# richardshuai/ExPecto

Measured on AMD Instinct MI355X. Metric: variants/sec (200 windows × 2002 feats) at 1/2/4/8 MI355X; HBM GB/s vs peak, higher is better.
Workload: dtype fp32 in/out (f16x3: power-of-2-scaled 2-way fp16 split = 22-bit operands, 3 MFMA products, fp32 accumulate; bf16x6 recompute on fp16 overflow)

## Files before the change

expecto_amd/csrc/beluga.hip:

```cpp
#include <hip/hip_runtime.h>

#include <algorithm>
#include <array>
#include <cassert>
#include <cstdint>
#include <cstdlib>
#include <cstring>
#include <map>
#include <mutex>
#include <tuple>
#include <string>
#include <vector>

#include "common.h"
#include "gemm_kernel.h"

namespace expecto {

constexpr int kLen = 2000;
constexpr int kNFeat = 2002;
constexpr int kFc1In = 67840;
constexpr int kFc1Out = 2003;
constexpr int kHidLd = 2016;
constexpr int kWM = 4;
// ... 218 lines not shown
  if (bad && ovf) *ovf = 1;
  _Float16* d = reinterpret_cast<_Float16*>(h1) + act_index<2>(row, kHidLd, n);
  *reinterpret_cast<halfx4*>(d) = hv;
  *reinterpret_cast<halfx4*>(d + 32) = lv;
}

constexpr int kFc2Chunk = 8;
__device__ __forceinline__ float fc2_value(float s, const float* __restrict__ col_scale, const float* __restrict__ bias,
                                           int n) {
  if (col_scale) s *= col_scale[n];
  const float v = s + bias[n];
  return 1.0f / (1.0f + expf(-v));
}
__global__ __launch_bounds__(256) void fc2_reduce(const float* __restrict__ part, int splits, long long split_stride,
                                                  int M, const float* __restrict__ bias,
                                                  const float* __restrict__ col_scale,
                                                  const long long* __restrict__ c_rows, float* __restrict__ y) {
  static_assert(kNFeat % 2 == 0 && kHidLd % 2 == 0, "2 features per thread");
  const int n = 2 * (blockIdx.x * blockDim.x + threadIdx.x);
  if (n >= kNFeat) return;
  for (long long m = blockIdx.y; m < M; m += gridDim.y) {
    const float* src = part + m * kHidLd + n;
    float s0 = 0.f, s1 = 0.f;
    for (int k0 = 0; k0 < splits; k0 += kFc2Chunk) {
      float2 v[kFc2Chunk];
#pragma unroll
      for (int u = 0; u < kFc2Chunk; ++u)
        v[u] = *reinterpret_cast<const float2*>(src + (long long)min(k0 + u, splits - 1) * split_stride);
#pragma unroll
      for (int u = 0; u < kFc2Chunk; ++u)
        if (k0 + u < splits) {
          s0 += v[u].x;
          s1 += v[u].y;
        }
    }
    float2 o;
    o.x = fc2_value(s0, col_scale, bias, n);
    o.y = fc2_value(s1, col_scale, bias, n + 1);
    *reinterpret_cast<float2*>(y + (c_rows ? c_rows[m] : m) * kNFeat + n) = o;
  }
}
__global__ void fc2_reduce1(const float* __restrict__ part, int splits, long long split_stride, int M,
                            const float* __restrict__ bias, const float* __restrict__ col_scale,
                            const long long* __restrict__ c_rows, float* __restrict__ y) {
  const long long i = (long long)blockIdx.x * blockDim.x + threadIdx.x;
  if (i >= (long long)M * kNFeat) return;
  const int m = (int)(i / kNFeat), n = (int)(i - (long long)m * kNFeat);
  const long long src = (long long)m * kHidLd + n;
  float s = 0.f;
  for (int k = 0; k < splits; ++k) s += part[k * split_stride + src];
  y[(c_rows ? c_rows[m] : m) * kNFeat + n] = fc2_value(s, col_scale, bias, n);
}

__global__ void pool4_phases(const float* __restrict__ in, int n_seg, int s_in, int t_in, int C,
                             int n_ph, int4 ph, int s_out, float* __restrict__ out, int fmt) {
  const int c = threadIdx.x;
  const int g = blockIdx.x;
  const int i = blockIdx.y % n_ph;
  const long long seg = blockIdx.y / n_ph;
  const int p = i == 0 ? ph.x : i == 1 ? ph.y : i == 2 ? ph.z : ph.w;
  if (c >= C || g >= (t_in - p) / 4) return;
  const long long r0 = seg * s_in + p + 4LL * g, orow = (seg * n_ph + i) * s_out + g;
  float m = load_act_rt(fmt, in, r0, C, c);
#pragma unroll
  for (int j = 1; j < 4; ++j) m = fmaxf(m, load_act_rt(fmt, in, r0 + j, C, c));
  store_act_rt(fmt, out, orow, C, c, m);
}

typedef _Float16 halfx8 __attribute__((ext_vector_type(8)));
__global__ __launch_bounds__(256) void pool4_phases_h2(const float* __restrict__ in, int s_in, int t_in, int C,
                                                        int n_ph, int4 ph, int s_out, float* __restrict__ out) {
  const int c8 = threadIdx.x & 63;
  const int g = blockIdx.x * 4 + (threadIdx.x >> 6);
  const int i = blockIdx.y % n_ph;
  const long long seg = blockIdx.y / n_ph;
  const int p = i == 0 ? ph.x : i == 1 ? ph.y : i == 2 ? ph.z : ph.w;
  if (c8 >= C / 8 || g >= (t_in - p) / 4) return;
  const long long rb = (long long)C * 4;
  const int cofs = (c8 >> 2) * 128 + (c8 & 3) * 16;
  const char* src = reinterpret_cast<const char*>(in) + (seg * s_in + p + 4LL * g) * rb + cofs;
  halfx8 hi[4], lo[4];
#pragma unroll
  for (int j = 0; j < 4; ++j) {
    hi[j] = *reinterpret_cast<const halfx8*>(src + j * rb);
    lo[j] = *reinterpret_cast<const halfx8*>(src + j * rb + 64);
  }
  halfx8 oh, ol;
#pragma unroll
  for (int e = 0; e < 8; ++e) {
    float m = (float)hi[0][e] + (float)lo[0][e];
#pragma unroll
    for (int j = 1; j < 4; ++j) m = fmaxf(m, (float)hi[j][e] + (float)lo[j][e]);
    _Float16 h, l;
    split_h2(m, h, l);
    oh[e] = h;
    ol[e] = l;
  }
  char* dst = reinterpret_cast<char*>(out) + ((seg * n_ph + i) * s_out + g) * rb + cofs;
  *reinterpret_cast<halfx8*>(dst) = oh;
  *reinterpret_cast<halfx8*>(dst + 64) = ol;
}

__global__ __launch_bounds__(256) void pool4_phases_h2m(const float* __restrict__ in, int s_in, int t_in, int C,
                                                         int n_ph, int4 ph, int s_out, float* __restrict__ out) {
  const int c8 = threadIdx.x & 63;
  const int g = blockIdx.x * 4 + (threadIdx.x >> 6);
  const long long seg = blockIdx.y;
  const int pmin = ph.x;
  const int pmax = n_ph == 1 ? ph.x : n_ph == 2 ? ph.y : n_ph == 3 ? ph.z : ph.w;
  if (c8 >= C / 8 || g >= (t_in - pmin) / 4) return;
  const long long rb = (long long)C * 4;
  const int cofs = (c8 >> 2) * 128 + (c8 & 3) * 16;
  const char* src = reinterpret_cast<const char*>(in) + (seg * s_in + pmin + 4LL * g) * rb + cofs;
  const int nr = min(pmax - pmin + 4, t_in - pmin - 4 * g);
  halfx8 hi[7], lo[7];
#pragma unroll
  for (int j = 0; j < 7; ++j) {
    if (j < nr) {
      hi[j] = *reinterpret_cast<const halfx8*>(src + j * rb);
      lo[j] = *reinterpret_cast<const halfx8*>(src + j * rb + 64);
    }
  }
  float fv[7][8];
#pragma unroll
  for (int j = 0; j < 7; ++j)
#pragma unroll
    for (int e = 0; e < 8; ++e) fv[j][e] = j < nr ? (float)hi[j][e] + (float)lo[j][e] : 0.f;
#pragma unroll
  for (int i = 0; i < 4; ++i) {
    if (i >= n_ph) break;
    const int p = i == 0 ? ph.x : i == 1 ? ph.y : i == 2 ? ph.z : ph.w;
    if (g >= (t_in - p) / 4) continue;
    const int o = p - pmin;
    halfx8 oh, ol;
#pragma unroll
    for (int e = 0; e < 8; ++e) {
      float m = 0.f;
#pragma unroll
      for (int j = 0; j < 4; ++j) {
        const float v = o == 0 ? fv[j][e] : o == 1 ? fv[j + 1][e] : o == 2 ? fv[j + 2][e] : fv[j + 3][e];
        m = j == 0 ? v : fmaxf(m, v);
      }
      _Float16 h, l;
      split_h2(m, h, l);
      oh[e] = h;
      ol[e] = l;
    }
    char* dst = reinterpret_cast<char*>(out) + ((seg * n_ph + i) * s_out + g) * rb + cofs;
    *reinterpret_cast<halfx8*>(dst) = oh;
    *reinterpret_cast<halfx8*>(dst + 64) = ol;
  }
}

__global__ void seg_a_rows(const int* __restrict__ win_seg, const int* __restrict__ win_off,
                           const int* __restrict__ win_row, const int* __restrict__ widx, int w0, int m_count,
                           int seg_base, int rc, int seg_len, int n_ph, int4 ph_idx, int s7, long long row_base,
                           long long* __restrict__ a_rows, long long* __restrict__ c_rows) {
  const int m = blockIdx.x * blockDim.x + threadIdx.x;
  if (m >= m_count) return;
  const int w = widx ? widx[m] : w0 + m;
  c_rows[m] = row_base + (win_row ? win_row[w] : w);
  const int o = rc ? seg_len - 2000 - win_off[w] : win_off[w];
  const int q = o >> 2, p = q & 3, off6 = (q - p) >> 2;
  const int pi = p == 0 ? ph_idx.x : p == 1 ? ph_idx.y : p == 2 ? ph_idx.z : ph_idx.w;
  const long long blk = (long long)(win_seg[w] - seg_base) * n_ph + pi;
  a_rows[m] = (blk * s7 + off6) * 640;
}

constexpr int kDW[7] = {0, 8, 5, 12, 6, 13, 20};
constexpr int kDA[7] = {0, 15, 28, 19, 32, 20, 27};
constexpr int kDT[7] = {0, 1993, 496, 489, 120, 113, 106};
constexpr int kDC[7] = {4, 320, 320, 480, 480, 640, 640};

struct DeltaRows {
  int r[7];
  int base[7];
};

__device__ __forceinline__ int clampi(int v, int lo, int hi) { return v < lo ? lo : (v > hi ? hi : v); }
__device__ __forceinline__ int floor4(int v) { return v >= 0 ? v >> 2 : -((3 - v) >> 2); }

__device__ __forceinline__ DeltaRows delta_rows(int p) {
  DeltaRows d;
  d.r[0] = p;
  d.r[1] = clampi(p - 7, 0, kDT[1] - kDW[1]);
  d.r[2] = clampi(floor4(d.r[1] - 7), 0, kDT[2] - kDW[2]);
  d.r[3] = clampi(d.r[2] - 7, 0, kDT[3] - kDW[3]);
  d.r[4] = clampi(floor4(d.r[3] - 7), 0, kDT[4] - kDW[4]);
  d.r[5] = clampi(d.r[4] - 7, 0, kDT[5] - kDW[5]);
  d.r[6] = clampi(d.r[5] - 7, 0, kDT[6] - kDW[6]);
  d.base[0] = 0;
  d.base[1] = d.r[1];
  d.base[2] = 4 * d.r[2];
  d.base[3] = d.r[3];
  d.base[4] = 4 * d.r[4];
  d.base[5] = d.r[5];
  d.base[6] = d.r[6];
  return d;
}

__device__ __forceinline__ int pair_pos(const int* var_pos, int m, int nv, int v0) {
  const int s = m / nv, v = v0 + m % nv;
  const int pv = min(max(var_pos[v], 0), kLen - 1);
  return s ? kLen - 1 - pv : pv;
}

__global__ void delta_codes(const uint8_t* __restrict__ alt, long long stride, int nv, int v0,
                            const int* __restrict__ var_pos, uint8_t* __restrict__ out, int R) {
  const int i = threadIdx.x & 15;
  const int m = blockIdx.x * (blockDim.x >> 4) + (threadIdx.x >> 4);
  if (m >= R) return;
  const int s = m / nv, v = v0 + m % nv;
  const int start = delta_rows(pair_pos(var_pos, m, nv, v0)).r[1];
  const uint8_t* a = alt + (long long)v * stride;
  const int pos = min(start + i, kLen - 1);
  uint8_t c;
  if (s) {
    const uint8_t f = a[kLen - 1 - pos];
    c = f < 4 ? (uint8_t)(3 - f) : f;
  } else {
    c = a[pos];
  }
  out[(long long)m * 16 + i] = c;
}

__global__ __launch_bounds__(256) void delta_assemble(const float* __restrict__ ref, int ref_rows,
                                                      const float* __restrict__ dprev, int l, int row16, int nv, int v0,
                                                      const int* __restrict__ var_pos, float* __restrict__ out) {
  const int m = blockIdx.x;
  const DeltaRows d = delta_rows(pair_pos(var_pos, m, nv, v0));
  const int rp = d.r[l - 1], wp = kDW[l - 1];
  floatx4* to = reinterpret_cast<floatx4*>(out) + (long long)m * kDA[l] * row16;
  for (int k = threadIdx.x; k < kDA[l] * row16; k += blockDim.x) {
    const int i = k / row16, c = k - i * row16;
    const int src = min(d.base[l] + i, ref_rows - 1);
    const floatx4* from = (src >= rp && src < rp + wp)
                              ? reinterpret_cast<const floatx4*>(dprev) + ((long long)m * wp + src - rp) * row16
                              : reinterpret_cast<const floatx4*>(ref) + ((long long)m * ref_rows + src) * row16;
    to[k] = from[c];
  }
}

__global__ void fc1_slab_mask(const int* __restrict__ var_pos, int nv, int v0, int R, int tile_rows, int slab_k,
                              unsigned* __restrict__ mask) {
  const int m = blockIdx.x * blockDim.x + threadIdx.x;
  if (m >= R) return;
  const int r6 = delta_rows(pair_pos(var_pos, m, nv, v0)).r[6];
  const int k0 = r6 * 640, k1 = (r6 + kDW[6]) * 640 - 1;
  unsigned bits = 0;
  for (int ks = k0 / slab_k; ks <= k1 / slab_k; ++ks) bits |= 1u << ks;
  atomicOr(mask + m / tile_rows, bits);
}

__global__ __launch_bounds__(64) void slab_macs(const unsigned* __restrict__ mask, int tiles, double per_bit,
                                                double* __restrict__ acc) {
  int bits = 0;
  for (int i = threadIdx.x; i < tiles; i += 64) bits += __popc(mask[i]);
  for (int o = 32; o > 0; o >>= 1) bits += __shfl_down(bits, o);
  if (threadIdx.x == 0) atomicAdd(acc, bits * per_bit);
}

__global__ __launch_bounds__(256) void pair_patch_apply(const float* __restrict__ d6, float* __restrict__ act6, int nv,
                                                        int v0, const int* __restrict__ var_pos, int row16) {
  const int m = blockIdx.x;
  const int r6 = delta_rows(pair_pos(var_pos, m, nv, v0)).r[6];
  const floatx4* src = reinterpret_cast<const floatx4*>(d6) + (long long)m * kDW[6] * row16;
  floatx4* dst = reinterpret_cast<floatx4*>(act6) + ((long long)m * 106 + r6) * row16;
  for (int k = threadIdx.x; k < kDW[6] * row16; k += blockDim.x) dst[k] = src[k];
}

constexpr int kSegTab = 20;
constexpr int kW4u = 19, kA4u = 26;
struct SegDims {
  int L, T1, P1, T3, T4, S5, T5, T6;
};

__global__ void seg_delta_table(const int* __restrict__ var_pos, int s0, int ns, int rc, SegDims g, int n_ph, int4 ph,
                                int* __restrict__ tab) {
  const int m = blockIdx.x * blockDim.x + threadIdx.x;
  if (m >= ns) return;
  int q = min(max(var_pos[s0 + m], 0), g.L - 1);
  if (rc) q = g.L - 1 - q;
  int* t = tab + m * kSegTab;
  const int r1 = clampi(q - 7, 0, g.T1 - kDW[1]);
  const int r2 = clampi(floor4(r1 - 7), 0, g.P1 - kDW[2]);
  const int r3 = clampi(r2 - 7, 0, g.T3 - kDW[3]);
  const int r4 = clampi(r3 - 7, 0, g.T4 - kW4u);
  t[0] = q;
  t[1] = r1;
  t[2] = r2;
  t[3] = r3;
  t[4] = r4;
  for (int i = 0; i < n_ph; ++i) {
    const int p = i == 0 ? ph.x : i == 1 ? ph.y : i == 2 ? ph.z : ph.w;
    const int r4p = clampi(floor4(r4 - p), 0, g.S5 - kDW[4]);
    const int r5 = clampi(r4p - 7, 0, g.T5 - kDW[5]);
    t[5 + i] = r4p;
    t[9 + i] = r5;
    t[13 + i] = clampi(r5 - 7, 0, g.T6 - kDW[6]);
  }
}

__global__ void seg_delta_codes(const uint8_t* __restrict__ codes, long long stride, const uint8_t* __restrict__ alt_code,
                                int s0, int ns, int rc, int L, const int* __restrict__ tab, uint8_t* __restrict__ out) {
  const int i = threadIdx.x & 15;
  const int m = blockIdx.x * (blockDim.x >> 4) + (threadIdx.x >> 4);
  if (m >= ns) return;
  const int q = tab[m * kSegTab], x = min(tab[m * kSegTab + 1] + i, L - 1);
  uint8_t c = x == q ? alt_code[s0 + m] : codes[(long long)(s0 + m) * stride + (rc ? L - 1 - x : x)];
  if (rc && c < 4) c = (uint8_t)(3 - c);
  out[(long long)m * 16 + i] = c;
}

constexpr int kC1Pat = kDA[2] + 7, kC1PatStride = 48;
__global__ void seg_delta_codes2(const uint8_t* __restrict__ codes, long long stride, const uint8_t* __restrict__ alt_code,
                                 int s0, int ns, int rc, int L, const int* __restrict__ tab, uint8_t* __restrict__ out) {
  const int i = threadIdx.x % kC1PatStride;
  const int m = blockIdx.x * (blockDim.x / kC1PatStride) + threadIdx.x / kC1PatStride;
  if (m >= ns) return;
  const int q = tab[m * kSegTab], x = 4 * tab[m * kSegTab + 2] + i;
  uint8_t c = 4;
  if (i < kC1Pat && x < L) {
    c = x == q ? alt_code[s0 + m] : codes[(long long)(s0 + m) * stride + (rc ? L - 1 - x : x)];
    if (rc && c < 4) c = (uint8_t)(3 - c);
  }
  out[(long long)m * kC1PatStride + i] = c;
}

__global__ void delta_codes2(const uint8_t* __restrict__ alt, long long stride, int nv, int v0,
                             const int* __restrict__ var_pos, uint8_t* __restrict__ out, int R) {
  const int i = threadIdx.x % kC1PatStride;
  const int m = blockIdx.x * (blockDim.x / kC1PatStride) + threadIdx.x / kC1PatStride;
  if (m >= R) return;
  const int s = m / nv, v = v0 + m % nv;
  const int pos = 4 * delta_rows(pair_pos(var_pos, m, nv, v0)).r[2] + i;
  const uint8_t* a = alt + (long long)v * stride;
  uint8_t c = 4;
  if (i < kC1Pat && pos < kLen) {
    if (s) {
      const uint8_t f = a[kLen - 1 - pos];
      c = f < 4 ? (uint8_t)(3 - f) : f;
    } else {
      c = a[pos];
    }
  }
  out[(long long)m * kC1PatStride + i] = c;
}

__global__ __launch_bounds__(256) void seg_delta_assemble(const float* __restrict__ ref, int ref_rows,
                                                          const float* __restrict__ dprev, int wprev,
                                                          const int* __restrict__ tab, int nb, int ib, int mult, int irp,
                                                          int arows, int row16, float* __restrict__ out) {
  const int m = blockIdx.x;
  const int seg = m / nb, off = nb > 1 ? m % nb : 0;
  const int base = mult * tab[seg * kSegTab + ib + off], rp = tab[seg * kSegTab + irp + off];
  floatx4* to = reinterpret_cast<floatx4*>(out) + (long long)m * arows * row16;
  for (int k = threadIdx.x; k < arows * row16; k += blockDim.x) {
    const int i = k / row16, c = k - i * row16;
    const int src = min(base + i, ref_rows - 1);
    const floatx4* from = (src >= rp && src < rp + wprev)
                              ? reinterpret_cast<const floatx4*>(dprev) + ((long long)m * wprev + src - rp) * row16
                              : reinterpret_cast<const floatx4*>(ref) + ((long long)m * ref_rows + src) * row16;
    to[k] = from[c];
  }
}

constexpr int kSegEdge = 32;
__device__ __forceinline__ int seg_edge_lo(const int* t) { return min(4 * t[5], 2 + 4 * t[6]); }
__global__ void seg_delta_pool(const float* __restrict__ conv4, int t4, const float* __restrict__ d4, int n_ph,
                               int4 ph, const int* __restrict__ tab, int fmt, float* __restrict__ out, int edge = 0) {
  const int c = threadIdx.x;
  if (c >= 480) return;
  const int gi = blockIdx.x, m = blockIdx.y;
  const int seg = m / n_ph, i = m % n_ph;
  const int p = i == 0 ? ph.x : i == 1 ? ph.y : i == 2 ? ph.z : ph.w;
  const int r4 = tab[seg * kSegTab + 4];
  const int row0 = p + 4 * (tab[seg * kSegTab + 5 + i] + gi);
  const int elo = edge ? seg_edge_lo(tab + seg * kSegTab) : 0;
  float mx = 0.f;
#pragma unroll
  for (int j = 0; j < 4; ++j) {
    const int row = row0 + j;
    const bool alt = row >= r4 && row < r4 + kW4u;
    const float* b = alt ? d4 : conv4;
    const long long r = alt    ? (long long)seg * kW4u + row - r4
                        : edge ? (long long)seg * kSegEdge + row - elo
                               : (long long)seg * t4 + row;
    const float v = load_act_rt(fmt, b, r, 480, c);
    mx = j == 0 ? v : fmaxf(mx, v);
  }
  store_act_rt(fmt, out, (long long)m * kDW[4] + gi, 480, c, mx);
}

__global__ void pool2_tile_seams(const float* __restrict__ seam, long long M, int s_in, int t4, int s5,
                                 float* __restrict__ out) {
  const int c8 = threadIdx.x;
  if (c8 >= 60) return;
  const long long k = blockIdx.x + 1, b = 256 * k;
  if (b + 1 >= M) return;
  const long long w = (b - 2) / s_in;
  const int t = (int)(b - 2 - w * s_in), g = (t - 2) >> 2;
  if (t + 3 >= t4) return;
  constexpr long long rb = 480 * 4;
  const int cofs = (c8 >> 2) * 128 + (c8 & 3) * 16;
  const char* sb = reinterpret_cast<const char*>(seam);
  const char* src[4] = {sb + ((k - 1) * 4 + 2) * rb, sb + ((k - 1) * 4 + 3) * rb, sb + (k * 4 + 0) * rb,
                        sb + (k * 4 + 1) * rb};
  halfx8 oh, ol;
  float m[8];
#pragma unroll
  for (int j = 0; j < 4; ++j) {
    const halfx8 hv = *reinterpret_cast<const halfx8*>(src[j] + cofs), lv = *reinterpret_cast<const halfx8*>(src[j] + cofs + 64);
#pragma unroll
    for (int e = 0; e < 8; ++e) {
      const float v = (float)hv[e] + (float)lv[e];
      m[e] = j == 0 ? v : fmaxf(m[e], v);
    }
  }
#pragma unroll
  for (int e = 0; e < 8; ++e) {
    _Float16 h, l;
    split_h2(m[e], h, l);
    oh[e] = h;
    ol[e] = l;
  }
  char* dst = reinterpret_cast<char*>(out) + ((2 * w + 1) * s5 + g) * rb + cofs;
  *reinterpret_cast<halfx8*>(dst) = oh;
  *reinterpret_cast<halfx8*>(dst + 64) = ol;
}

constexpr int kAltRows6 = 232;
__global__ void seg_alt_blocks(const float* __restrict__ ref6, const float* __restrict__ d6, int n_ph, int t6,
                               const int* __restrict__ tab, int row16, float* __restrict__ out) {
  const int m = blockIdx.y;
  const int q = tab[(m / n_ph) * kSegTab];
  const int t = (q >= 1999 ? (q - 1999) >> 4 : 0) + blockIdx.x;
  if (t >= t6 || t >= (q >> 4) + 106) return;
  const int r6 = tab[(m / n_ph) * kSegTab + 13 + m % n_ph];
  const floatx4* src = (t >= r6 && t < r6 + kDW[6])
                           ? reinterpret_cast<const floatx4*>(d6) + ((long long)m * kDW[6] + t - r6) * row16
                           : reinterpret_cast<const floatx4*>(ref6) + ((long long)m * t6 + t) * row16;
  floatx4* dst = reinterpret_cast<floatx4*>(out) + ((long long)m * t6 + t) * row16;
  for (int c = threadIdx.x; c < row16; c += blockDim.x) dst[c] = src[c];
}

__global__ void fc1_slab_mask_seg(const int* __restrict__ widx, int n_alt, const int* __restrict__ win_seg,
                                  const int* __restrict__ win_off, int seg_base, int rc, int seg_len, int4 ph_idx,
                                  const int* __restrict__ tab, int tile_rows, int slab_k, unsigned* __restrict__ mask) {
  const int m = blockIdx.x * blockDim.x + threadIdx.x;
  if (m >= n_alt) return;
  const int w = widx[m];
  const int o = rc ? seg_len - 2000 - win_off[w] : win_off[w];
  const int q = o >> 2, p = q & 3, off6 = (q - p) >> 2;
  const int pi = p == 0 ? ph_idx.x : p == 1 ? ph_idx.y : p == 2 ? ph_idx.z : ph_idx.w;
  const int r6 = tab[(win_seg[w] - seg_base) * kSegTab + 13 + pi];
  const int lo = max(r6 - off6, 0), hi = min(r6 + kDW[6] - off6, 106);
  if (lo >= hi) return;
  unsigned bits = 0;
  for (int ks = lo * 640 / slab_k; ks <= (hi * 640 - 1) / slab_k; ++ks) bits |= 1u << ks;
  atomicOr(mask + m / tile_rows, bits);
}

__global__ void copy_rows(const float* __restrict__ src, float* __restrict__ dst, const int* __restrict__ widx,
                          const int* __restrict__ win_row, long long row_base) {
  const int w = widx[blockIdx.x];
  const long long r = (row_base + (win_row ? win_row[w] : w)) * kNFeat;
  for (int i = threadIdx.x; i < kNFeat; i += blockDim.x) dst[r + i] = src[r + i];
}

__global__ void pair_rows(long long* __restrict__ c_rows, int M, int nv, int v0, long long strand_stride) {
  const int m = blockIdx.x * blockDim.x + threadIdx.x;
  if (m < M) c_rows[m] = (long long)(m / nv) * strand_stride + v0 + m % nv;
}

constexpr int kFkK = 16000;
constexpr int kFkKb = kFkK / GBK;
constexpr int kFkSlabs = 2;
constexpr int kFkTailK = kFc1In - 4 * kFkK;
constexpr int kFkKbTotal = 9 * kFkKb + kFkTailK / GBK;
constexpr long long kFkKTotal = 9LL * kFkK + kFkTailK;
constexpr int kFkSeq[9] = {3, 2, 3, 1, 0, 1, 3, 2, 3};
constexpr int kFkBlk[9] = {0, 1, 1, 2, 3, 3, 2, 3, 3};
constexpr int kFkRole[4][4] = {{0, 1, 3, 4}, {1, 2, 4, 5}, {3, 4, 6, 7}, {4, 5, 7, 8}};
constexpr int kFkW[9][4] = {{1, 0, 0, 0}, {1, 1, 0, 0}, {0, -1, 0, 0}, {1, 0, 1, 0}, {1, 1, 1, 1},
                            {0, -1, 0, -1}, {0, 0, -1, 0}, {0, 0, -1, -1}, {0, 0, 0, 1}};
constexpr int kFkParts = 4 * kFkSlabs + 1;

__global__ void fk_weights(const float* __restrict__ w1, long long rows, float* __restrict__ wk) {
  const long long i = (long long)blockIdx.x * blockDim.x + threadIdx.x;
  if (i >= rows * kFkKTotal) return;
  const long long n = i / kFkKTotal;
  const int k = (int)(i - n * kFkKTotal);
  const float* wr = w1 + n * kFc1In;
  if (k >= 9 * kFkK) {
    wk[i] = wr[4 * kFkK + (k - 9 * kFkK)];
    return;
  }
  const int g = k / kFkK, kk = k - g * kFkK;
  double s = 0.0;
#pragma unroll
  for (int q = 0; q < 4; ++q)
    if (kFkW[g][q]) s += kFkW[g][q] * (double)wr[q * kFkK + kk];
  wk[i] = (float)s;
}

__global__ __launch_bounds__(320) void fk_seq_h2(const float* __restrict__ x, int T, int s, const int* __restrict__ tab,
                                                 int n_ph, const int* __restrict__ gres, float* __restrict__ d1,
                                                 float* __restrict__ d2, float* __restrict__ dd, int* __restrict__ ovf) {
  const int c8 = threadIdx.x % 80;
  const long long blk = blockIdx.x / 7;
  const int k = (int)(blockIdx.x - blk * 7) * 4 + threadIdx.x / 80;
  if (k >= 25) return;
  int lo = 0, hi = T;
  if (tab) {
    const int q = tab[(blk / n_ph) * kSegTab];
    lo = q >= 1999 ? (q - 1999) >> 4 : 0;
    hi = min(T, (q >> 4) + 106);
  }
  const int g = gres ? gres[blk] : -1;
  if (g == -2) return;
  int r = k;
  if (r < lo) r += (lo - r + 24) / 25 * 25;
  if (r + 25 >= hi) return;
  constexpr long long rb = 640 * 4;
  const long long base = blk * s * rb + (c8 >> 2) * 128 + (c8 & 3) * 16;
  auto ld = [&](int row, float (&v)[8]) {
    const char* p = reinterpret_cast<const char*>(x) + base + row * rb;
    const halfx8 h = *reinterpret_cast<const halfx8*>(p);
    const halfx8 l = *reinterpret_cast<const halfx8*>(p + 64);
#pragma unroll
    for (int e = 0; e < 8; ++e) v[e] = (float)h[e] + (float)l[e];
  };
  bool bad = false;
  auto put = [&](float* dst, int row, const float (&y)[8]) {
    halfx8 h, l;
#pragma unroll
    for (int e = 0; e < 8; ++e) {
      bad |= !(fabsf(y[e]) < 65504.f);
      _Float16 a, b;
      split_h2p(y[e], a, b);
      h[e] = a;
      l[e] = b;
    }
    const int j = c8 & 7;
    const bool low = j < 4;
    u32x4 send = __builtin_bit_cast(u32x4, low ? l : h), recv;
#pragma unroll
    for (int w = 0; w < 4; ++w) recv[w] = (unsigned)__builtin_amdgcn_update_dpp(0, (int)send[w], 0x141, 0xf, 0xf, false);
    const u32x4 keep = __builtin_bit_cast(u32x4, low ? h : l);
    char* d = reinterpret_cast<char*>(dst) + blk * s * rb + row * rb + (c8 >> 3) * 256;
    auto st = [](char* p, const u32x4& v) { *reinterpret_cast<u32x4*>(p) = v; };
    if (low) {
      st(d + j * 16, keep);
      st(d + 128 + (3 - j) * 16, recv);
    } else {
      st(d + 64 + (7 - j) * 16, recv);
      st(d + 128 + 64 + (j - 4) * 16, keep);
    }
  };
  float v0[8], v1[8], v2[8] = {}, v3[8] = {};
  ld(r, v0);
  ld(r + 25, v1);
  if (r + 50 < hi) ld(r + 50, v2);
  if (r + 75 < hi) ld(r + 75, v3);
  for (; r + 25 < hi; r += 25) {
    float nv[8] = {};
    if (r + 100 < hi) ld(r + 100, nv);
    bool need1 = true, need2 = true;
    if (g >= 0) {
      const int rel = ((r - g) % 100 + 100) % 100;
      need1 = rel >= 50;
      need2 = (rel >= 25 && rel < 50) || rel >= 75;
    }
    float a[8], y[8];
#pragma unroll
    for (int e = 0; e < 8; ++e) a[e] = v0[e] - v1[e];
    if (need1) put(d1, r, a);
    if (r + 50 < hi && need2) {
#pragma unroll
      for (int e = 0; e < 8; ++e) y[e] = v0[e] - v2[e];
      put(d2, r, y);
    }
    if (r + 75 < hi) {
#pragma unroll
      for (int e = 0; e < 8; ++e) y[e] = a[e] - (v2[e] - v3[e]);
      put(dd, r, y);
    }
#pragma unroll
    for (int e = 0; e < 8; ++e) {
      v0[e] = v1[e];
      v1[e] = v2[e];
      v2[e] = v3[e];
      v3[e] = nv[e];
    }
  }
  if (bad) *ovf = 1;
}

__global__ void fk_reduce_h2(const float* __restrict__ part, const int* __restrict__ prow, long long count4,
                             const float* __restrict__ bias, float* __restrict__ h1, const float* __restrict__ col_scale,
                             float osc, int* __restrict__ ovf) {
  const long long i4 = (long long)blockIdx.x * blockDim.x + threadIdx.x;
  if (i4 >= count4) return;
  const long long row = i4 / (kHidLd / 4);
  const int n = (int)(i4 - row * (kHidLd / 4)) * 4;
  floatx4 s = {0.f, 0.f, 0.f, 0.f};
#pragma unroll
  for (int j = 0; j < kFkParts; ++j) {
    const floatx4 v = *reinterpret_cast<const floatx4*>(part + (long long)prow[row * kFkParts + j] * kHidLd + n);
#pragma unroll
    for (int e = 0; e < 4; ++e) s[e] += v[e];
  }
  halfx4 hv, lv;
  bool bad = false;
#pragma unroll
  for (int e = 0; e < 4; ++e) {
    const float t = s[e] * col_scale[n + e];
    const float v = n + e < kFc1Out ? fmaxf(t + bias[min(n + e, kFc1Out - 1)], 0.f) : 0.f;
    const float x = v * osc;
// ... 337 lines not shown
#pragma unroll
    for (int c = 0; c < 4; ++c) m[c] = r == 0 ? s[c] : fmaxf(m[c], s[c]);
  }
  floatx4 v;
  float vmax = 0.f;
#pragma unroll
  for (int c = 0; c < 4; ++c) {
    v[c] = fmaxf(fmaf(m[c], osc, bb[c] * osc), 0.f);
    vmax = fmaxf(vmax, v[c]);
  }
  if (fmt == 1) {
    bf16x4 x0, x1, x2;
    split3(v, x0, x1, x2);
    char* d = reinterpret_cast<char*>(out) + ((win * s_out + g) * 10 + (q >> 3)) * 192 + (q & 7) * 8;
    *reinterpret_cast<bf16x4*>(d) = x0;
    *reinterpret_cast<bf16x4*>(d + 64) = x1;
    *reinterpret_cast<bf16x4*>(d + 128) = x2;
    return;
  }
  const halfx4 hv = __builtin_convertvector(v, halfx4);
  const halfx4 lv = __builtin_convertvector(v - __builtin_convertvector(hv, floatx4), halfx4);
  char* d = reinterpret_cast<char*>(out) + ((win * s_out + g) * 10 + (q >> 3)) * 128 + (q & 7) * 8;
  *reinterpret_cast<halfx4*>(d) = hv;
  *reinterpret_cast<halfx4*>(d + 64) = lv;
  if (!(vmax < 65504.f)) *ovf = 1;
}

__global__ __launch_bounds__(256) void onehot_codes(const float* __restrict__ x, long long n, int len,
                                                    uint8_t* __restrict__ codes, int* __restrict__ bad) {
  const int len4 = len >> 2;
  const long long q = (long long)blockIdx.x * blockDim.x + threadIdx.x;
  if (q >= n * len4) return;
  const long long w = q / len4;
  const int p = (int)(q - w * len4) * 4;
  const float* xr = x + w * 4LL * len + p;
  unsigned b[4][4];
#pragma unroll
  for (int c = 0; c < 4; ++c) {
    const floatx4 v = *reinterpret_cast<const floatx4*>(xr + (long long)c * len);
#pragma unroll
    for (int e = 0; e < 4; ++e) b[c][e] = __float_as_uint(v[e]);
  }
  bool ok = true;
  unsigned packed = 0;
#pragma unroll
  for (int e = 0; e < 4; ++e) {
    unsigned code = 4, ones = 0;
#pragma unroll
    for (int c = 0; c < 4; ++c) {
      if (b[c][e] == 0x3f800000u) {
        ++ones;
        code = c;
      } else if (b[c][e] != 0u) {
        ok = false;
      }
    }
    ok &= ones <= 1;
    packed |= code << (8 * e);
  }
  if (!ok) *bad = 1;
  if (codes) *reinterpret_cast<unsigned*>(codes + w * len + p) = packed;
}

namespace {
constexpr int kNumLayers = 9;
struct ConvGeo {
  int cin, cout, s_in, t_valid, s_out, pool;
};
constexpr int kS1 = 1996;
constexpr ConvGeo kConv[5] = {
    {320, 320, kS1, 496, 496, 1},
    {320, 480, 496, 489, 492, 0},
    {480, 480, 492, 120, 120, 1},
    {480, 640, 120, 113, 113, 0},
    {640, 640, 113, 106, 106, 0},
};
constexpr int kFc2SplitsDefault = 7;
constexpr int kFcSplitsDefault = 8;
}

struct expecto_beluga {
  int device = 0;
  int max_batch = 0;
  float* w1 = nullptr;
  float* b1 = nullptr;
  float* wt[5] = {};
  float* bt[5] = {};
  float* fc1w = nullptr;
  float* fc1b = nullptr;
  float* fc2w = nullptr;
  float* fc2b = nullptr;
  float* wp[5] = {};
  float* fc1p = nullptr;
  float* fc2p = nullptr;
  float* wh[7] = {};
  int* swd[7] = {};
  float* w1h = nullptr;
  float* cs1 = nullptr;
  float* cs[7] = {};
  int sx[7] = {};
  int f16_target = 10;
  bool f16_ready = false;
  int* ovf = nullptr;
  bool ovf_deferred = false;
  float* calib = nullptr;
  long long fallbacks = 0;
  void* stage_buf[2] = {};
  size_t stage_cap[2] = {};
  hipEvent_t stage_ev[2] = {};
  int stage_next = 0;
  double* macs_d = nullptr;
  float* P = nullptr;
  float* Q = nullptr;
  float* part = nullptr;
  float* part2 = nullptr;
  float* h1 = nullptr;
  long long* a_rows = nullptr;
  long long* c_rows = nullptr;
  int fc2_rows = 0;
  int* win_seg_d = nullptr;
  int* alt_w_d = nullptr;
  int* copy_w_d = nullptr;
  int* seg_var_d = nullptr;
  int seg_var_cap = 0;
  int* win_off_d = nullptr;
  int* win_row_d = nullptr;
  int* fc_perm_d = nullptr;
  hipStream_t st2 = nullptr;
  hipEvent_t pev[16] = {};
  bool overlap = true;
  float* DA = nullptr;
  float* D0 = nullptr;
  float* D1 = nullptr;
  uint8_t* delta_codes = nullptr;
  int* seg_tab = nullptr;
  float* slab_mask = nullptr;
  int win_cap = 0;
  size_t bytes = 0;
  std::vector<void*> allocs;
  int precision = EXPECTO_PRECISION_BF16X6;
  int fc_splits = kFcSplitsDefault;
  int fc2_splits = kFc2SplitsDefault;
  double fc1_m_order_mb = 80.0;
  int fc1_order = 3;
  int fc1_m_group = 8;
  bool fc_wide = true;
  int conv_tile = 0;
  bool conv_ea = true;
  bool fc_skinny = true;
  int fc1_narrow = -1;
  int conv_narrow = -1;
  bool narrow_scope = false;
  int seg_chunk_windows = 0;
  int cus = 0;
  bool pool_one_pass = true;
  bool pool_fused = true;
  float* seam = nullptr;
  float* edge = nullptr;
  size_t seam_cap = 0, edge_cap = 0;
  bool fuse_conv1 = true;
  bool kmer_on = true;
  float* kmer = nullptr;
  uint64_t kmer_key = 0;
  bool kmer_quad = true;
  int kmer_state = 1;
  bool fk_on = true;
  int fk_role = 4;
  float* fkw = nullptr;
  int* fk_sw = nullptr;
  float* fk_cs = nullptr;
  float* fk_seq[3] = {};
  long long fk_seq_rows = 0;
  long long* fk_grows = nullptr;
  long long* fk_wrows = nullptr;
  int* fk_prow = nullptr;
  unsigned* fk_mask = nullptr;
  int fk_slice = 24576;
  float* fk_part = nullptr;
  float* fk_h1 = nullptr;
  long long* fk_arows = nullptr;
  long long* fk_crows = nullptr;
  int* fk_gres = nullptr;
  long long fk_gres_cap = 0;
  float* fk_aseq[3] = {};
  long long fk_aseq_rows = 0;
  int* fk_rgrp = nullptr;
  int* fk_ginfo = nullptr;
  int* fk_winfo = nullptr;
  int* fk_aprow = nullptr;
  int* fk_aperm = nullptr;
  unsigned* fk_smask = nullptr;
  bool onehot_as_codes = true;
  uint8_t* oh_codes = nullptr;
  int* oh_bad = nullptr;
  bool oh_hint_bad = false;
  int* hflags = nullptr;
  int* hflags_d = nullptr;
  bool profiling = false;
  std::vector<hipEvent_t> ev_pool;
  std::vector<std::pair<int, int>> pending;
  size_t ev_next = 0;
  int timer_base = 0;
  double ms[2 * kNumLayers] = {};
  long long calls[2 * kNumLayers] = {};
  double macs[2 * kNumLayers] = {};
  struct LaunchRec {
    int layer;
    long long rows;
    int idx;
    double macs;
  };
  std::vector<LaunchRec> pending_launch;
  std::map<std::pair<int, long long>, std::array<double, 3>> launch_stats;
};

namespace {
int dalloc(expecto_beluga* h, float** p, size_t nfloat) {
  void* ptr = nullptr;
  hipError_t e = hipMalloc(&ptr, nfloat * sizeof(float));
  if (e != hipSuccess) {
    set_error(std::string("hipMalloc: ") + hipGetErrorString(e));
    return EXPECTO_ENOMEM;
  }
  e = hipMemset(ptr, 0, nfloat * sizeof(float));
  if (e != hipSuccess) {
    (void)hipFree(ptr);
    set_error(std::string("hipMemset: ") + hipGetErrorString(e));
    return EXPECTO_EHIP;
  }
  h->allocs.push_back(ptr);
  h->bytes += nfloat * sizeof(float);
  *p = static_cast<float*>(ptr);
  return EXPECTO_OK;
}

int npad_of(int n) { return (n + GBN - 1) / GBN * GBN; }

struct KmerEntry {
  int device;
  uint64_t key;
  std::vector<float> w;
  float* T;
  std::vector<const expecto_beluga*> holders;
};
std::mutex g_kmer_mu;
std::vector<KmerEntry> g_kmer;

uint64_t fnv1a(const void* p, size_t n, uint64_t hsh = 1469598103934665603ULL) {
  const unsigned char* b = static_cast<const unsigned char*>(p);
  for (size_t i = 0; i < n; ++i) hsh = (hsh ^ b[i]) * 1099511628211ULL;
  return hsh;
}

int kmer_no_room(expecto_beluga* h, const char* why) {
  h->kmer_state = 2;
  fprintf(stderr, "expecto_hip: no k-mer tables on device %d (%s): conv2 runs on the MFMAs (about -25%% throughput)\n",
          h->device, why);
  return EXPECTO_OK;
}

int kmer_acquire(expecto_beluga* h, const float* const* params, hipStream_t st) {
  const size_t tb = kKmerFloats * sizeof(float), fb = (size_t)kMer8 * 320 * sizeof(double);
  if (const char* e = getenv("EXPECTO_KMER_MAX_BYTES"))
    if ((double)tb > atof(e)) return kmer_no_room(h, "EXPECTO_KMER_MAX_BYTES");
  std::vector<float> hw(320 * 32 + 320 + 320 * 320 * 8);
  EXPECTO_HIP_CHECK(hipMemcpyAsync(hw.data(), params[0], 320 * 32 * sizeof(float), hipMemcpyDeviceToHost, st));
  EXPECTO_HIP_CHECK(hipMemcpyAsync(hw.data() + 320 * 32, params[1], 320 * sizeof(float), hipMemcpyDeviceToHost, st));
  EXPECTO_HIP_CHECK(hipMemcpyAsync(hw.data() + 320 * 33, params[2], 320 * 320 * 8 * sizeof(float),
                                   hipMemcpyDeviceToHost, st));
  EXPECTO_HIP_CHECK(hipStreamSynchronize(st));
  const uint64_t key = fnv1a(hw.data(), hw.size() * sizeof(float));
  std::lock_guard<std::mutex> lock(g_kmer_mu);
  for (KmerEntry& e : g_kmer)
    if (e.device == h->device && e.key == key && e.w == hw) {
      e.holders.push_back(h);
      h->kmer = e.T;
      h->kmer_key = key;
      h->kmer_state = 0;
      return EXPECTO_OK;
    }
  void *t = nullptr, *f = nullptr, *gg = nullptr;
  if (hipMalloc(&t, tb) != hipSuccess || hipMalloc(&f, fb) != hipSuccess || hipMalloc(&gg, 8 * fb) != hipSuccess) {
    (void)hipGetLastError();
    for (void* x : {t, f, gg})
      if (x) (void)hipFree(x);
    return kmer_no_room(h, "device allocation failed");
  }
  float* T = static_cast<float*>(t);
  double* F = static_cast<double*>(f);
  double* G = static_cast<double*>(gg);
  kmer_conv1<<<dim3(kMer8), dim3(320), 0, st>>>(h->w1, h->b1, F);
  int rc = check_launch("kmer_conv1");
  for (int j = 0; j < 8; ++j)
    kmer_conv2<<<dim3((kMer8 + 63) / 64, 5), dim3(256), 0, st>>>(F, h->wt[0], j, G + (size_t)j * kMer8 * 320);
  for (int i = 0; i < 4; ++i)
    kmer_pair<<<dim3((unsigned)((kMer9 * 320 + 255) / 256)), dim3(256), 0, st>>>(
        G + (size_t)(2 * i) * kMer8 * 320, G + (size_t)(2 * i + 1) * kMer8 * 320, T + (size_t)i * kMer9 * 320);
  for (int hq = 0; hq < 2; ++hq)
    kmer_quad<<<dim3((unsigned)((kMer11 * 320 + 255) / 256)), dim3(256), 0, st>>>(
        G, hq, T + (4 * (size_t)kMer9 + hq * (size_t)kMer11) * 320);
  rc = rc ? rc : check_launch("kmer table");
  if (!rc && hipStreamSynchronize(st) != hipSuccess) rc = check_launch("kmer table sync");
  (void)hipFree(f);
  (void)hipFree(gg);
  if (rc) {
    (void)hipFree(t);
    return rc;
  }
  g_kmer.push_back({h->device, key, std::move(hw), T, {h}});
  h->kmer = T;
  h->kmer_key = key;
  h->kmer_state = 0;
  return EXPECTO_OK;
}

void kmer_release(expecto_beluga* h) {
  if (!h->kmer) return;
  std::lock_guard<std::mutex> lock(g_kmer_mu);
  for (size_t i = 0; i < g_kmer.size(); ++i)
    if (g_kmer[i].T == h->kmer) {
      auto& hs = g_kmer[i].holders;
      const auto it = std::find(hs.begin(), hs.end(), h);
      assert(it != hs.end() && "k-mer table held by an unregistered handle");
      if (it != hs.end()) hs.erase(it);
      if (hs.empty()) {
        (void)hipFree(g_kmer[i].T);
        g_kmer.erase(g_kmer.begin() + (long)i);
      }
      break;
    }
  h->kmer = nullptr;
}

size_t kmer_reported_bytes(const expecto_beluga* h) {
  if (!h->kmer) return 0;
  std::lock_guard<std::mutex> lock(g_kmer_mu);
// ... 398 lines not shown
    if ((rc = check_launch("beluga_conv_h3p pool2"))) return rc;
  }
  LayerTimer lt(h, 3, st);
  if (a.m_tiles > 1)
    pool2_tile_seams<<<dim3((unsigned)(a.m_tiles - 1)), dim3(64), 0, st>>>(h->seam, a.M, s_in, t4, s5, dst);
  return check_launch("pool2_tile_seams");
}

float* h1_rows(expecto_beluga* h, long long rows) { return h->h1 + rows * kHidLd * act_bytes() / 4; }

bool fc_wide_tiles(const expecto_beluga* h) { return h->fc_wide && g_precision == EXPECTO_PRECISION_F16X3; }

bool fc1_narrow(const expecto_beluga* h, long long mtt);
bool fc_skinny(const expecto_beluga* h, long long rows);

int run_fc1(expecto_beluga* h, const float* act, const long long* a_rows, int nb, float* h1, hipStream_t st,
            const unsigned* ks_mask = nullptr, double slab_frac = 1.0, long long part_rows = 0) {
  if (part_rows <= 0) part_rows = nb;
  int rc;
  const long long m_tiles = (nb + gemm_bm() - 1) / gemm_bm();
  const bool wide = fc_wide_tiles(h);
  const int n_tiles1 = wide ? (kHidLd + FCW_BN - 1) / FCW_BN : npad_of(kFc1Out) / GBN;
  const int splits = h->fc_splits;
  {
    GemmArgs a{};
    a.A = act;
    a.a_rows = a_rows;
    a.lda = (long long)kFc1In;
    a.M = nb;
    a.B = h->fc1w;
    a.Bp = g_precision == EXPECTO_PRECISION_F16X3 ? h->wh[5] : h->fc1p;
    a.ldb = kFc1In;
    a.kper = kFc1In / splits;
    a.taps = 1;
    a.n_tiles = n_tiles1;
    a.m_tiles = m_tiles;
    a.m_fastest = (double)m_tiles * gemm_bm() * (kFc1In / splits) * 4.0 <= h->fc1_m_order_mb * (1 << 20) ? 1 : 0;
    a.linear_order = a.m_fastest;
    if (h->fc1_order == 2 && !a.m_fastest && m_tiles % 8 == 0 && planes_gemm() && g_precision == EXPECTO_PRECISION_F16X3)
      a.m_fastest = 2;
    if (h->fc1_order == 3 && g_precision == EXPECTO_PRECISION_F16X3) {
      a.m_fastest = 3;
      a.m_group = h->fc1_m_group;
      a.linear_order = 0;
    }
    if (wide) {
      a.m_fastest = 0;
      a.linear_order = 0;
      a.n_tile_cols = FCW_BN;
      if (!ks_mask && fc_skinny(h, nb)) {
        a.n_tile_cols = 16 * FCS_NB;
        a.n_tiles = kHidLd / a.n_tile_cols;
      } else if (!ks_mask && fc1_narrow(h, m_tiles * splits)) {
        a.n_tile_cols = 112;
        a.n_tiles = kHidLd / 112;
      }
    }
    a.C = h->part;
    a.ldc = kHidLd;
    a.n_store = kHidLd;
    a.split_stride = part_rows * kHidLd;
    a.ks_mask = ks_mask;
    EXPECTO_REQUIRE(!ks_mask || planes_gemm(), "slab mask needs the planes GEMM");
    LayerTimer lt(h, 6, st);
    if (h->profiling) h->macs[h->timer_base + 6] += (double)nb * kFc1Out * kFc1In * slab_frac;
    if ((rc = launch_gemm<7, EPI_PARTIAL>(a, splits, st))) return rc;
  }
  {
    LayerTimer lt(h, 7, st);
    const long long count = (long long)nb * kHidLd;
    const bool f16 = g_precision == EXPECTO_PRECISION_F16X3;
    if (act_fmt() == 2)
      fc1_reduce_h2<<<dim3((unsigned)((count / 4 + 255) / 256)), dim3(256), 0, st>>>(
          h->part, splits, part_rows * kHidLd, count / 4, h->fc1b, h1, h->cs[5], exp2i(h->sx[6]), h->ovf);
    else
      fc1_reduce<<<dim3((unsigned)((count + 255) / 256)), dim3(256), 0, st>>>(
          h->part, splits, part_rows * kHidLd, count, h->fc1b, h1, act_fmt(), f16 ? h->cs[5] : nullptr, exp2i(h->sx[6]), h->ovf);
    if ((rc = check_launch("fc1_reduce"))) return rc;
  }
  return EXPECTO_OK;
}

int run_fc2(expecto_beluga* h, const float* h1, int nb, float* y, hipStream_t st, const long long* c_rows) {
  int rc;
  const long long m_tiles = (nb + gemm_bm() - 1) / gemm_bm();
  {
    GemmArgs a{};
    a.A = h1;
    a.lda = kHidLd;
    a.M = nb;
    a.B = h->fc2w;
    a.Bp = g_precision == EXPECTO_PRECISION_F16X3 ? h->wh[6] : h->fc2p;
    a.col_scale = g_precision == EXPECTO_PRECISION_F16X3 ? h->cs[6] : nullptr;
    a.ldb = kHidLd;
    a.kper = kHidLd / h->fc2_splits;
    a.taps = 1;
    const bool wide = fc_wide_tiles(h) && h->fc2_splits > 1;
    a.n_tiles = wide ? (kNFeat + FCW_BN - 1) / FCW_BN : npad_of(kNFeat) / GBN;
    a.m_tiles = m_tiles;
    a.m_fastest = (double)m_tiles * gemm_bm() * (kHidLd / h->fc2_splits) * 4.0 <= h->fc1_m_order_mb * (1 << 20) ? 1 : 0;
    if (wide) {
      a.m_fastest = 0;
      a.n_tile_cols = FCW_BN;
      if (fc_skinny(h, nb)) {
        a.n_tile_cols = 16 * FCS_NB;
        a.n_tiles = (kNFeat + a.n_tile_cols - 1) / a.n_tile_cols;
      } else if (fc1_narrow(h, m_tiles * h->fc2_splits)) {
        a.n_tile_cols = 112;
        a.n_tiles = (kNFeat + 111) / 112;
      }
    }
    a.C = h->part2;
    a.ldc = kHidLd;
    a.n_store = kNFeat;
    a.split_stride = (long long)nb * kHidLd;
    LayerTimer lt(h, 8, st);
    if (h->profiling) h->macs[h->timer_base + 8] += (double)nb * kNFeat * kFc1Out;
    if (h->fc2_splits == 1) {
      a.C = y;
      a.ldc = kNFeat;
      a.c_rows = c_rows;
      a.bias = h->fc2b;
      a.s_in = a.t_valid = a.s_out = 1;
      return launch_gemm<8, EPI_SIGMOID>(a, 1, st);
    }
    if ((rc = launch_gemm<8, EPI_PARTIAL>(a, h->fc2_splits, st))) return rc;
    if ((reinterpret_cast<uintptr_t>(y) & 7) == 0)
      fc2_reduce<<<dim3((unsigned)((kNFeat / 2 + 255) / 256), (unsigned)std::max<long long>(1, std::min<long long>(nb, 65535))), dim3(256), 0,
                   st>>>(h->part2, h->fc2_splits, (long long)nb * kHidLd, nb, h->fc2b, a.col_scale, c_rows, y);
    else
      fc2_reduce1<<<dim3((unsigned)(((long long)nb * kNFeat + 255) / 256)), dim3(256), 0, st>>>(
          h->part2, h->fc2_splits, (long long)nb * kHidLd, nb, h->fc2b, a.col_scale, c_rows, y);
    if ((rc = check_launch("fc2_reduce"))) return rc;
  }
  return EXPECTO_OK;
}

int run_fc(expecto_beluga* h, const float* act, const long long* a_rows, int nb, float* y, hipStream_t st,
           const long long* c_rows = nullptr, const unsigned* ks_mask = nullptr, double slab_frac = 1.0,
           long long part_rows = 0) {
  int rc;
  if ((rc = run_fc1(h, act, a_rows, nb, h->h1, st, ks_mask, slab_frac, part_rows))) return rc;
  return run_fc2(h, h->h1, nb, y, st, c_rows);
}

int count_desc_macs(expecto_beluga* h, const unsigned* mask, int tiles, double per_tile, hipStream_t st);

bool fk_use(const expecto_beluga* h) {
  return h->fk_on && h->fkw && g_precision == EXPECTO_PRECISION_F16X3 && h->fk_role < 4;
}
bool fk_use_seg(const expecto_beluga* h) { return h->fk_on && h->fkw && g_precision == EXPECTO_PRECISION_F16X3; }

int fk_cap(const expecto_beluga* h) { return std::max(h->max_batch, h->fk_slice); }

int fk_tables(expecto_beluga* h) {
  if (h->fk_grows) return EXPECTO_OK;
  const size_t mb = h->max_batch, tiles = (mb + 255) / 256, cap = fk_cap(h);
  float *a = nullptr, *b = nullptr, *c = nullptr, *d = nullptr;
  int rc;
  if ((rc = dalloc(h, &a, 2 * 9 * cap)) || (rc = dalloc(h, &b, 2 * mb)) || (rc = dalloc(h, &c, kFkParts * cap)) ||
      (rc = dalloc(h, &d, kFkParts * tiles)))
    return rc;
  h->fk_grows = reinterpret_cast<long long*>(a);
  h->fk_wrows = reinterpret_cast<long long*>(b);
  h->fk_prow = reinterpret_cast<int*>(c);
  h->fk_mask = reinterpret_cast<unsigned*>(d);
  return EXPECTO_OK;
}

int fk_seg_buffers(expecto_beluga* h) {
  if (h->fk_part) return EXPECTO_OK;
  const size_t cap = fk_cap(h);
  float *a = nullptr, *b = nullptr;
  int rc;
  if ((rc = dalloc(h, &h->fk_part, (size_t)kFkParts * cap * kHidLd)) || (rc = dalloc(h, &h->fk_h1, act_alloc(cap * kHidLd))) ||
      (rc = dalloc(h, &a, 2 * cap)) || (rc = dalloc(h, &b, 2 * cap)))
    return rc;
  h->fk_arows = reinterpret_cast<long long*>(a);
  h->fk_crows = reinterpret_cast<long long*>(b);
  float *c = nullptr, *d = nullptr, *e = nullptr, *f = nullptr, *q = nullptr, *m = nullptr;
  if ((rc = dalloc(h, &c, 9 * cap)) || (rc = dalloc(h, &d, 2 * cap)) || (rc = dalloc(h, &e, 2 * cap)) ||
      (rc = dalloc(h, &f, kFkParts * cap)) || (rc = dalloc(h, &q, cap)) || (rc = dalloc(h, &m, 19 * (cap / 256 + 1))))
    return rc;
  h->fk_rgrp = reinterpret_cast<int*>(c);
  h->fk_ginfo = reinterpret_cast<int*>(d);
  h->fk_winfo = reinterpret_cast<int*>(e);
  h->fk_aprow = reinterpret_cast<int*>(f);
  h->fk_aperm = reinterpret_cast<int*>(q);
  h->fk_smask = reinterpret_cast<unsigned*>(m);
  return EXPECTO_OK;
}

int fk_seq_alloc(expecto_beluga* h, long long rows, int set = 0) {
  float** b = set ? h->fk_aseq : h->fk_seq;
  long long& cap = set ? h->fk_aseq_rows : h->fk_seq_rows;
  if (rows <= cap && b[0]) return EXPECTO_OK;
  for (int i = 0; i < 3; ++i)
    if (b[i]) {
      EXPECTO_HIP_CHECK(hipFree(b[i]));
      b[i] = nullptr;
    }
  h->bytes -= (size_t)cap * 640 * 4 * 3;
  cap = 0;
  for (int i = 0; i < 3; ++i) {
    hipError_t e = hipMalloc(&b[i], (size_t)rows * 640 * 4 + 16 * 640 * 4);
    if (e != hipSuccess) {
      set_error(std::string("hipMalloc (FC1 sequences): ") + hipGetErrorString(e));
      return EXPECTO_ENOMEM;
    }
  }
  cap = rows;
  h->bytes += (size_t)rows * 640 * 4 * 3;
  return EXPECTO_OK;
}

int fk_sequences(expecto_beluga* h, const float* x, long long blocks, int T, int s, const int* tab, int n_ph,
                 hipStream_t st, const int* gres = nullptr, int set = 0) {
  int rc;
  if ((rc = fk_seq_alloc(h, blocks * s, set))) return rc;
  float* const* out = set ? h->fk_aseq : h->fk_seq;
  LayerTimer lt(h, 7, st);
  const long long nblk = blocks * 7;
  EXPECTO_REQUIRE(nblk > 0 && nblk < (1LL << 31), "FC1 sequence grid");
  fk_seq_h2<<<dim3((unsigned)nblk), dim3(320), 0, st>>>(x, T, s, tab, n_ph, gres, out[0], out[1], out[2], h->ovf);
  return check_launch("fk_seq_h2");
}

struct FkProducts {
  const long long* g_rows;
  int off[9];
  int cnt[9];
  int lay[9];
};

int fk_reduce(expecto_beluga* h, const float* part, const int* prow, int n, float* h1, hipStream_t st) {
  LayerTimer lt(h, 7, st);
  const long long count4 = (long long)n * (kHidLd / 4);
  fk_reduce_h2<<<dim3((unsigned)((count4 + 255) / 256)), dim3(256), 0, st>>>(part, prow, count4, h->fc1b, h1, h->fk_cs,
                                                                           exp2i(h->sx[6]), h->ovf);
  return check_launch("fk_reduce_h2");
}

constexpr int kFcNarrowNb = 7;
static_assert(kHidLd % (16 * kFcNarrowNb) == 0 && kHidLd % FCW_BN == 0, "FC1 N tiles");
bool fc1_narrow(const expecto_beluga* h, long long mtt) {
  if (h->fc1_narrow >= 0) return h->fc1_narrow != 0;
  if (!h->narrow_scope) return false;
  const long long cus = h->cus > 0 ? h->cus : 256;
  return mtt * (kHidLd / (16 * kFcNarrowNb)) <= cus;
}

static_assert(kHidLd % (16 * FCS_NB) == 0 &&
                  (kNFeat + 16 * FCS_NB - 1) / (16 * FCS_NB) * 16 * FCS_NB <= (kNFeat + GBN - 1) / GBN * GBN,
              "skinny FC tiles");
bool fc_skinny(const expecto_beluga* h, long long rows) {
  return h->fc_skinny && rows <= 32 && (h->fc1_narrow >= 0 ? h->fc1_narrow != 0 : h->narrow_scope);
}

int fk_fc1(expecto_beluga* h, const float* x, float* const* seq, const FkProducts& pr, const long long* w_rows, int n,
           const int* prow, float* h1, hipStream_t st, const unsigned* mask = nullptr, int tiles = 0,
           float* part = nullptr, long long part_cap = 0) {
  if (!part) {
    part = h->part;
    part_cap = (long long)std::max(h->fc_splits, kFkParts) * h->max_batch;
  }
  FcGroup G{};
  G.kb_total = kFkKbTotal;
  G.n_tiles = (kHidLd + FCW_BN - 1) / FCW_BN;
  G.n_store = kHidLd;
  G.ldc = kHidLd;
  const char* wb = reinterpret_cast<const char*>(h->fkw);
  long long row = 0;
  long long blk = 0;
  int mslot = 0;
  double macs = 0.0;
  auto add = [&](const float* A, const long long* ar, long long aoff, int kb0, int nk, int M, int lay) {
    FcDesc& d = G.d[G.n];
    d.A = A;
    d.a_rows = ar;
    d.a_off = aoff;
    d.Bp = wb + (long long)kb0 * 128;
    d.C = part + row * kHidLd;
    d.mask = mask ? mask + (size_t)mslot * tiles : nullptr;
    ++mslot;
    d.M = M;
    d.m_tiles = (M + X6P_BM - 1) / X6P_BM;
    d.nk = nk;
    d.blk0 = (int)blk;
    blk += (long long)d.m_tiles * G.n_tiles;
    row += lay;
    macs += (double)M * kFc1Out * nk * GBK;
    ++G.n;
  };
  for (int g = 0; g < 9; ++g) {
    const int lay = pr.lay[g] ? pr.lay[g] : pr.cnt[g];
    for (int s = 0; lay > 0 && s < kFkSlabs; ++s) {
      if (pr.cnt[g] > 0)
        add(kFkSeq[g] ? seq[kFkSeq[g] - 1] : x, pr.g_rows + pr.off[g], 25LL * kFkBlk[g] * 640 + (long long)s * kFkK / kFkSlabs,
            g * kFkKb + s * kFkKb / kFkSlabs, kFkKb / kFkSlabs, pr.cnt[g], lay);
      else {
        row += lay;
        ++mslot;
      }
    }
  }
  add(x, w_rows, 100LL * 640, 9 * kFkKb, kFkTailK / GBK, n, n);
  EXPECTO_REQUIRE(G.n <= FCK_MAX && blk < (1LL << 31), "Karatsuba FC1 descriptors");
  EXPECTO_REQUIRE(row <= part_cap, "Karatsuba FC1 partial rows");
  {
    LayerTimer lt(h, 6, st);
    if (h->profiling) {
      if (!mask) {
        h->macs[h->timer_base + 6] += macs;
      } else {
        for (int i = 0; i < G.n; ++i) {
          const FcDesc& d = G.d[i];
          int rc = count_desc_macs(h, d.mask, d.m_tiles, (double)d.M / d.m_tiles * kFc1Out * d.nk * GBK, st);
          if (rc) return rc;
        }
      }
    }
    G.rr = mask ? 0 : 1;
    const long long mtt = blk / G.n_tiles;
    const bool narrow = !mask && fc1_narrow(h, mtt);
    if (narrow) {
      G.n_tiles = kHidLd / (16 * kFcNarrowNb);
      for (int i = 0; i < G.n; ++i) G.d[i].blk0 = G.d[i].blk0 / (kHidLd / FCW_BN) * G.n_tiles;
    }
    const long long grid = G.rr ? (mtt + 7) / 8 * 8 * G.n_tiles : mtt * G.n_tiles;
    if (narrow)
      beluga_fc_h3k_narrow<<<dim3((unsigned)grid), dim3(512), 0, st>>>(G);
    else
      beluga_fc_h3k<0><<<dim3((unsigned)grid), dim3(512), 0, st>>>(G);
    int rc = check_launch("beluga_fc_h3k");
    if (rc) return rc;
  }
  return prow ? fk_reduce(h, part, prow, n, h1, st) : EXPECTO_OK;
}

struct FkWin {
  int w, blk, off6;
};
int fk_role_of(int off6) { return (off6 / 25) & 3; }
FkWin fk_win(int w, const int* win_seg, const int* win_off, int s0, bool rc, int L, int n_ph, const int* ph_idx) {
  const int o = rc ? L - kLen - win_off[w] : win_off[w];
  const int q = o >> 2, p = q & 3;
  return {w, (win_seg[w] - s0) * n_ph + ph_idx[p], (q - p) >> 2};
}
bool fk_same_group(const FkWin& a, const FkWin& b) {
  return a.blk == b.blk && a.off6 - 25 * fk_role_of(a.off6) == b.off6 - 25 * fk_role_of(b.off6);
}

void fk_slice_tables(const std::vector<FkWin>& ws, int i0, int i1, int T6, std::vector<long long>& grows,
                     FkProducts& pr, std::vector<int>& prow, std::vector<int>* rgrp = nullptr,
                     std::vector<int>* ginfo = nullptr) {
  const int n = i1 - i0;
  std::vector<int> gi(n);
  std::vector<long long> gst;
  std::vector<unsigned> need;
  for (int i = i0; i < i1; ++i) {
    const FkWin& w = ws[i];
    if (i == i0 || !fk_same_group(w, ws[i - 1])) {
      gst.push_back(((long long)w.blk * T6 + w.off6 - 25 * fk_role_of(w.off6)) * 640);
      need.push_back(0u);
    }
    gi[i - i0] = (int)gst.size() - 1;
    for (int j = 0; j < 4; ++j) need.back() |= 1u << kFkRole[fk_role_of(w.off6)][j];
    if (ginfo && gi[i - i0] * 2 == (int)ginfo->size()) {
      ginfo->push_back(w.blk);
      ginfo->push_back(w.off6 - 25 * fk_role_of(w.off6));
    }
  }
  const int ng = (int)gst.size();
  std::vector<int> ridx((size_t)9 * ng, -1);
  grows.clear();
  if (rgrp) rgrp->clear();
  for (int g = 0; g < 9; ++g) {
    pr.off[g] = (int)grows.size();
    int c = 0;
    for (int k = 0; k < ng; ++k)
      if ((need[k] >> g) & 1u) {
        ridx[(size_t)g * ng + k] = c++;
        grows.push_back(gst[k]);
        if (rgrp) rgrp->push_back(k);
      }
    pr.cnt[g] = c;
    pr.lay[g] = 0;
  }
  int base[9][kFkSlabs] = {};
  int row = 0;
  for (int g = 0; g < 9; ++g)
    for (int s = 0; pr.cnt[g] > 0 && s < kFkSlabs; ++s) {
      base[g][s] = row;
      row += pr.cnt[g];
    }
  prow.assign((size_t)n * kFkParts, 0);
  for (int i = 0; i < n; ++i) {
    const int role = fk_role_of(ws[i0 + i].off6);
    for (int j = 0; j < 4; ++j) {
      const int g = kFkRole[role][j];
      for (int s = 0; s < kFkSlabs; ++s) prow[(size_t)i * kFkParts + kFkSlabs * j + s] = base[g][s] + ridx[(size_t)g * ng + gi[i]];
    }
    prow[(size_t)i * kFkParts + kFkParts - 1] = row + i;
  }
}

int fk_windows(expecto_beluga* h, const float* act, int R, float* y, hipStream_t st, const long long* c_rows,
               const unsigned* mask = nullptr, int tiles = 0) {
  int rc;
  if ((rc = fk_tables(h)) || (rc = fk_sequences(h, act, R, 106, 106, nullptr, 1, st))) return rc;
  fk_window_tables<<<dim3((R + 255) / 256), dim3(256), 0, st>>>(R, 106, h->fk_role, h->fk_grows, h->fk_wrows, h->fk_prow);
  if ((rc = check_launch("fk_window_tables"))) return rc;
  FkProducts pr{h->fk_grows, {}, {}, {}};
  for (int j = 0; j < 4; ++j) pr.cnt[kFkRole[h->fk_role][j]] = R;
  if ((rc = fk_fc1(h, act, h->fk_seq, pr, h->fk_wrows, R, h->fk_prow, h->h1, st, mask, tiles))) return rc;
  return run_fc2(h, h->h1, R, y, st, c_rows);
}

int count_slab_macs(expecto_beluga* h, const unsigned* mask, int tiles, long long nb, hipStream_t st) {
  if (!h->macs_d) {
    float* f = nullptr;
    int rc = dalloc(h, &f, 4 * kNumLayers);
    if (rc) return rc;
    h->macs_d = reinterpret_cast<double*>(f);
    EXPECTO_HIP_CHECK(hipMemsetAsync(h->macs_d, 0, 2 * kNumLayers * sizeof(double), st));
  }
  const double per_bit = (double)nb * kFc1Out * kFc1In / ((double)tiles * h->fc_splits);
  slab_macs<<<dim3(1), dim3(64), 0, st>>>(mask, tiles, per_bit, h->macs_d + kNumLayers + 6);
  return check_launch("slab_macs");
}

int count_desc_macs(expecto_beluga* h, const unsigned* mask, int tiles, double per_tile, hipStream_t st) {
  if (!h->macs_d) {
    float* f = nullptr;
    int rc = dalloc(h, &f, 4 * kNumLayers);
    if (rc) return rc;
    h->macs_d = reinterpret_cast<double*>(f);
    EXPECTO_HIP_CHECK(hipMemsetAsync(h->macs_d, 0, 2 * kNumLayers * sizeof(double), st));
  }
  slab_macs<<<dim3(1), dim3(64), 0, st>>>(mask, tiles, per_tile, h->macs_d + h->timer_base + 6);
  return check_launch("slab_macs");
}

int forward_chunk(expecto_beluga* h, const float* x, const uint8_t* codes, long long code_stride, int n_src,
                  int mode, long long row0, int nb, float* y, hipStream_t st) {
  int rc;
  g_precision = h->precision;
  g_conv_ea = h->conv_ea;
  struct Scope {
    expecto_beluga* h;
    ~Scope() { h->narrow_scope = false; }
  } scope{h};
  h->narrow_scope = true;
  const bool kmer = use_kmer(h, x);
  const bool fuse = !kmer && fuse_conv1(h, x);
  const C1Src f1{codes, code_stride, n_src, mode, row0, kLen};
  if (!kmer && !fuse && (rc = run_conv1(h, x, codes, code_stride, n_src, mode, row0, nb, kLen, kS1, st))) return rc;
  float* src = h->P;
  float* dst = h->Q;
  for (int l = 0; l < 5; ++l) {
    const ConvGeo& g = kConv[l];
    if (l == 0 && kmer)
      rc = run_conv2_kmer(h, f1, nb, g.t_valid, g.s_out, dst, st);
    else
      rc = run_conv(h, l, src, dst, nb, g.s_in, g.t_valid, g.s_out, g.pool != 0, st, l == 0 && fuse ? &f1 : nullptr);
    if (rc) return rc;
    std::swap(src, dst);
  }
  if (fk_use(h)) return fk_windows(h, src, nb, y, st, nullptr);
  return run_fc(h, src, nullptr, nb, y, st);
}

int ensure_delta(expecto_beluga* h) {
  if (h->DA) return EXPECTO_OK;
  const size_t pad = 16 * 640;
  const size_t da = (size_t)h->max_batch * kDA[6] * 640 + pad, dd = (size_t)h->max_batch * kDW[6] * 640 + pad;
  float *pc = nullptr, *tb = nullptr;
  int rc;
  if ((rc = dalloc(h, &h->DA, act_alloc(da))) || (rc = dalloc(h, &h->D0, act_alloc(dd))) ||
      (rc = dalloc(h, &h->D1, act_alloc(dd))) || (rc = dalloc(h, &pc, (size_t)h->max_batch * kC1PatStride / 4)) ||
      (rc = dalloc(h, &tb, (size_t)h->max_batch * kSegTab)) ||
      (rc = dalloc(h, &h->slab_mask, (size_t)h->max_batch / 64 + 64)))
    return rc;
  h->delta_codes = reinterpret_cast<uint8_t*>(pc);
  h->seg_tab = reinterpret_cast<int*>(tb);
  if (h->overlap) {
    EXPECTO_HIP_CHECK(hipStreamCreateWithFlags(&h->st2, hipStreamNonBlocking));
    for (hipEvent_t& e : h->pev) EXPECTO_HIP_CHECK(hipEventCreateWithFlags(&e, hipEventDisableTiming));
  }
  return EXPECTO_OK;
}

struct SegGeo {
  int L, T1, S1, P1, T3, T4, S5, T5, T6;
  size_t p_rows_floats, q_rows_floats;
};

SegGeo seg_geo(int L, int n_ph) {
  SegGeo g{};
  g.L = L;
  g.T1 = L - 7;
  g.S1 = (g.T1 + 3) / 4 * 4;
  g.P1 = (g.T1 - 7) / 4;
  g.T3 = g.P1 - 7;
  g.T4 = g.T3 - 7;
  g.S5 = g.T4 / 4;
  g.T5 = g.S5 - 7;
  g.T6 = g.T5 - 7;
  const size_t p_conv1 = (size_t)g.S1 * 320, p_conv3 = (size_t)((g.T3 + 3) & ~3) * 480, p_pool2 = (size_t)n_ph * g.S5 * 480,
               p_conv6 = (size_t)n_ph * g.T6 * 640;
  const size_t q_pool1 = (size_t)g.P1 * 320, q_conv4 = (size_t)g.T4 * 480, q_conv5 = (size_t)n_ph * g.T5 * 640;
  g.p_rows_floats = std::max(std::max(p_conv1, p_conv3), std::max(p_pool2, p_conv6));
  g.q_rows_floats = std::max(q_pool1, std::max(q_conv4, q_conv5));
  return g;
}

struct SegPairs {
  const int* var_pos;
  const uint8_t* alt_code;
  float* y_alt;
  long long strand_stride;
};

int forward_segments(expecto_beluga* h, const uint8_t* codes, int n_seg, int L, long long code_stride, int mode,
                     const int* win_seg, const int* win_off, const int* win_row, int n_win, float* y,
                     hipStream_t st, const SegPairs* pr = nullptr) {
  EXPECTO_REQUIRE(L >= kLen && L % 4 == 0, "segment length must be >= 2000 and a multiple of 4");
  g_precision = h->precision;
  g_conv_ea = h->conv_ea;
  int rc;
  if (pr && (rc = ensure_delta(h))) return rc;
  int present[4] = {0, 0, 0, 0};
  for (int w = 0; w < n_win; ++w) {
    EXPECTO_REQUIRE(win_seg[w] >= 0 && win_seg[w] < n_seg, "window segment out of range");
    EXPECTO_REQUIRE(w == 0 || win_seg[w] >= win_seg[w - 1], "windows must be sorted by segment");
    const int o = win_off[w];
    EXPECTO_REQUIRE(o >= 0 && o % 4 == 0 && o + kLen <= L, "window offset must be 4-aligned inside the segment");
    if (mode != EXPECTO_STRAND_RC) present[(o >> 2) & 3] = 1;
    if (mode != EXPECTO_STRAND_FWD) present[((L - kLen - o) >> 2) & 3] = 1;
  }
  int n_ph = 0, ph[4] = {0, 0, 0, 0}, ph_idx[4] = {0, 0, 0, 0};
  for (int p = 0; p < 4; ++p)
    if (present[p]) {
      ph_idx[p] = n_ph;
      ph[n_ph++] = p;
    }
  const SegGeo g = seg_geo(L, std::max(n_ph, 1));
  const size_t p_cap = p_floats(h->max_batch) - 16 * 640, q_cap = q_floats(h->max_batch) - 16 * 640;
  const int seg_cap = (int)std::min<size_t>(p_cap / g.p_rows_floats, q_cap / g.q_rows_floats);
  EXPECTO_REQUIRE(seg_cap >= 1, "segment too long for this handle's workspace (raise max_batch)");
  std::vector<int> first(n_seg + 1, n_win);
  for (int w = n_win - 1; w >= 0; --w) first[win_seg[w]] = w;
  for (int sg = n_seg - 1; sg >= 0; --sg) first[sg] = std::min(first[sg], first[sg + 1]);
  if (n_win > h->win_cap) {
    for (int** b : {&h->win_seg_d, &h->win_off_d, &h->win_row_d, &h->alt_w_d, &h->copy_w_d, &h->fc_perm_d}) {
      if (*b) EXPECTO_HIP_CHECK(hipFree(*b));
      *b = nullptr;
    }
    h->win_cap = 0;
    for (int** b : {&h->win_seg_d, &h->win_off_d, &h->win_row_d, &h->alt_w_d, &h->copy_w_d})
      EXPECTO_HIP_CHECK(hipMalloc(b, n_win * sizeof(int)));
    EXPECTO_HIP_CHECK(hipMalloc(&h->fc_perm_d, 4 * n_win * sizeof(int)));
    h->win_cap = n_win;
  }
  std::vector<int> alt_w, copy_w;
  if (pr) {
    for (int sg = 0; sg < n_seg; ++sg)
      EXPECTO_REQUIRE(pr->var_pos[sg] >= 0 && pr->var_pos[sg] < L, "variant position outside its segment");
    for (int w = 0; w < n_win; ++w) {
      const int q = pr->var_pos[win_seg[w]];
      (win_off[w] <= q && q < win_off[w] + kLen ? alt_w : copy_w).push_back(w);
    }
    if (n_seg > h->seg_var_cap) {
      if (h->seg_var_d) EXPECTO_HIP_CHECK(hipFree(h->seg_var_d));
      h->seg_var_d = nullptr;
      h->seg_var_cap = 0;
      EXPECTO_HIP_CHECK(hipMalloc(&h->seg_var_d, n_seg * sizeof(int)));
      h->seg_var_cap = n_seg;
    }
  }
  std::vector<HostCopy> copies;
  if (pr) {
    copies.push_back({h->seg_var_d, pr->var_pos, n_seg * sizeof(int)});
    copies.push_back({h->alt_w_d, alt_w.data(), alt_w.size() * sizeof(int)});
    copies.push_back({h->copy_w_d, copy_w.data(), copy_w.size() * sizeof(int)});
  }
  if (win_row) {
    for (int w = 0; w < n_win; ++w) EXPECTO_REQUIRE(win_row[w] >= 0 && win_row[w] < n_win, "window row out of range");
    copies.push_back({h->win_row_d, win_row, n_win * sizeof(int)});
  }
  copies.push_back({h->win_seg_d, win_seg, n_win * sizeof(int)});
  copies.push_back({h->win_off_d, win_off, n_win * sizeof(int)});
  const int strands = mode == EXPECTO_STRAND_BOTH ? 2 : 1;
  const int blk_per_seg = pr ? std::max(n_ph, 1) : 0;
  std::vector<std::pair<int, int>> chunks;
  for (int s0 = 0; s0 < n_seg;) {
    int s1 = s0 + 1;
    while (s1 < n_seg && s1 - s0 < seg_cap && (long long)(s1 + 1 - s0) * blk_per_seg <= h->max_batch &&
           (h->seg_chunk_windows <= 0 || first[s1 + 1] - first[s0] <= h->seg_chunk_windows))
      ++s1;
    chunks.push_back({s0, s1});
    s0 = s1;
  }
  std::vector<int> fc_perm;
  if (pr) {
    fc_perm.resize((size_t)strands * n_win);
    std::vector<char> is_alt(n_win, 0);
    for (int w : alt_w) is_alt[w] = 1;
    for (int sd = 0; sd < strands; ++sd) {
      const bool rcs = (mode == EXPECTO_STRAND_RC) || sd == 1;
      int* out = fc_perm.data() + (size_t)sd * n_win;
      for (const auto& c : chunks) {
        const int w0 = first[c.first], w1 = first[c.second];
        int k = w0;
        std::vector<int> a;
        for (int w = w0; w < w1; ++w)
          if (is_alt[w]) a.push_back(w);
        std::stable_sort(a.begin(), a.end(), [&](int x, int y) {
          const int px = pr->var_pos[win_seg[x]] - win_off[x], py = pr->var_pos[win_seg[y]] - win_off[y];
          return rcs ? px > py : px < py;
        });
        for (int w : a) out[k++] = w;
        for (int w = w0; w < w1; ++w)
          if (!is_alt[w]) out[k++] = w;
      }
    }
    copies.push_back({h->fc_perm_d, fc_perm.data(), fc_perm.size() * sizeof(int)});
  }
  const bool fkm = fk_use_seg(h) && !(pr && 3 * alt_w.size() > (size_t)n_win);
  std::vector<std::vector<FkWin>> fk_ref, fk_alt;
  std::vector<char> fk_is_alt(pr ? n_win : 0, 0);
  for (int w : alt_w) fk_is_alt[w] = 1;
  if (fkm) {
    fc_perm.assign((size_t)4 * n_win, 0);
    for (int sd = 0; sd < strands; ++sd) {
      const bool rcs = (mode == EXPECTO_STRAND_RC) || sd == 1;
      for (const auto& c : chunks) {
        const int w0 = first[c.first], w1 = first[c.second];
        struct Key {
          int cls;
          long long rel;
          int blk, G, off6, w;
        };
        std::vector<FkWin> ref, alt;
        std::vector<Key> key;
        std::map<std::pair<int, int>, int> galt;
        for (int w = w0; w < w1; ++w) {
          const FkWin fw = fk_win(w, win_seg, win_off, c.first, rcs, L, n_ph, ph_idx);
          ref.push_back(fw);
          if (pr && fk_is_alt[w]) {
            alt.push_back(fw);
            galt[{fw.blk, fw.off6 - 25 * fk_role_of(fw.off6)}] = 1;
          }
        }
        for (const FkWin& fw : ref) {
          const int G = fw.off6 - 25 * fk_role_of(fw.off6);
          const bool ga = pr && galt.count({fw.blk, G});
          long long rel = 0;
          if (ga) {
            const int q = pr->var_pos[win_seg[fw.w]];
            rel = (long long)(rcs ? L - 1 - q : q) - 16LL * G;
          }
          key.push_back({ga ? 0 : 1, rel, fw.blk, G, fw.off6, fw.w});
        }
        std::vector<int> ord(ref.size());
        for (size_t k = 0; k < ord.size(); ++k) ord[k] = (int)k;
        std::sort(ord.begin(), ord.end(), [&](int a, int b) {
          const Key &x = key[a], &y = key[b];
          return std::tie(x.cls, x.rel, x.blk, x.G, x.off6, x.w) < std::tie(y.cls, y.rel, y.blk, y.G, y.off6, y.w);
        });
        std::vector<FkWin> sorted;
        for (int k : ord) sorted.push_back(ref[k]);
        for (size_t k = 0; k < sorted.size(); ++k) fc_perm[(size_t)sd * n_win + w0 + k] = sorted[k].w;
        fk_ref.push_back(std::move(sorted));
        fk_alt.push_back(std::move(alt));
      }
    }
    if (pr) copies.pop_back();
    copies.push_back({h->fc_perm_d, fc_perm.data(), fc_perm.size() * sizeof(int)});
  }
  if ((rc = stage_copies(h, copies, st))) return rc;
  const long long strand_rows = pr ? pr->strand_stride : n_win;
  const int eb = act_bytes();
  hipStream_t sa = (pr && h->st2) ? h->st2 : st;
  const SegDims gd{L, g.T1, g.P1, g.T3, g.T4, g.S5, g.T5, g.T6};
  const int4 ph4 = make_int4(ph[0], ph[1], ph[2], ph[3]);
  for (int sd = 0; sd < strands; ++sd) {
    const bool is_rc = (mode == EXPECTO_STRAND_RC) || sd == 1;
    for (const auto& chunk : chunks) {
      const int s0 = chunk.first, s1 = chunk.second;
      const int w0 = first[s0], nw = first[s1] - first[s0];
      const int ns = s1 - s0;
      const long long nb = (long long)ns * n_ph;
      auto alt_asm = [&](int l, const float* ref, int ref_rows, const float* dprev, int wprev, int nbk, int ib,
                         int mult, int irp, int arows, hipEvent_t ready, hipEvent_t done) -> int {
        if (sa != st) {
          EXPECTO_HIP_CHECK(hipEventRecord(ready, st));
          EXPECTO_HIP_CHECK(hipStreamWaitEvent(sa, ready, 0));
        }
        const int row16 = kConv[l].cin * eb / 16;
        seg_delta_assemble<<<dim3(ns * nbk), dim3(256), 0, sa>>>(ref, ref_rows, dprev, wprev, h->seg_tab, nbk,
                                                                      ib, mult, irp, arows, row16, h->DA);
        int r = check_launch("seg_delta_assemble");
        if (!r && sa != st) EXPECTO_HIP_CHECK(hipEventRecord(done, sa));
        return r;
      };
      auto alt_gemm = [&](int l, int nbk, int arows, int w, bool pool, float* dnext) -> int {
        DeltaScope ds(h);
        return run_conv(h, l, h->DA, dnext, (long long)ns * nbk, arows, w, w, pool, sa);
      };
      auto st_wait = [&](hipEvent_t e) -> int {
        if (sa != st) EXPECTO_HIP_CHECK(hipStreamWaitEvent(st, e, 0));
        return EXPECTO_OK;
      };
      if (pr && sa != st) {
        EXPECTO_HIP_CHECK(hipEventRecord(h->pev[0], st));
        EXPECTO_HIP_CHECK(hipStreamWaitEvent(sa, h->pev[0], 0));
      }
      const bool kmer = use_kmer(h, nullptr);
      const bool fuse = !kmer && fuse_conv1(h, nullptr);
      const C1Src f1{codes + (long long)s0 * code_stride, code_stride, ns, is_rc ? EXPECTO_STRAND_RC : EXPECTO_STRAND_FWD,
                     0, L};
      if (!kmer && !fuse && (rc = run_conv1(h, nullptr, f1.codes, code_stride, ns, f1.mode, 0, ns, L, g.S1, st)))
        return rc;
      if (pr) {
        seg_delta_table<<<dim3((ns + 255) / 256), dim3(256), 0, sa>>>(h->seg_var_d, s0, ns, is_rc ? 1 : 0, gd, n_ph,
                                                                     ph4, h->seg_tab);
        if ((rc = check_launch("seg_delta_table"))) return rc;
        if (kmer || fuse) {
          seg_delta_codes2<<<dim3((ns + 4) / 5), dim3(5 * kC1PatStride), 0, sa>>>(
              codes, code_stride, pr->alt_code, s0, ns, is_rc ? 1 : 0, L, h->seg_tab, h->delta_codes);
          if ((rc = check_launch("seg_delta_codes2"))) return rc;
          DeltaScope ds(h);
          if (fuse && (rc = run_conv1(h, nullptr, h->delta_codes, kC1PatStride, ns, EXPECTO_STRAND_FWD, 0, ns, kC1Pat,
                                      kDA[2], sa, h->DA)))
            return rc;
        } else {
          seg_delta_codes<<<dim3((ns + 15) / 16), dim3(256), 0, sa>>>(codes, code_stride, pr->alt_code, s0, ns,
                                                                     is_rc ? 1 : 0, L, h->seg_tab, h->delta_codes);
          if ((rc = check_launch("seg_delta_codes"))) return rc;
          DeltaScope ds(h);
          if ((rc = run_conv1(h, nullptr, h->delta_codes, 16, ns, EXPECTO_STRAND_FWD, 0, ns, kDA[1], kDW[1], sa,
                              h->D0)))
            return rc;
        }
      }
      if (pr && !kmer && !fuse && (rc = alt_asm(0, h->P, g.S1, h->D0, kDW[1], 1, 2, 4, 1, kDA[2], h->pev[1], h->pev[2])))
        return rc;
      if (kmer)
        rc = run_conv2_kmer(h, f1, ns, g.P1, g.P1, h->Q, st);
      else
        rc = run_conv(h, 0, h->P, h->Q, ns, g.S1, g.P1, g.P1, true, st, fuse ? &f1 : nullptr);
      if (rc) return rc;
      if (pr && kmer) {
        DeltaScope ds(h);
        const C1Src fa{h->delta_codes, kC1PatStride, ns, EXPECTO_STRAND_FWD, 0, kC1Pat};
        if ((rc = run_conv2_kmer(h, fa, ns, kDW[2], kDW[2], h->D1, sa))) return rc;
      } else if (pr && ((!fuse && (rc = st_wait(h->pev[2]))) || (rc = alt_gemm(0, 1, kDA[2], kDW[2], true, h->D1)))) {
        return rc;
      }
      if (pr && (rc = alt_asm(1, h->Q, g.P1, h->D1, kDW[2], 1, 3, 1, 2, kDA[3], h->pev[3], h->pev[4]))) return rc;
      const int T3p = (g.T3 + 3) & ~3;
      if ((rc = run_conv(h, 1, h->Q, h->P, ns, g.P1, g.T3, T3p, false, st))) return rc;
      if (pr && ((rc = st_wait(h->pev[4])) || (rc = alt_gemm(1, 1, kDA[3], kDW[3], false, h->D0)))) return rc;
      if (pr && (rc = alt_asm(2, h->P, T3p, h->D0, kDW[3], 1, 4, 1, 3, kA4u, h->pev[5], h->pev[6]))) return rc;
      const bool pfused = conv4_pool_fused(h, (long long)ns * T3p, n_ph, ph);
      struct PQSwap {
        expecto_beluga* h;
        bool on;
        ~PQSwap() {
          if (on) std::swap(h->P, h->Q);
        }
      } pq{h, false};
      if (pfused) {
        if ((rc = run_conv4_pool_fused(h, h->P, h->Q, ns, T3p, g.T4, g.S5, pr ? h->seg_tab : nullptr, st))) return rc;
        std::swap(h->P, h->Q);
        pq.on = true;
      } else if ((rc = run_conv(h, 2, h->P, h->Q, ns, T3p, g.T4, g.T4, false, st))) {
        return rc;
      }
      if (pr && ((rc = st_wait(h->pev[6])) || (rc = alt_gemm(2, 1, kA4u, kW4u, false, h->D1)))) return rc;
      if (!pfused) {
        LayerTimer lt(h, 3, st);
        if (act_fmt() == 2 && h->pool_one_pass) {
          dim3 grid((g.S5 + 3) / 4, ns);
          pool4_phases_h2m<<<grid, dim3(256), 0, st>>>(h->Q, g.T4, g.T4, 480, n_ph, ph4, g.S5, h->P);
        } else if (act_fmt() == 2) {
          dim3 grid((g.S5 + 3) / 4, ns * n_ph);
          pool4_phases_h2<<<grid, dim3(256), 0, st>>>(h->Q, g.T4, g.T4, 480, n_ph, ph4, g.S5, h->P);
        } else {
          dim3 grid(g.S5, ns * n_ph);
          pool4_phases<<<grid, dim3(480), 0, st>>>(h->Q, ns, g.T4, g.T4, 480, n_ph, ph4, g.S5, h->P, act_fmt());
        }
        if ((rc = check_launch("pool4_phases"))) return rc;
      }
      if (pr) {
        if (sa != st) {
          EXPECTO_HIP_CHECK(hipEventRecord(h->pev[7], st));
          EXPECTO_HIP_CHECK(hipStreamWaitEvent(sa, h->pev[7], 0));
        }
        seg_delta_pool<<<dim3(kDW[4], (unsigned)nb), dim3(480), 0, sa>>>(pfused ? h->edge : h->Q, g.T4, h->D1, n_ph,
                                                                         ph4, h->seg_tab, act_fmt(), h->D0,
                                                                         pfused ? 1 : 0);
        if ((rc = check_launch("seg_delta_pool"))) return rc;
        if (sa != st) EXPECTO_HIP_CHECK(hipEventRecord(h->pev[8], sa));
        if ((rc = alt_asm(3, h->P, g.S5, h->D0, kDW[4], n_ph, 9, 1, 5, kDA[5], h->pev[9], h->pev[10]))) return rc;
        if ((rc = st_wait(h->pev[8]))) return rc;
      }
      if ((rc = run_conv(h, 3, h->P, h->Q, nb, g.S5, g.T5, g.T5, false, st))) return rc;
      if (pr && ((rc = st_wait(h->pev[10])) || (rc = alt_gemm(3, n_ph, kDA[5], kDW[5], false, h->D1)))) return rc;
      if (pr && (rc = alt_asm(4, h->Q, g.T5, h->D1, kDW[5], n_ph, 13, 1, 9, kDA[6], h->pev[11], h->pev[12])))
        return rc;
      if ((rc = run_conv(h, 4, h->Q, h->P, nb, g.T5, g.T6, g.T6, false, st))) return rc;
      if (pr) {
        if ((rc = alt_gemm(4, n_ph, kDA[6], kDW[6], false, h->D0))) return rc;
        if (sa != st) EXPECTO_HIP_CHECK(hipEventRecord(h->pev[13], sa));
      }
      if (nw > 0 && fkm) {
        const int4 phi = make_int4(ph_idx[0], ph_idx[1], ph_idx[2], ph_idx[3]);
        const long long row_base = (long long)sd * strand_rows;
        const size_t ci = (size_t)sd * chunks.size() + (size_t)(&chunk - chunks.data());
        const long long cap = fk_cap(h);
        const std::vector<FkWin>& ws = fk_ref[ci];
        const int* perm = h->fc_perm_d + (size_t)sd * n_win + w0;
        std::vector<int> gres((size_t)nb, -2);
        for (const FkWin& w : ws) {
          const int r = (w.off6 - 25 * fk_role_of(w.off6)) % 100;
          int& e = gres[(size_t)w.blk];
          e = e == -2 ? r : (e == r ? r : -1);
        }
        if (nb > h->fk_gres_cap) {
          if (h->fk_gres) EXPECTO_HIP_CHECK(hipFree(h->fk_gres));
          h->fk_gres = nullptr;
          h->bytes -= (size_t)h->fk_gres_cap * sizeof(int);
          h->fk_gres_cap = 0;
          EXPECTO_HIP_CHECK(hipMalloc(&h->fk_gres, (size_t)nb * sizeof(int)));
          h->fk_gres_cap = nb;
          h->bytes += (size_t)nb * sizeof(int);
        }
        if ((rc = stage_copies(h, {{h->fk_gres, gres.data(), gres.size() * sizeof(int)}}, st)) || (rc = fk_tables(h)) ||
            (rc = fk_seg_buffers(h)) || (rc = fk_sequences(h, h->P, nb, g.T6, g.T6, nullptr, n_ph, st, h->fk_gres)))
          return rc;
        const bool has_alt = pr && !fk_alt[ci].empty();
        bool alt_ready = false;
        for (size_t i0 = 0; i0 < ws.size();) {
          size_t i1 = i0;
          while (i1 < ws.size()) {
            size_t j = i1 + 1;
            while (j < ws.size() && fk_same_group(ws[j], ws[i1])) ++j;
            if (j - i0 > (size_t)cap && i1 > i0) break;
            i1 = j;
          }
          EXPECTO_REQUIRE(i1 - i0 <= (size_t)cap, "a Karatsuba FC1 window group exceeds the FC1 slice");
          const int fn = (int)(i1 - i0);
          std::vector<long long> grows;
          std::vector<int> prow, rgrp, ginfo;
          FkProducts prd{h->fk_grows, {}, {}, {}};
          fk_slice_tables(ws, (int)i0, (int)i1, g.T6, grows, prd, prow, &rgrp, &ginfo);
          if ((rc = stage_copies(h, {{h->fk_grows, grows.data(), grows.size() * sizeof(long long)},
                                     {h->fk_prow, prow.data(), prow.size() * sizeof(int)}}, st)))
            return rc;
          seg_a_rows<<<dim3((fn + 255) / 256), dim3(256), 0, st>>>(
              h->win_seg_d, h->win_off_d, win_row ? h->win_row_d : nullptr, perm + i0, 0, fn, s0, is_rc ? 1 : 0, L,
              n_ph, phi, g.T6, row_base, h->fk_arows, h->fk_crows);
          if ((rc = check_launch("seg_a_rows")) ||
              (rc = fk_fc1(h, h->P, h->fk_seq, prd, h->fk_arows, fn, h->fk_prow, h->fk_h1, st, nullptr, 0, h->fk_part,
                           kFkParts * cap)))
            return rc;
          for (int r0 = 0; r0 < fn; r0 += h->max_batch)
            if ((rc = run_fc2(h, h->fk_h1 + (long long)r0 * kHidLd, std::min(h->max_batch, fn - r0), y, st,
                              h->fk_crows + r0)))
              return rc;
          int n_ag = 0;
          size_t nw_pre = 0;
          for (size_t i = i0; has_alt && i < i1; ++i) {
            bool galt = false;
            size_t j = i;
            for (; j < i1 && fk_same_group(ws[j], ws[i]); ++j) galt |= fk_is_alt[ws[j].w] != 0;
            if (!galt) break;
            ++n_ag;
            nw_pre = j - i0;
            i = j - 1;
          }
          if (n_ag > 0) {
            FkProducts pa = prd;
            FkMaskDesc md{};
            for (int gq = 0; gq < 9; ++gq) {
              int c = 0;
              for (int i = 0; i < prd.cnt[gq]; ++i)
                if (rgrp[prd.off[gq] + i] < n_ag) ++c;
              pa.cnt[gq] = c;
              pa.lay[gq] = prd.cnt[gq];
              for (int sb = 0; prd.cnt[gq] > 0 && sb < kFkSlabs; ++sb) {
                md.g[md.n] = gq;
                md.s[md.n] = sb;
                md.off[md.n] = prd.off[gq];
                md.cnt[md.n] = c;
                ++md.n;
              }
            }
            md.nw = (int)nw_pre;
            std::vector<int> winfo, aperm, aprow;
            for (size_t i = 0; i < nw_pre; ++i) {
              winfo.push_back(ws[i0 + i].blk);
              winfo.push_back(ws[i0 + i].off6);
              if (fk_is_alt[ws[i0 + i].w]) {
                aperm.push_back(ws[i0 + i].w);
                aprow.insert(aprow.end(), prow.begin() + (long long)i * kFkParts, prow.begin() + (long long)(i + 1) * kFkParts);
              }
            }
            const int na = (int)aperm.size();
            const int tiles = (int)(cap / 256 + 1);
            if ((rc = stage_copies(h, {{h->fk_rgrp, rgrp.data(), rgrp.size() * sizeof(int)},
                                       {h->fk_ginfo, ginfo.data(), ginfo.size() * sizeof(int)},
                                       {h->fk_winfo, winfo.data(), winfo.size() * sizeof(int)},
                                       {h->fk_aperm, aperm.data(), aperm.size() * sizeof(int)},
                                       {h->fk_aprow, aprow.data(), aprow.size() * sizeof(int)}}, st)))
              return rc;
            if (!alt_ready) {
              if ((rc = st_wait(h->pev[13]))) return rc;
              seg_alt_blocks<<<dim3(kAltRows6, (unsigned)nb), dim3(64), 0, st>>>(h->P, h->D0, n_ph, g.T6, h->seg_tab,
                                                                                640 * eb / 16, h->Q);
              if ((rc = check_launch("seg_alt_blocks"))) return rc;
              DeltaScope ds(h);
              if ((rc = fk_sequences(h, h->Q, nb, g.T6, g.T6, h->seg_tab, n_ph, st, h->fk_gres, 1))) return rc;
              alt_ready = true;
            }
            EXPECTO_HIP_CHECK(hipMemsetAsync(h->fk_smask, 0, (size_t)(md.n + 1) * tiles * sizeof(unsigned), st));
            int rows_max = md.nw;
            for (int i = 0; i < md.n; ++i) rows_max = std::max(rows_max, md.cnt[i]);
            if (rows_max > 0) {
              fk_seg_mask<<<dim3((rows_max + 255) / 256, md.n + 1), dim3(256), 0, st>>>(
                  md, h->fk_rgrp, h->fk_ginfo, h->fk_winfo, h->seg_tab, n_ph, make_int4(0, 0, 0, 0), tiles, h->fk_smask);
              if ((rc = check_launch("fk_seg_mask"))) return rc;
            }
            DeltaScope ds(h);
            if ((rc = fk_fc1(h, h->Q, h->fk_aseq, pa, h->fk_arows, (int)nw_pre, nullptr, h->fk_h1, st, h->fk_smask, tiles,
                             h->fk_part, kFkParts * cap)) ||
                (na > 0 && (rc = fk_reduce(h, h->fk_part, h->fk_aprow, na, h->fk_h1, st))))
              return rc;
            if (na > 0) {
              seg_a_rows<<<dim3((na + 255) / 256), dim3(256), 0, st>>>(
                  h->win_seg_d, h->win_off_d, win_row ? h->win_row_d : nullptr, h->fk_aperm, 0, na, s0, is_rc ? 1 : 0,
                  L, n_ph, phi, g.T6, row_base, h->fk_arows, h->fk_crows);
              if ((rc = check_launch("seg_a_rows"))) return rc;
              for (int r0 = 0; r0 < na; r0 += h->max_batch)
                if ((rc = run_fc2(h, h->fk_h1 + (long long)r0 * kHidLd, std::min(h->max_batch, na - r0), pr->y_alt, st,
                                  h->fk_crows + r0)))
                  return rc;
            }
          }
          i0 = i1;
        }
        if (pr) {
          const int ic0 = (int)(std::lower_bound(copy_w.begin(), copy_w.end(), w0) - copy_w.begin());
          const int ic1 = (int)(std::lower_bound(copy_w.begin(), copy_w.end(), w0 + nw) - copy_w.begin());
          if (ic1 > ic0) {
            copy_rows<<<dim3(ic1 - ic0), dim3(256), 0, st>>>(y, pr->y_alt, h->copy_w_d + ic0,
                                                             win_row ? h->win_row_d : nullptr, row_base);
            if ((rc = check_launch("copy_rows"))) return rc;
          }
        }
      } else if (nw > 0) {
        const int4 phi = make_int4(ph_idx[0], ph_idx[1], ph_idx[2], ph_idx[3]);
        const long long row_base = (long long)sd * strand_rows;
        const int* widx = pr ? h->fc_perm_d + (size_t)sd * n_win + w0 : nullptr;
        int n_alt = 0, ic0 = 0, ic1 = 0;
        if (pr) {
          n_alt = (int)(std::lower_bound(alt_w.begin(), alt_w.end(), w0 + nw) -
                        std::lower_bound(alt_w.begin(), alt_w.end(), w0));
          ic0 = (int)(std::lower_bound(copy_w.begin(), copy_w.end(), w0) - copy_w.begin());
          ic1 = (int)(std::lower_bound(copy_w.begin(), copy_w.end(), w0 + nw) - copy_w.begin());
        }
        const bool gather2 = h->fc2_splits == 1;
        int pend = 0;
        auto flush2 = [&]() -> int {
          const int n2 = pend;
          pend = 0;
          return n2 ? run_fc2(h, h->h1, n2, y, st, h->c_rows) : EXPECTO_OK;
        };
        for (int f0 = 0; f0 < nw; f0 += h->max_batch) {
          const int fn = std::min(h->max_batch, nw - f0);
          if (gather2 && pend + fn > h->fc2_rows && (rc = flush2())) return rc;
          long long* crow = h->c_rows + (gather2 ? pend : 0);
          seg_a_rows<<<dim3((fn + 255) / 256), dim3(256), 0, st>>>(
              h->win_seg_d, h->win_off_d, win_row ? h->win_row_d : nullptr, widx ? widx + f0 : nullptr, w0 + f0,
              fn, s0, is_rc ? 1 : 0, L, n_ph, phi, g.T6, row_base, h->a_rows, crow);
          if ((rc = check_launch("seg_a_rows"))) return rc;
          if (gather2) {
            if ((rc = run_fc1(h, h->P, h->a_rows, fn, h1_rows(h, pend), st))) return rc;
            pend += fn;
          } else if ((rc = run_fc(h, h->P, h->a_rows, fn, y, st, h->c_rows))) {
            return rc;
          }
          const int na = std::min(n_alt - f0, fn);
          if (na <= 0) continue;
          if (f0 == 0) {
            if ((rc = st_wait(h->pev[13]))) return rc;
            seg_alt_blocks<<<dim3(kAltRows6, (unsigned)nb), dim3(64), 0, st>>>(h->P, h->D0, n_ph, g.T6, h->seg_tab,
                                                                              640 * eb / 16, h->Q);
            if ((rc = check_launch("seg_alt_blocks"))) return rc;
          }
          long long* acrow = gather2 ? h->c_rows + h->fc2_rows : h->c_rows;
          seg_a_rows<<<dim3((na + 255) / 256), dim3(256), 0, st>>>(
              h->win_seg_d, h->win_off_d, win_row ? h->win_row_d : nullptr, widx + f0, 0, na, s0, is_rc ? 1 : 0,
              L, n_ph, phi, g.T6, row_base, h->a_rows, acrow);
          if ((rc = check_launch("seg_a_rows"))) return rc;
          const unsigned* mask = nullptr;
          double frac = 1.0;
          if (planes_gemm()) {
            const int tiles = (int)((na + gemm_bm() - 1) / gemm_bm());
            unsigned* md = reinterpret_cast<unsigned*>(h->slab_mask);
            EXPECTO_HIP_CHECK(hipMemsetAsync(md, 0, tiles * sizeof(unsigned), st));
            fc1_slab_mask_seg<<<dim3((na + 255) / 256), dim3(256), 0, st>>>(
                widx + f0, na, h->win_seg_d, h->win_off_d, s0, is_rc ? 1 : 0, L, phi, h->seg_tab, (int)gemm_bm(),
                kFc1In / h->fc_splits, md);
            if ((rc = check_launch("fc1_slab_mask_seg"))) return rc;
            mask = md;
            if (h->profiling) {
              if ((rc = count_slab_macs(h, md, tiles, na, st))) return rc;
              frac = 0.0;
            }
          }
          DeltaScope ds(h);
          if (gather2) {
            float* h1a = h1_rows(h, h->fc2_rows);
            if ((rc = run_fc1(h, h->Q, h->a_rows, na, h1a, st, mask, frac, fn)) ||
                (rc = run_fc2(h, h1a, na, pr->y_alt, st, acrow)))
              return rc;
          } else if ((rc = run_fc(h, h->Q, h->a_rows, na, pr->y_alt, st, h->c_rows, mask, frac, fn))) {
            return rc;
          }
        }
        if ((rc = flush2())) return rc;
        if (pr) {
          if (ic1 > ic0) {
            copy_rows<<<dim3(ic1 - ic0), dim3(256), 0, st>>>(y, pr->y_alt, h->copy_w_d + ic0,
                                                             win_row ? h->win_row_d : nullptr, row_base);
            if ((rc = check_launch("copy_rows"))) return rc;
          }
        }
      }
      if (pr && (rc = st_wait(h->pev[13]))) return rc;
    }
  }
  return EXPECTO_OK;
}
int forward_pairs(expecto_beluga* h, const uint8_t* ref, const uint8_t* alt, int n, long long stride,
                  const int* var_pos, int mode, float* y_ref, float* y_alt, long long strand_stride, hipStream_t st) {
  g_precision = h->precision;
  g_conv_ea = h->conv_ea;
  const int strands = mode == EXPECTO_STRAND_BOTH ? 2 : 1;
  int rc;
  if ((rc = ensure_delta(h))) return rc;
  const int eb = act_bytes();
  const int nv_max = std::max(1, h->max_batch / strands);
  hipStream_t sa = h->st2 ? h->st2 : st;
  auto order = [&](hipStream_t from, hipStream_t to, hipEvent_t e) -> int {
    if (from == to) return EXPECTO_OK;
    EXPECTO_HIP_CHECK(hipEventRecord(e, from));
    EXPECTO_HIP_CHECK(hipStreamWaitEvent(to, e, 0));
    return EXPECTO_OK;
  };
  for (int v0 = 0; v0 < n; v0 += nv_max) {
    const int nv = std::min(nv_max, n - v0), R = strands * nv;
    if ((rc = order(st, sa, h->pev[0]))) return rc;
    const bool kmer = use_kmer(h, nullptr);
    const bool fuse = !kmer && fuse_conv1(h, nullptr);
    const C1Src f1{ref + (long long)v0 * stride, stride, nv, mode, 0, kLen};
    if (!kmer && !fuse && (rc = run_conv1(h, nullptr, f1.codes, stride, nv, mode, 0, R, kLen, kS1, st))) return rc;
    if (kmer || fuse) {
      delta_codes2<<<dim3((R + 4) / 5), dim3(5 * kC1PatStride), 0, sa>>>(alt, stride, nv, v0, var_pos, h->delta_codes, R);
      if ((rc = check_launch("delta_codes2"))) return rc;
      DeltaScope ds(h);
      if (fuse && (rc = run_conv1(h, nullptr, h->delta_codes, kC1PatStride, R, EXPECTO_STRAND_FWD, 0, R, kC1Pat, kDA[2],
                                  sa, h->DA)))
        return rc;
    } else {
      delta_codes<<<dim3((R + 15) / 16), dim3(256), 0, sa>>>(alt, stride, nv, v0, var_pos, h->delta_codes, R);
      if ((rc = check_launch("delta_codes"))) return rc;
      DeltaScope ds(h);
      if ((rc = run_conv1(h, nullptr, h->delta_codes, 16, R, EXPECTO_STRAND_FWD, 0, R, kDA[1], kDW[1], sa, h->D0)))
        return rc;
    }
    float* src = h->P;
    float* dst = h->Q;
    float* dprev = h->D0;
    float* dnext = h->D1;
    for (int l = 0; l < 5; ++l) {
      const ConvGeo& g = kConv[l];
      const int L = l + 2;
      if ((rc = order(st, sa, h->pev[1 + 2 * l]))) return rc;
      const bool fused = l == 0 && fuse;
      const bool tab = l == 0 && kmer;
      if (tab)
        rc = run_conv2_kmer(h, f1, R, g.t_valid, g.s_out, dst, st);
      else
        rc = run_conv(h, l, src, dst, R, g.s_in, g.t_valid, g.s_out, g.pool != 0, st, fused ? &f1 : nullptr);
      if (rc) return rc;
      const int row16 = g.cin * eb / 16;
      if (!fused && !tab) {
        delta_assemble<<<dim3(R), dim3(256), 0, sa>>>(src, g.s_in, dprev, L, row16, nv, v0, var_pos, h->DA);
        if ((rc = check_launch("delta_assemble"))) return rc;
      }
      if ((rc = order(sa, st, h->pev[2 + 2 * l]))) return rc;
      DeltaScope ds(h);
      if (tab) {
        const C1Src fa{h->delta_codes, kC1PatStride, R, EXPECTO_STRAND_FWD, 0, kC1Pat};
        if ((rc = run_conv2_kmer(h, fa, R, kDW[L], kDW[L], dnext, sa))) return rc;
      } else if ((rc = run_conv(h, l, h->DA, dnext, R, kDA[L], kDW[L], kDW[L], g.pool != 0, sa))) {
        return rc;
      }
      std::swap(src, dst);
      std::swap(dprev, dnext);
    }
    if ((rc = order(sa, st, h->pev[11]))) return rc;
    float* act6 = src;
    pair_rows<<<dim3((R + 255) / 256), dim3(256), 0, st>>>(h->c_rows, R, nv, v0, strand_stride);
    if ((rc = check_launch("pair_rows"))) return rc;
    const bool fk = fk_use(h);
    if ((rc = fk ? fk_windows(h, act6, R, y_ref, st, h->c_rows) : run_fc(h, act6, nullptr, R, y_ref, st, h->c_rows)))
      return rc;
    pair_patch_apply<<<dim3(R), dim3(256), 0, st>>>(dprev, act6, nv, v0, var_pos, 640 * eb / 16);
    if ((rc = check_launch("pair_patch_apply"))) return rc;
    if (fk) {
      const int tiles = (R + X6P_BM - 1) / X6P_BM;
      EXPECTO_HIP_CHECK(hipMemsetAsync(h->fk_mask, 0, (size_t)kFkParts * tiles * sizeof(unsigned), st));
      fk_window_mask<<<dim3((R + 255) / 256), dim3(256), 0, st>>>(var_pos, nv, v0, R, h->fk_role, tiles, h->fk_mask);
      if ((rc = check_launch("fk_window_mask"))) return rc;
      DeltaScope ds(h);
      if ((rc = fk_windows(h, act6, R, y_alt, st, h->c_rows, h->fk_mask, tiles))) return rc;
      continue;
    }
    const unsigned* mask = nullptr;
    double frac = 1.0;
    if (planes_gemm()) {
      const int tiles = (int)((R + gemm_bm() - 1) / gemm_bm());
      unsigned* md = reinterpret_cast<unsigned*>(h->slab_mask);
      EXPECTO_HIP_CHECK(hipMemsetAsync(md, 0, tiles * sizeof(unsigned), st));
      fc1_slab_mask<<<dim3((R + 255) / 256), dim3(256), 0, st>>>(var_pos, nv, v0, R, (int)gemm_bm(),
                                                                  kFc1In / h->fc_splits, md);
      if ((rc = check_launch("fc1_slab_mask"))) return rc;
      mask = md;
      if (h->profiling) {
        if ((rc = count_slab_macs(h, md, tiles, R, st))) return rc;
        frac = 0.0;
      }
    }
    DeltaScope ds(h);
    if ((rc = run_fc(h, act6, nullptr, R, y_alt, st, h->c_rows, mask, frac))) return rc;
  }
  return EXPECTO_OK;
}

constexpr int kCalibWindows = 256;

int f16_col_scales(expecto_beluga* h, hipStream_t st) {
  const int np[7] = {npad_of(320), npad_of(480), npad_of(480), npad_of(640), npad_of(640), npad_of(kFc1Out),
                     npad_of(kNFeat)};
  for (int g = 0; g < 7; ++g) {
    col_scales<<<dim3((np[g] + 255) / 256), dim3(256), 0, st>>>(h->swd[g], np[g], h->sx[g], h->cs[g]);
    int rc = check_launch("col_scales");
    if (rc) return rc;
  }
  if (h->fkw) {
    col_scales<<<dim3((np[5] + 255) / 256), dim3(256), 0, st>>>(h->fk_sw, np[5], h->sx[5], h->fk_cs);
    return check_launch("col_scales (FC1 Karatsuba)");
  }
  return EXPECTO_OK;
}

int f16_calibrate(expecto_beluga* h, hipStream_t st) {
  const int nb = std::min(kCalibWindows, h->max_batch);
  int rc;
  if (!h->calib && (rc = dalloc(h, &h->calib, (size_t)nb * kNFeat + (size_t)nb * kLen / 4 + 64))) return rc;
  float* buf = h->calib;
  float* y = buf;
  uint8_t* codes = reinterpret_cast<uint8_t*>(buf + (size_t)nb * kNFeat);
  unsigned* amax = reinterpret_cast<unsigned*>(buf + (size_t)nb * kNFeat + (size_t)nb * kLen / 4);
  EXPECTO_HIP_CHECK(hipMemsetAsync(amax, 0, 8 * sizeof(unsigned), st));
  const long long nc = (long long)nb * kLen;
  calib_codes<<<dim3((unsigned)((nc + 255) / 256)), dim3(256), 0, st>>>(codes, nc, 0x5eed1234u);
  if ((rc = check_launch("calib_codes"))) return rc;
  const int saved = g_precision;
  const bool prof = h->profiling;
  h->profiling = false;
  g_precision = EXPECTO_PRECISION_BF16X6;
  auto amax_of = [&](const float* A, long long groups, int s_rows, int t_valid, int C, int b) {
    act_max<<<dim3(1024), dim3(256), 0, st>>>(A, groups, s_rows, t_valid, C, C, amax + b);
    return check_launch("act_max");
  };
  rc = run_conv1(h, nullptr, codes, kLen, nb, EXPECTO_STRAND_FWD, 0, nb, kLen, kS1, st);
  if (!rc) rc = amax_of(h->P, nb, kS1, kLen - 7, 320, 0);
  float* src = h->P;
  float* dst = h->Q;
  for (int l = 0; l < 5 && !rc; ++l) {
    const ConvGeo& g = kConv[l];
// ... 53 lines not shown
    split_planes_h2<<<dim3((unsigned)((n4 + 255) / 256)), dim3(256), 0, st>>>(
        y.w, y.rows, (int)y.K, h->swd[g], reinterpret_cast<_Float16*>(h->wh[g]));
    if ((rc = check_launch("split_planes_h2"))) return rc;
  }
  {
    float *w1r = nullptr, *sw1 = nullptr;
    if ((rc = dalloc(h, &w1r, 320 * 32)) || (rc = dalloc(h, &sw1, 320)) || (rc = dalloc(h, &h->cs1, 320)) ||
        (rc = dalloc(h, &h->w1h, 320 * 32)))
      return rc;
    repack_conv1<<<dim3(40), dim3(256), 0, st>>>(h->w1, w1r);
    row_scale_exp<<<dim3(320), dim3(256), 0, st>>>(w1r, 32, reinterpret_cast<int*>(sw1));
    split_planes_h2<<<dim3(10), dim3(256), 0, st>>>(w1r, 320, 32, reinterpret_cast<int*>(sw1),
                                                    reinterpret_cast<_Float16*>(h->w1h));
    col_scales<<<dim3(2), dim3(256), 0, st>>>(reinterpret_cast<int*>(sw1), 320, 0, h->cs1);
    if ((rc = check_launch("conv1 planes"))) return rc;
  }
  if (h->fk_on) {
    const int np1 = npad_of(kFc1Out);
    float* wk = nullptr;
    EXPECTO_HIP_CHECK(hipMalloc(&wk, (size_t)np1 * kFkKTotal * sizeof(float)));
    float *swf = nullptr;
    if ((rc = dalloc(h, &swf, np1)) || (rc = dalloc(h, &h->fk_cs, np1)) ||
        (rc = dalloc(h, &h->fkw, (size_t)np1 * kFkKTotal))) {
      (void)hipFree(wk);
      return rc;
    }
    h->fk_sw = reinterpret_cast<int*>(swf);
    const long long tot = (long long)np1 * kFkKTotal;
    fk_weights<<<dim3((unsigned)((tot + 255) / 256)), dim3(256), 0, st>>>(h->fc1w, np1, wk);
    row_scale_exp<<<dim3(np1), dim3(256), 0, st>>>(wk, (int)kFkKTotal, h->fk_sw);
    split_planes_h2<<<dim3((unsigned)((tot / 4 + 255) / 256)), dim3(256), 0, st>>>(
        wk, np1, (int)kFkKTotal, h->fk_sw, reinterpret_cast<_Float16*>(h->fkw));
    rc = check_launch("FC1 Karatsuba weights");
    (void)hipStreamSynchronize(st);
    (void)hipFree(wk);
    if (rc) return rc;
  }
  if ((rc = f16_calibrate(h, st))) return rc;
  h->f16_ready = true;
  return EXPECTO_OK;
}

__global__ void take_flags(const int* __restrict__ ovf, int* __restrict__ bad, int* __restrict__ out) {
  if (threadIdx.x != 0) return;
  if (ovf) out[0] = __hip_atomic_load(ovf, __ATOMIC_RELAXED, __HIP_MEMORY_SCOPE_AGENT);
  if (bad) {
    out[1] = __hip_atomic_load(bad, __ATOMIC_RELAXED, __HIP_MEMORY_SCOPE_AGENT);
    *bad = 0;
  }
}

template <class F>
int run_checked(expecto_beluga* h, hipStream_t st, F&& fn) {
  if (h->precision != EXPECTO_PRECISION_F16X3 || h->ovf_deferred) return fn();
  int rc = fn();
  if (rc) return rc;
  int* flag = h->hflags;
  take_flags<<<1, 64, 0, st>>>(h->ovf, nullptr, h->hflags_d);
  EXPECTO_HIP_CHECK(hipGetLastError());
  EXPECTO_HIP_CHECK(hipStreamSynchronize(st));
  if (!*flag) return EXPECTO_OK;
  EXPECTO_HIP_CHECK(hipMemsetAsync(h->ovf, 0, sizeof(int), st));
  h->fallbacks += 1;
  h->precision = EXPECTO_PRECISION_BF16X6;
  rc = fn();
  h->precision = EXPECTO_PRECISION_F16X3;
  return rc;
}
}

extern "C" {

int expecto_beluga_create(int device, const float* const* params, int max_batch, void* stream,
                          expecto_beluga_t* out) {
  EXPECTO_REQUIRE(out != nullptr && params != nullptr, "null argument");
  EXPECTO_REQUIRE(max_batch > 0 && max_batch <= (1 << 16), "max_batch out of range");
  for (int i = 0; i < EXPECTO_BELUGA_NPARAMS; ++i) EXPECTO_REQUIRE(params[i] != nullptr, "null parameter pointer");
  EXPECTO_HIP_CHECK(hipSetDevice(device));
  hipStream_t st = as_stream(stream);
  auto* h = new expecto_beluga();
  h->device = device;
  h->max_batch = max_batch;
  if (hipDeviceGetAttribute(&h->cus, hipDeviceAttributeMultiprocessorCount, device) != hipSuccess) h->cus = 0;
  int rc = 0;
  auto fail = [&](int code) {
    expecto_beluga_destroy(h);
    return code;
  };
  if ((rc = dalloc(h, &h->w1, 320 * 32)) || (rc = dalloc(h, &h->b1, 320))) return fail(rc);
  if (hipHostMalloc(&h->hflags, 4 * sizeof(int), hipHostMallocMapped) != hipSuccess ||
      hipHostGetDevicePointer(reinterpret_cast<void**>(&h->hflags_d), h->hflags, 0) != hipSuccess) {
    set_error("hipHostMalloc (flag words)");
    return fail(EXPECTO_ENOMEM);
  }
  EXPECTO_HIP_CHECK(hipMemcpyAsync(h->w1, params[0], 320 * 32 * sizeof(float), hipMemcpyDeviceToDevice, st));
  EXPECTO_HIP_CHECK(hipMemcpyAsync(h->b1, params[1], 320 * sizeof(float), hipMemcpyDeviceToDevice, st));
  for (int l = 0; l < 5; ++l) {
    const ConvGeo& g = kConv[l];
    const int np = npad_of(g.cout);
    const long long K = 8LL * g.cin;
    if ((rc = dalloc(h, &h->wt[l], (size_t)np * K)) || (rc = dalloc(h, &h->bt[l], np))) return fail(rc);
    const long long tot = np * K;
    repack_conv<<<dim3((unsigned)((tot + 255) / 256)), dim3(256), 0, st>>>(params[2 + 2 * l], g.cout, g.cin, np,
                                                                          h->wt[l]);
    pad_copy<<<dim3((np + 255) / 256), dim3(256), 0, st>>>(params[3 + 2 * l], g.cout, np, h->bt[l]);
    if ((rc = make_planes(h, h->wt[l], np, K, &h->wp[l], st))) return fail(rc);
  }
  const int np1 = npad_of(kFc1Out), np2 = npad_of(kNFeat);
  if ((rc = dalloc(h, &h->fc1w, (size_t)np1 * kFc1In)) || (rc = dalloc(h, &h->fc1b, np1)) ||
      (rc = dalloc(h, &h->fc2w, (size_t)np2 * kHidLd)) || (rc = dalloc(h, &h->fc2b, np2)))
    return fail(rc);
  {
    const long long tot = (long long)np1 * kFc1In;
    repack_fc1<<<dim3((unsigned)((tot + 255) / 256)), dim3(256), 0, st>>>(params[12], np1, h->fc1w);
    pad_copy<<<dim3((np1 + 255) / 256), dim3(256), 0, st>>>(params[13], kFc1Out, np1, h->fc1b);
    const long long tot2 = (long long)np2 * kHidLd;
    repack_fc2<<<dim3((unsigned)((tot2 + 255) / 256)), dim3(256), 0, st>>>(params[14], np2, h->fc2w);
    pad_copy<<<dim3((np2 + 255) / 256), dim3(256), 0, st>>>(params[15], kNFeat, np2, h->fc2b);
    if ((rc = make_planes(h, h->fc1w, np1, kFc1In, &h->fc1p, st)) ||
        (rc = make_planes(h, h->fc2w, np2, kHidLd, &h->fc2p, st)))
      return fail(rc);
  }
  if ((rc = check_launch("repack"))) return fail(rc);
  const size_t pf = p_floats(max_batch), qf = q_floats(max_batch);
  if (const char* e = getenv("EXPECTO_FC1_SPLITS")) {
    const int v = atoi(e);
    EXPECTO_REQUIRE(v >= 1 && v <= 32 && (kFc1In / GBK) % v == 0, "EXPECTO_FC1_SPLITS must divide 2120 and be <= 32");
    h->fc_splits = v;
  }
  if (const char* e = getenv("EXPECTO_FC2_SPLITS")) {
    const int v = atoi(e);
    EXPECTO_REQUIRE(v >= 1 && 63 % v == 0, "EXPECTO_FC2_SPLITS must divide 63");
    h->fc2_splits = v;
  }
  if (const char* e = getenv("EXPECTO_FC1_M_ORDER_MB")) h->fc1_m_order_mb = atof(e);
  if (const char* e = getenv("EXPECTO_FC1_ORDER")) h->fc1_order = atoi(e);
  if (const char* e = getenv("EXPECTO_FC1_M_GROUP")) h->fc1_m_group = std::max(1, atoi(e));
  if (const char* e = getenv("EXPECTO_FC_WIDE")) h->fc_wide = atoi(e) != 0;
  if (const char* e = getenv("EXPECTO_OVERLAP")) h->overlap = atoi(e) != 0;
  if (const char* e = getenv("EXPECTO_POOL_ONE_PASS")) h->pool_one_pass = atoi(e) != 0;
  if (const char* e = getenv("EXPECTO_POOL_FUSED")) h->pool_fused = atoi(e) != 0;
  if (const char* e = getenv("EXPECTO_FUSE_CONV1")) h->fuse_conv1 = atoi(e) != 0;
  if (const char* e = getenv("EXPECTO_CONV2_TABLE")) h->kmer_on = atoi(e) != 0;
  if (const char* e = getenv("EXPECTO_KMER_QUAD")) h->kmer_quad = atoi(e) != 0;
  if (const char* e = getenv("EXPECTO_ONEHOT_CODES")) h->onehot_as_codes = atoi(e) != 0;
  if (const char* e = getenv("EXPECTO_FC1_KARATSUBA")) h->fk_on = atoi(e) != 0;
  if (const char* e = getenv("EXPECTO_FC1K_SLICE")) h->fk_slice = std::max(1, atoi(e));
  if (const char* e = getenv("EXPECTO_FC1_ROLE")) {
    const int v = atoi(e);
    EXPECTO_REQUIRE(v >= 0 && v <= 4, "EXPECTO_FC1_ROLE must be 0..4");
    h->fk_role = v;
  }
  if (const char* e = getenv("EXPECTO_SEG_CHUNK_WINDOWS")) h->seg_chunk_windows = atoi(e);
  if (const char* e = getenv("EXPECTO_CONV_NARROW")) {
    const int v = atoi(e);
    EXPECTO_REQUIRE(v >= -1 && v <= 1, "EXPECTO_CONV_NARROW must be -1 (auto), 0 or 1");
    h->conv_narrow = v;
  }
  if (const char* e = getenv("EXPECTO_FC1_NARROW")) {
    const int v = atoi(e);
    EXPECTO_REQUIRE(v >= -1 && v <= 1, "EXPECTO_FC1_NARROW must be -1 (auto), 0 or 1");
    h->fc1_narrow = v;
  }
  if (const char* e = getenv("EXPECTO_CONV_EA")) h->conv_ea = atoi(e) != 0;
  if (const char* e = getenv("EXPECTO_FC_SKINNY")) h->fc_skinny = atoi(e) != 0;
  if (const char* e = getenv("EXPECTO_CONV_TILE")) {
    const int v = atoi(e);
    EXPECTO_REQUIRE(v == 0 || v == 256 || v == 384, "EXPECTO_CONV_TILE must be 0 (auto), 256 or 384");
    h->conv_tile = v;
  }
  h->fc2_rows = h->fc2_splits == 1 ? 4 * max_batch : max_batch;
  if (const char* e = getenv("EXPECTO_FC2_ROWS"))
    if (h->fc2_splits == 1) h->fc2_rows = std::max(max_batch, atoi(e));
  const size_t partf = (size_t)std::max(h->fc_splits, kFkParts) * max_batch * kHidLd;
  const size_t h1_rows = (size_t)h->fc2_rows + (h->fc2_splits == 1 ? max_batch : 0);
  if ((rc = dalloc(h, &h->P, act_alloc(pf))) || (rc = dalloc(h, &h->Q, act_alloc(qf))) ||
      (rc = dalloc(h, &h->part, partf)) || (rc = dalloc(h, &h->h1, act_alloc(h1_rows * kHidLd))) ||
      (rc = dalloc(h, &h->part2, (size_t)h->fc2_splits * max_batch * kHidLd)))
    return fail(rc);
  {
    float* rows = nullptr;
    if ((rc = dalloc(h, &rows, (size_t)(max_batch + h1_rows) * 2))) return fail(rc);
    h->a_rows = reinterpret_cast<long long*>(rows);
    h->c_rows = h->a_rows + max_batch;
  }
  EXPECTO_HIP_CHECK(hipMemsetAsync(h->P, 0, act_alloc(pf) * sizeof(float), st));
  EXPECTO_HIP_CHECK(hipMemsetAsync(h->Q, 0, act_alloc(qf) * sizeof(float), st));
  if ((rc = f16_prepare(h, st))) return fail(rc);
  if (h->kmer_on && (rc = kmer_acquire(h, params, st))) return fail(rc);
  h->precision = EXPECTO_PRECISION_F16X3;
  EXPECTO_HIP_CHECK(hipStreamSynchronize(st));
  *out = h;
  return EXPECTO_OK;
}

void expecto_beluga_destroy(expecto_beluga_t h) {
  if (!h) return;
  kmer_release(h);
  if (h->win_seg_d) (void)hipFree(h->win_seg_d);
  if (h->alt_w_d) (void)hipFree(h->alt_w_d);
  if (h->copy_w_d) (void)hipFree(h->copy_w_d);
  if (h->fc_perm_d) (void)hipFree(h->fc_perm_d);
  if (h->seg_var_d) (void)hipFree(h->seg_var_d);
  if (h->win_off_d) (void)hipFree(h->win_off_d);
  if (h->win_row_d) (void)hipFree(h->win_row_d);
  for (float* p : h->fk_seq)
    if (p) (void)hipFree(p);
  for (float* p : h->fk_aseq)
    if (p) (void)hipFree(p);
  if (h->fk_gres) (void)hipFree(h->fk_gres);
  if (h->seam) (void)hipFree(h->seam);
  if (h->edge) (void)hipFree(h->edge);
  for (void* p : h->allocs) (void)hipFree(p);
  for (hipEvent_t e : h->ev_pool) (void)hipEventDestroy(e);
  for (hipEvent_t e : h->pev)
    if (e) (void)hipEventDestroy(e);
  if (h->st2) (void)hipStreamDestroy(h->st2);
  for (int s = 0; s < 2; ++s) {
    if (h->stage_ev[s]) (void)hipEventSynchronize(h->stage_ev[s]);
    if (h->stage_buf[s]) (void)hipHostFree(h->stage_buf[s]);
    if (h->stage_ev[s]) (void)hipEventDestroy(h->stage_ev[s]);
  }
  if (h->hflags) (void)hipHostFree(h->hflags);
  delete h;
}

size_t expecto_beluga_device_bytes(expecto_beluga_t h) {
  return h ? h->bytes + kmer_reported_bytes(h) : 0;
}

int expecto_beluga_conv2_table_active(expecto_beluga_t h, int* reason) {
  EXPECTO_REQUIRE(h != nullptr, "null handle");
  if (reason) *reason = h->kmer_state;
  return h->kmer ? 1 : 0;
}

int expecto_beluga_set_fc1_role(expecto_beluga_t h, int role) {
  EXPECTO_REQUIRE(h != nullptr, "null handle");
  EXPECTO_REQUIRE(role >= 0 && role <= 4, "FC1 role must be 0..4");
  h->fk_role = role;
  return EXPECTO_OK;
}

int expecto_beluga_forward_onehot(expecto_beluga_t h, const float* x, int n, float* y, void* stream) {
  EXPECTO_REQUIRE(h != nullptr, "null handle");
  EXPECTO_REQUIRE(n >= 0, "negative batch");
  if (n == 0) return EXPECTO_OK;
  EXPECTO_REQUIRE(x != nullptr && y != nullptr, "null input/output");
  EXPECTO_HIP_CHECK(hipSetDevice(h->device));
  hipStream_t st = as_stream(stream);
  const bool candidate = h->onehot_as_codes && h->kmer && (reinterpret_cast<uintptr_t>(x) & 15) == 0 &&
                         (h->precision == EXPECTO_PRECISION_F16X3 || h->precision == EXPECTO_PRECISION_BF16X6);
  if (candidate && !h->oh_codes) {
    float *c = nullptr, *f = nullptr;
    int rc;
    if ((rc = dalloc(h, &c, ((size_t)h->max_batch * kLen + 3) / 4)) || (rc = dalloc(h, &f, 1))) return rc;
    h->oh_codes = reinterpret_cast<uint8_t*>(c);
    h->oh_bad = reinterpret_cast<int*>(f);
  }
  auto run = [&](bool as_codes, int* bad) {
    for (long long r0 = 0; r0 < n; r0 += h->max_batch) {
      const int nb = (int)std::min<long long>(h->max_batch, n - r0);
      int rc;
      if (as_codes) {
        {
          LayerTimer lt(h, 0, st);
          const long long q = (long long)nb * (kLen / 4);
          onehot_codes<<<dim3((unsigned)((q + 255) / 256)), dim3(256), 0, st>>>(x + r0 * 4 * kLen, nb, kLen,
                                                                              h->oh_codes, bad);
          if ((rc = check_launch("onehot_codes"))) return rc;
        }
        rc = forward_chunk(h, nullptr, h->oh_codes, kLen, nb, EXPECTO_STRAND_FWD, 0, nb, y + r0 * kNFeat, st);
      } else {
        rc = forward_chunk(h, x, nullptr, 0, 0, 0, r0, nb, y + r0 * kNFeat, st);
      }
      if (rc) return rc;
    }
    return (int)EXPECTO_OK;
  };
  if (candidate && h->precision == EXPECTO_PRECISION_F16X3 && !h->ovf_deferred && !h->oh_hint_bad) {
    int rc = run(true, h->oh_bad);
    if (rc) return rc;
    int* flags = h->hflags;
    take_flags<<<1, 64, 0, st>>>(h->ovf, h->oh_bad, h->hflags_d);
    EXPECTO_HIP_CHECK(hipGetLastError());
    EXPECTO_HIP_CHECK(hipStreamSynchronize(st));
    if (flags[1]) {
      h->oh_hint_bad = true;
      EXPECTO_HIP_CHECK(hipMemsetAsync(h->ovf, 0, sizeof(int), st));
      return run_checked(h, st, [&]() { return run(false, nullptr); });
    }
    if (!flags[0]) return EXPECTO_OK;
    EXPECTO_HIP_CHECK(hipMemsetAsync(h->ovf, 0, sizeof(int), st));
    h->fallbacks += 1;
    h->precision = EXPECTO_PRECISION_BF16X6;
    rc = run(true, nullptr);
    h->precision = EXPECTO_PRECISION_F16X3;
    return rc;
  }
  bool as_codes = false;
  if (candidate) {
    int bad = 0;
    {
      LayerTimer lt(h, 0, st);
      EXPECTO_HIP_CHECK(hipMemsetAsync(h->oh_bad, 0, sizeof(int), st));
      const long long q = (long long)n * (kLen / 4);
      onehot_codes<<<dim3((unsigned)((q + 255) / 256)), dim3(256), 0, st>>>(x, n, kLen, nullptr, h->oh_bad);
      int rc = check_launch("onehot_codes check");
      if (rc) return rc;
    }
    take_flags<<<1, 64, 0, st>>>(nullptr, h->oh_bad, h->hflags_d);
    EXPECTO_HIP_CHECK(hipGetLastError());
    EXPECTO_HIP_CHECK(hipStreamSynchronize(st));
    bad = h->hflags[1];
    as_codes = bad == 0;
    h->oh_hint_bad = !as_codes;
  }
  return run_checked(h, st, [&]() { return run(as_codes, nullptr); });
}

int expecto_beluga_forward_codes(expecto_beluga_t h, const uint8_t* codes, int n, long long code_stride,
                                 int strand_mode, float* y, void* stream) {
  EXPECTO_REQUIRE(h != nullptr, "null handle");
  EXPECTO_REQUIRE(n >= 0, "negative batch");
  EXPECTO_REQUIRE(strand_mode >= 0 && strand_mode <= 2, "bad strand mode");
  if (n == 0) return EXPECTO_OK;
  EXPECTO_REQUIRE(codes != nullptr && y != nullptr, "null input/output");
  EXPECTO_REQUIRE(code_stride >= kLen, "code_stride < 2000");
  EXPECTO_HIP_CHECK(hipSetDevice(h->device));
  hipStream_t st = as_stream(stream);
  const long long rows = strand_mode == EXPECTO_STRAND_BOTH ? 2LL * n : n;
  return run_checked(h, st, [&]() {
    for (long long r0 = 0; r0 < rows; r0 += h->max_batch) {
      const int nb = (int)std::min<long long>(h->max_batch, rows - r0);
      int rc = forward_chunk(h, nullptr, codes, code_stride, n, strand_mode, r0, nb, y + r0 * kNFeat, st);
      if (rc) return rc;
    }
    return (int)EXPECTO_OK;
  });
}

int expecto_beluga_forward_segments(expecto_beluga_t h, const uint8_t* codes, int n_seg, int seg_len,
                                    long long code_stride, int strand_mode, const int* win_seg, const int* win_off,
                                    const int* win_row, int n_win, float* y, void* stream) {
  EXPECTO_REQUIRE(h != nullptr, "null handle");
  EXPECTO_REQUIRE(n_seg >= 0 && n_win >= 0, "negative count");
  EXPECTO_REQUIRE(strand_mode >= 0 && strand_mode <= 2, "bad strand mode");
  if (n_win == 0 || n_seg == 0) return EXPECTO_OK;
  EXPECTO_REQUIRE(codes && y && win_seg && win_off, "null argument");
  EXPECTO_REQUIRE(code_stride >= seg_len, "code_stride < seg_len");
  EXPECTO_HIP_CHECK(hipSetDevice(h->device));
  hipStream_t st = as_stream(stream);
  return run_checked(h, st, [&]() {
    return forward_segments(h, codes, n_seg, seg_len, code_stride, strand_mode, win_seg, win_off, win_row, n_win, y,
                            st);
  });
}

int expecto_beluga_forward_segment_pairs(expecto_beluga_t h, const uint8_t* codes, const int* var_pos,
                                         const uint8_t* alt_code, int n_seg, int seg_len, long long code_stride,
                                         int strand_mode, const int* win_seg, const int* win_off, const int* win_row,
                                         int n_win, float* y_ref, float* y_alt, long long strand_stride,
                                         void* stream) {
// ... 170 lines not shown
```

Before: 1532.

## Merge forward and reverse-complement strands into one segment chunk loop

Folds the forward and reverse-complement strands into a single virtual entry space, so segments and windows of both strands can share one chunk. Kernels now take a SegStrands descriptor and work out strand, row offset and complement per element instead of being launched once per strand. This is meant to halve the number of chunk iterations and launches and to make the fc1/fc2 GEMM batches larger. It also moves fk_gres to a fixed per-batch allocation, and it brings more index arithmetic and a larger restructuring risk.

Measured after the change: 1558, median of 6. 1.02x the previous value.

```diff
diff --git a/expecto_amd/csrc/beluga.hip b/expecto_amd/csrc/beluga.hip
--- a/expecto_amd/csrc/beluga.hip
+++ b/expecto_amd/csrc/beluga.hip
@@ -394,18 +394,24 @@
   }
 }
 
+struct SegStrands {
+  int n_seg, rc_ent, n_win, rc_win;
+  long long rc_rows;
+};
+
 __global__ void seg_a_rows(const int* __restrict__ win_seg, const int* __restrict__ win_off,
                            const int* __restrict__ win_row, const int* __restrict__ widx, int w0, int m_count,
-                           int seg_base, int rc, int seg_len, int n_ph, int4 ph_idx, int s7, long long row_base,
+                           int ent_base, SegStrands ss, int seg_len, int n_ph, int4 ph_idx, int s7,
                            long long* __restrict__ a_rows, long long* __restrict__ c_rows) {
   const int m = blockIdx.x * blockDim.x + threadIdx.x;
   if (m >= m_count) return;
-  const int w = widx ? widx[m] : w0 + m;
-  c_rows[m] = row_base + (win_row ? win_row[w] : w);
-  const int o = rc ? seg_len - 2000 - win_off[w] : win_off[w];
+  const int v = widx ? widx[m] : w0 + m;
+  const int sd = v >= ss.n_win ? 1 : 0, w = v - sd * ss.n_win;
+  c_rows[m] = sd * ss.rc_rows + (win_row ? win_row[w] : w);
+  const int o = v >= ss.rc_win ? seg_len - 2000 - win_off[w] : win_off[w];
   const int q = o >> 2, p = q & 3, off6 = (q - p) >> 2;
   const int pi = p == 0 ? ph_idx.x : p == 1 ? ph_idx.y : p == 2 ? ph_idx.z : ph_idx.w;
-  const long long blk = (long long)(win_seg[w] - seg_base) * n_ph + pi;
+  const long long blk = (long long)(win_seg[w] + sd * ss.n_seg - ent_base) * n_ph + pi;
   a_rows[m] = (blk * s7 + off6) * 640;
 }
 
@@ -517,12 +523,13 @@
   int L, T1, P1, T3, T4, S5, T5, T6;
 };
 
-__global__ void seg_delta_table(const int* __restrict__ var_pos, int s0, int ns, int rc, SegDims g, int n_ph, int4 ph,
-                                int* __restrict__ tab) {
+__global__ void seg_delta_table(const int* __restrict__ var_pos, int e0, int ns, SegStrands ss, SegDims g, int n_ph,
+                                int4 ph, int* __restrict__ tab) {
   const int m = blockIdx.x * blockDim.x + threadIdx.x;
   if (m >= ns) return;
-  int q = min(max(var_pos[s0 + m], 0), g.L - 1);
-  if (rc) q = g.L - 1 - q;
+  const int e = e0 + m;
+  int q = min(max(var_pos[e >= ss.n_seg ? e - ss.n_seg : e], 0), g.L - 1);
+  if (e >= ss.rc_ent) q = g.L - 1 - q;
   int* t = tab + m * kSegTab;
   const int r1 = clampi(q - 7, 0, g.T1 - kDW[1]);
   const int r2 = clampi(floor4(r1 - 7), 0, g.P1 - kDW[2]);
@@ -544,26 +551,32 @@
 }
 
 __global__ void seg_delta_codes(const uint8_t* __restrict__ codes, long long stride, const uint8_t* __restrict__ alt_code,
-                                int s0, int ns, int rc, int L, const int* __restrict__ tab, uint8_t* __restrict__ out) {
+                                int e0, int ns, SegStrands ss, int L, const int* __restrict__ tab,
+                                uint8_t* __restrict__ out) {
   const int i = threadIdx.x & 15;
   const int m = blockIdx.x * (blockDim.x >> 4) + (threadIdx.x >> 4);
   if (m >= ns) return;
+  const int e = e0 + m, sg = e >= ss.n_seg ? e - ss.n_seg : e;
+  const bool rc = e >= ss.rc_ent;
   const int q = tab[m * kSegTab], x = min(tab[m * kSegTab + 1] + i, L - 1);
-  uint8_t c = x == q ? alt_code[s0 + m] : codes[(long long)(s0 + m) * stride + (rc ? L - 1 - x : x)];
+  uint8_t c = x == q ? alt_code[sg] : codes[(long long)sg * stride + (rc ? L - 1 - x : x)];
   if (rc && c < 4) c = (uint8_t)(3 - c);
   out[(long long)m * 16 + i] = c;
 }
 
 constexpr int kC1Pat = kDA[2] + 7, kC1PatStride = 48;
 __global__ void seg_delta_codes2(const uint8_t* __restrict__ codes, long long stride, const uint8_t* __restrict__ alt_code,
-                                 int s0, int ns, int rc, int L, const int* __restrict__ tab, uint8_t* __restrict__ out) {
+                                 int e0, int ns, SegStrands ss, int L, const int* __restrict__ tab,
+                                 uint8_t* __restrict__ out) {
   const int i = threadIdx.x % kC1PatStride;
   const int m = blockIdx.x * (blockDim.x / kC1PatStride) + threadIdx.x / kC1PatStride;
   if (m >= ns) return;
+  const int e = e0 + m, sg = e >= ss.n_seg ? e - ss.n_seg : e;
+  const bool rc = e >= ss.rc_ent;
   const int q = tab[m * kSegTab], x = 4 * tab[m * kSegTab + 2] + i;
   uint8_t c = 4;
   if (i < kC1Pat && x < L) {
-    c = x == q ? alt_code[s0 + m] : codes[(long long)(s0 + m) * stride + (rc ? L - 1 - x : x)];
+    c = x == q ? alt_code[sg] : codes[(long long)sg * stride + (rc ? L - 1 - x : x)];
     if (rc && c < 4) c = (uint8_t)(3 - c);
   }
   out[(long long)m * kC1PatStride + i] = c;
@@ -687,15 +700,17 @@
 }
 
 __global__ void fc1_slab_mask_seg(const int* __restrict__ widx, int n_alt, const int* __restrict__ win_seg,
-                                  const int* __restrict__ win_off, int seg_base, int rc, int seg_len, int4 ph_idx,
-                                  const int* __restrict__ tab, int tile_rows, int slab_k, unsigned* __restrict__ mask) {
+                                  const int* __restrict__ win_off, int ent_base, SegStrands ss, int seg_len,
+                                  int4 ph_idx, const int* __restrict__ tab, int tile_rows, int slab_k,
+                                  unsigned* __restrict__ mask) {
   const int m = blockIdx.x * blockDim.x + threadIdx.x;
   if (m >= n_alt) return;
-  const int w = widx[m];
-  const int o = rc ? seg_len - 2000 - win_off[w] : win_off[w];
+  const int v = widx[m];
+  const int sd = v >= ss.n_win ? 1 : 0, w = v - sd * ss.n_win;
+  const int o = v >= ss.rc_win ? seg_len - 2000 - win_off[w] : win_off[w];
   const int q = o >> 2, p = q & 3, off6 = (q - p) >> 2;
   const int pi = p == 0 ? ph_idx.x : p == 1 ? ph_idx.y : p == 2 ? ph_idx.z : ph_idx.w;
-  const int r6 = tab[(win_seg[w] - seg_base) * kSegTab + 13 + pi];
+  const int r6 = tab[(win_seg[w] + sd * ss.n_seg - ent_base) * kSegTab + 13 + pi];
   const int lo = max(r6 - off6, 0), hi = min(r6 + kDW[6] - off6, 106);
   if (lo >= hi) return;
   unsigned bits = 0;
@@ -704,9 +719,10 @@
 }
 
 __global__ void copy_rows(const float* __restrict__ src, float* __restrict__ dst, const int* __restrict__ widx,
-                          const int* __restrict__ win_row, long long row_base) {
-  const int w = widx[blockIdx.x];
-  const long long r = (row_base + (win_row ? win_row[w] : w)) * kNFeat;
+                          const int* __restrict__ win_row, int n_win, long long rc_rows) {
+  const int v = widx[blockIdx.x];
+  const int sd = v >= n_win ? 1 : 0, w = v - sd * n_win;
+  const long long r = (sd * rc_rows + (win_row ? win_row[w] : w)) * kNFeat;
   for (int i = threadIdx.x; i < kNFeat; i += blockDim.x) dst[r + i] = src[r + i];
 }
 
@@ -1350,6 +1366,7 @@
   int conv_narrow = -1;
   bool narrow_scope = false;
   int seg_chunk_windows = 0;
+  bool seg_merge_strands = true;
   int cus = 0;
   bool pool_one_pass = true;
   bool pool_fused = true;
@@ -1379,7 +1396,6 @@
   long long* fk_arows = nullptr;
   long long* fk_crows = nullptr;
   int* fk_gres = nullptr;
-  long long fk_gres_cap = 0;
   float* fk_aseq[3] = {};
   long long fk_aseq_rows = 0;
   int* fk_rgrp = nullptr;
@@ -2084,6 +2100,7 @@
 bool fk_use_seg(const expecto_beluga* h) { return h->fk_on && h->fkw && g_precision == EXPECTO_PRECISION_F16X3; }
 
 int fk_cap(const expecto_beluga* h) { return std::max(h->max_batch, h->fk_slice); }
+constexpr int kGresPerBatch = 3;
 
 int fk_tables(expecto_beluga* h) {
   if (h->fk_grows) return EXPECTO_OK;
@@ -2274,10 +2291,10 @@
   int w, blk, off6;
 };
 int fk_role_of(int off6) { return (off6 / 25) & 3; }
-FkWin fk_win(int w, const int* win_seg, const int* win_off, int s0, bool rc, int L, int n_ph, const int* ph_idx) {
-  const int o = rc ? L - kLen - win_off[w] : win_off[w];
+FkWin fk_win(int w, int seg, int off, bool rc, int L, int n_ph, const int* ph_idx) {
+  const int o = rc ? L - kLen - off : off;
   const int q = o >> 2, p = q & 3;
-  return {w, (win_seg[w] - s0) * n_ph + ph_idx[p], (q - p) >> 2};
+  return {w, seg * n_ph + ph_idx[p], (q - p) >> 2};
 }
 bool fk_same_group(const FkWin& a, const FkWin& b) {
   return a.blk == b.blk && a.off6 - 25 * fk_role_of(a.off6) == b.off6 - 25 * fk_role_of(b.off6);
@@ -2490,19 +2507,29 @@
       *b = nullptr;
     }
     h->win_cap = 0;
-    for (int** b : {&h->win_seg_d, &h->win_off_d, &h->win_row_d, &h->alt_w_d, &h->copy_w_d})
-      EXPECTO_HIP_CHECK(hipMalloc(b, n_win * sizeof(int)));
+    for (int** b : {&h->win_seg_d, &h->win_off_d, &h->win_row_d}) EXPECTO_HIP_CHECK(hipMalloc(b, n_win * sizeof(int)));
+    for (int** b : {&h->alt_w_d, &h->copy_w_d}) EXPECTO_HIP_CHECK(hipMalloc(b, 2 * n_win * sizeof(int)));
     EXPECTO_HIP_CHECK(hipMalloc(&h->fc_perm_d, 4 * n_win * sizeof(int)));
     h->win_cap = n_win;
   }
+  const int strands = mode == EXPECTO_STRAND_BOTH ? 2 : 1;
+  const int n_ent = strands * n_seg, n_vw = strands * n_win;
+  const SegStrands ss{n_seg, mode == EXPECTO_STRAND_FWD ? n_ent : mode == EXPECTO_STRAND_RC ? 0 : n_seg,
+                      n_win, mode == EXPECTO_STRAND_FWD ? n_vw : mode == EXPECTO_STRAND_RC ? 0 : n_win,
+                      pr ? pr->strand_stride : n_win};
+  auto vw_w = [&](int v) { return v >= n_win ? v - n_win : v; };
+  std::vector<int> vfirst(n_ent + 1, n_vw);
+  for (int e = 0; e < n_ent; ++e) vfirst[e] = e >= n_seg ? n_win + first[e - n_seg] : first[e];
+  std::vector<char> is_alt(n_win, 0);
   std::vector<int> alt_w, copy_w;
   if (pr) {
     for (int sg = 0; sg < n_seg; ++sg)
       EXPECTO_REQUIRE(pr->var_pos[sg] >= 0 && pr->var_pos[sg] < L, "variant position outside its segment");
     for (int w = 0; w < n_win; ++w) {
       const int q = pr->var_pos[win_seg[w]];
-      (win_off[w] <= q && q < win_off[w] + kLen ? alt_w : copy_w).push_back(w);
-    }
+      is_alt[w] = win_off[w] <= q && q < win_off[w] + kLen;
+    }
+    for (int v = 0; v < n_vw; ++v) (is_alt[vw_w(v)] ? alt_w : copy_w).push_back(v);
     if (n_seg > h->seg_var_cap) {
       if (h->seg_var_d) EXPECTO_HIP_CHECK(hipFree(h->seg_var_d));
       h->seg_var_d = nullptr;
@@ -2523,458 +2550,436 @@
   }
   copies.push_back({h->win_seg_d, win_seg, n_win * sizeof(int)});
   copies.push_back({h->win_off_d, win_off, n_win * sizeof(int)});
-  const int strands = mode == EXPECTO_STRAND_BOTH ? 2 : 1;
   const int blk_per_seg = pr ? std::max(n_ph, 1) : 0;
   std::vector<std::pair<int, int>> chunks;
-  for (int s0 = 0; s0 < n_seg;) {
-    int s1 = s0 + 1;
-    while (s1 < n_seg && s1 - s0 < seg_cap && (long long)(s1 + 1 - s0) * blk_per_seg <= h->max_batch &&
-           (h->seg_chunk_windows <= 0 || first[s1 + 1] - first[s0] <= h->seg_chunk_windows))
-      ++s1;
-    chunks.push_back({s0, s1});
-    s0 = s1;
+  for (int e0 = 0; e0 < n_ent;) {
+    int e1 = e0 + 1;
+    while (e1 < n_ent && (e1 != n_seg || h->seg_merge_strands) && e1 - e0 < seg_cap &&
+           (long long)(e1 + 1 - e0) * blk_per_seg <= h->max_batch &&
+           (h->seg_chunk_windows <= 0 || vfirst[e1 + 1] - vfirst[e0] <= h->seg_chunk_windows))
+      ++e1;
+    chunks.push_back({e0, e1});
+    e0 = e1;
   }
   std::vector<int> fc_perm;
   if (pr) {
-    fc_perm.resize((size_t)strands * n_win);
-    std::vector<char> is_alt(n_win, 0);
-    for (int w : alt_w) is_alt[w] = 1;
-    for (int sd = 0; sd < strands; ++sd) {
-      const bool rcs = (mode == EXPECTO_STRAND_RC) || sd == 1;
-      int* out = fc_perm.data() + (size_t)sd * n_win;
-      for (const auto& c : chunks) {
-        const int w0 = first[c.first], w1 = first[c.second];
-        int k = w0;
-        std::vector<int> a;
-        for (int w = w0; w < w1; ++w)
-          if (is_alt[w]) a.push_back(w);
-        std::stable_sort(a.begin(), a.end(), [&](int x, int y) {
-          const int px = pr->var_pos[win_seg[x]] - win_off[x], py = pr->var_pos[win_seg[y]] - win_off[y];
-          return rcs ? px > py : px < py;
-        });
-        for (int w : a) out[k++] = w;
-        for (int w = w0; w < w1; ++w)
-          if (!is_alt[w]) out[k++] = w;
-      }
+    fc_perm.resize((size_t)n_vw);
+    auto pos_of = [&](int v) {
+      const int w = vw_w(v), p = pr->var_pos[win_seg[w]] - win_off[w];
+      return v >= ss.rc_win ? kLen - 1 - p : p;
+    };
+    for (const auto& c : chunks) {
+      const int w0 = vfirst[c.first], w1 = vfirst[c.second];
+      int k = w0;
+      std::vector<int> a;
+      for (int v = w0; v < w1; ++v)
+        if (is_alt[vw_w(v)]) a.push_back(v);
+      std::stable_sort(a.begin(), a.end(), [&](int x, int y) { return pos_of(x) < pos_of(y); });
+      for (int v : a) fc_perm[k++] = v;
+      for (int v = w0; v < w1; ++v)
+        if (!is_alt[vw_w(v)]) fc_perm[k++] = v;
     }
     copies.push_back({h->fc_perm_d, fc_perm.data(), fc_perm.size() * sizeof(int)});
   }
-  const bool fkm = fk_use_seg(h) && !(pr && 3 * alt_w.size() > (size_t)n_win);
+  const bool fkm = fk_use_seg(h) && !(pr && 3 * alt_w.size() > (size_t)n_vw);
   std::vector<std::vector<FkWin>> fk_ref, fk_alt;
-  std::vector<char> fk_is_alt(pr ? n_win : 0, 0);
-  for (int w : alt_w) fk_is_alt[w] = 1;
+  auto fk_is_alt = [&](int v) { return is_alt[vw_w(v)] != 0; };
   if (fkm) {
     fc_perm.assign((size_t)4 * n_win, 0);
-    for (int sd = 0; sd < strands; ++sd) {
-      const bool rcs = (mode == EXPECTO_STRAND_RC) || sd == 1;
-      for (const auto& c : chunks) {
-        const int w0 = first[c.first], w1 = first[c.second];
-        struct Key {
-          int cls;
-          long long rel;
-          int blk, G, off6, w;
-        };
-        std::vector<FkWin> ref, alt;
-        std::vector<Key> key;
-        std::map<std::pair<int, int>, int> galt;
-        for (int w = w0; w < w1; ++w) {
-          const FkWin fw = fk_win(w, win_seg, win_off, c.first, rcs, L, n_ph, ph_idx);
-          ref.push_back(fw);
-          if (pr && fk_is_alt[w]) {
-            alt.push_back(fw);
-            galt[{fw.blk, fw.off6 - 25 * fk_role_of(fw.off6)}] = 1;
-          }
+    for (const auto& c : chunks) {
+      const int w0 = vfirst[c.first], w1 = vfirst[c.second];
+      struct Key {
+        int cls;
+        long long rel;
+        int blk, G, off6, w;
+      };
+      std::vector<FkWin> ref, alt;
+      std::vector<Key> key;
+      std::map<std::pair<int, int>, int> galt;
+      for (int v = w0; v < w1; ++v) {
+        const int w = vw_w(v);
+        const FkWin fw = fk_win(v, win_seg[w] + (v >= n_win ? n_seg : 0) - c.first, win_off[w], v >= ss.rc_win, L, n_ph,
+                                ph_idx);
+        ref.push_back(fw);
+        if (pr && fk_is_alt(v)) {
+          alt.push_back(fw);
+          galt[{fw.blk, fw.off6 - 25 * fk_role_of(fw.off6)}] = 1;
         }
-        for (const FkWin& fw : ref) {
-          const int G = fw.off6 - 25 * fk_role_of(fw.off6);
-          const bool ga = pr && galt.count({fw.blk, G});
-          long long rel = 0;
-          if (ga) {
-            const int q = pr->var_pos[win_seg[fw.w]];
-            rel = (long long)(rcs ? L - 1 - q : q) - 16LL * G;
-          }
-          key.push_back({ga ? 0 : 1, rel, fw.blk, G, fw.off6, fw.w});
+      }
+      for (const FkWin& fw : ref) {
+        const int G = fw.off6 - 25 * fk_role_of(fw.off6);
+        const bool ga = pr && galt.count({fw.blk, G});
+        long long rel = 0;
+        if (ga) {
+          const int q = pr->var_pos[win_seg[vw_w(fw.w)]];
+          rel = (long long)(fw.w >= ss.rc_win ? L - 1 - q : q) - 16LL * G;
         }
-        std::vector<int> ord(ref.size());
-        for (size_t k = 0; k < ord.size(); ++k) ord[k] = (int)k;
-        std::sort(ord.begin(), ord.end(), [&](int a, int b) {
-          const Key &x = key[a], &y = key[b];
-          return std::tie(x.cls, x.rel, x.blk, x.G, x.off6, x.w) < std::tie(y.cls, y.rel, y.blk, y.G, y.off6, y.w);
-        });
-        std::vector<FkWin> sorted;
-        for (int k : ord) sorted.push_back(ref[k]);
-        for (size_t k = 0; k < sorted.size(); ++k) fc_perm[(size_t)sd * n_win + w0 + k] = sorted[k].w;
-        fk_ref.push_back(std::move(sorted));
-        fk_alt.push_back(std::move(alt));
+        key.push_back({ga ? 0 : 1, rel, fw.blk, G, fw.off6, fw.w});
       }
+      std::vector<int> ord(ref.size());
+      for (size_t k = 0; k < ord.size(); ++k) ord[k] = (int)k;
+      std::sort(ord.begin(), ord.end(), [&](int a, int b) {
+        const Key &x = key[a], &y = key[b];
+        return std::tie(x.cls, x.rel, x.blk, x.G, x.off6, x.w) < std::tie(y.cls, y.rel, y.blk, y.G, y.off6, y.w);
+      });
+      std::vector<FkWin> sorted;
+      for (int k : ord) sorted.push_back(ref[k]);
+      for (size_t k = 0; k < sorted.size(); ++k) fc_perm[(size_t)w0 + k] = sorted[k].w;
+      fk_ref.push_back(std::move(sorted));
+      fk_alt.push_back(std::move(alt));
     }
     if (pr) copies.pop_back();
     copies.push_back({h->fc_perm_d, fc_perm.data(), fc_perm.size() * sizeof(int)});
   }
   if ((rc = stage_copies(h, copies, st))) return rc;
-  const long long strand_rows = pr ? pr->strand_stride : n_win;
   const int eb = act_bytes();
   hipStream_t sa = (pr && h->st2) ? h->st2 : st;
   const SegDims gd{L, g.T1, g.P1, g.T3, g.T4, g.S5, g.T5, g.T6};
   const int4 ph4 = make_int4(ph[0], ph[1], ph[2], ph[3]);
-  for (int sd = 0; sd < strands; ++sd) {
-    const bool is_rc = (mode == EXPECTO_STRAND_RC) || sd == 1;
-    for (const auto& chunk : chunks) {
-      const int s0 = chunk.first, s1 = chunk.second;
-      const int w0 = first[s0], nw = first[s1] - first[s0];
-      const int ns = s1 - s0;
-      const long long nb = (long long)ns * n_ph;
-      auto alt_asm = [&](int l, const float* ref, int ref_rows, const float* dprev, int wprev, int nbk, int ib,
-                         int mult, int irp, int arows, hipEvent_t ready, hipEvent_t done) -> int {
-        if (sa != st) {
-          EXPECTO_HIP_CHECK(hipEventRecord(ready, st));
-          EXPECTO_HIP_CHECK(hipStreamWaitEvent(sa, ready, 0));
+  for (const auto& chunk : chunks) {
+    const int s0 = chunk.first, s1 = chunk.second;
+    const int w0 = vfirst[s0], nw = vfirst[s1] - vfirst[s0];
+    const int ns = s1 - s0;
+    const long long nb = (long long)ns * n_ph;
+    auto alt_asm = [&](int l, const float* ref, int ref_rows, const float* dprev, int wprev, int nbk, int ib,
+                       int mult, int irp, int arows, hipEvent_t ready, hipEvent_t done) -> int {
+      if (sa != st) {
+        EXPECTO_HIP_CHECK(hipEventRecord(ready, st));
+        EXPECTO_HIP_CHECK(hipStreamWaitEvent(sa, ready, 0));
+      }
+      const int row16 = kConv[l].cin * eb / 16;
+      seg_delta_assemble<<<dim3(ns * nbk), dim3(256), 0, sa>>>(ref, ref_rows, dprev, wprev, h->seg_tab, nbk,
+                                                                    ib, mult, irp, arows, row16, h->DA);
+      int r = check_launch("seg_delta_assemble");
+      if (!r && sa != st) EXPECTO_HIP_CHECK(hipEventRecord(done, sa));
+      return r;
+    };
+    auto alt_gemm = [&](int l, int nbk, int arows, int w, bool pool, float* dnext) -> int {
+      DeltaScope ds(h);
+      return run_conv(h, l, h->DA, dnext, (long long)ns * nbk, arows, w, w, pool, sa);
+    };
+    auto st_wait = [&](hipEvent_t e) -> int {
+      if (sa != st) EXPECTO_HIP_CHECK(hipStreamWaitEvent(st, e, 0));
+      return EXPECTO_OK;
+    };
+    if (pr && sa != st) {
+      EXPECTO_HIP_CHECK(hipEventRecord(h->pev[0], st));
+      EXPECTO_HIP_CHECK(hipStreamWaitEvent(sa, h->pev[0], 0));
+    }
+    const bool kmer = use_kmer(h, nullptr);
+    const bool fuse = !kmer && fuse_conv1(h, nullptr);
+    const C1Src f1{codes, code_stride, n_seg, mode, s0, L};
+    if (!kmer && !fuse && (rc = run_conv1(h, nullptr, codes, code_stride, n_seg, mode, s0, ns, L, g.S1, st)))
+      return rc;
+    if (pr) {
+      seg_delta_table<<<dim3((ns + 255) / 256), dim3(256), 0, sa>>>(h->seg_var_d, s0, ns, ss, gd, n_ph, ph4,
+                                                                   h->seg_tab);
+      if ((rc = check_launch("seg_delta_table"))) return rc;
+      if (kmer || fuse) {
+        seg_delta_codes2<<<dim3((ns + 4) / 5), dim3(5 * kC1PatStride), 0, sa>>>(
+            codes, code_stride, pr->alt_code, s0, ns, ss, L, h->seg_tab, h->delta_codes);
+        if ((rc = check_launch("seg_delta_codes2"))) return rc;
+        DeltaScope ds(h);
+        if (fuse && (rc = run_conv1(h, nullptr, h->delta_codes, kC1PatStride, ns, EXPECTO_STRAND_FWD, 0, ns, kC1Pat,
+                                    kDA[2], sa, h->DA)))
+          return rc;
+      } else {
+        seg_delta_codes<<<dim3((ns + 15) / 16), dim3(256), 0, sa>>>(codes, code_stride, pr->alt_code, s0, ns, ss,
+                                                                   L, h->seg_tab, h->delta_codes);
+        if ((rc = check_launch("seg_delta_codes"))) return rc;
+        DeltaScope ds(h);
+        if ((rc = run_conv1(h, nullptr, h->delta_codes, 16, ns, EXPECTO_STRAND_FWD, 0, ns, kDA[1], kDW[1], sa,
+                            h->D0)))
+          return rc;
+      }
+    }
+    if (pr && !kmer && !fuse && (rc = alt_asm(0, h->P, g.S1, h->D0, kDW[1], 1, 2, 4, 1, kDA[2], h->pev[1], h->pev[2])))
+      return rc;
+    if (kmer)
+      rc = run_conv2_kmer(h, f1, ns, g.P1, g.P1, h->Q, st);
+    else
+      rc = run_conv(h, 0, h->P, h->Q, ns, g.S1, g.P1, g.P1, true, st, fuse ? &f1 : nullptr);
+    if (rc) return rc;
+    if (pr && kmer) {
+      DeltaScope ds(h);
+      const C1Src fa{h->delta_codes, kC1PatStride, ns, EXPECTO_STRAND_FWD, 0, kC1Pat};
+      if ((rc = run_conv2_kmer(h, fa, ns, kDW[2], kDW[2], h->D1, sa))) return rc;
+    } else if (pr && ((!fuse && (rc = st_wait(h->pev[2]))) || (rc = alt_gemm(0, 1, kDA[2], kDW[2], true, h->D1)))) {
+      return rc;
+    }
+    if (pr && (rc = alt_asm(1, h->Q, g.P1, h->D1, kDW[2], 1, 3, 1, 2, kDA[3], h->pev[3], h->pev[4]))) return rc;
+    const int T3p = (g.T3 + 3) & ~3;
+    if ((rc = run_conv(h, 1, h->Q, h->P, ns, g.P1, g.T3, T3p, false, st))) return rc;
+    if (pr && ((rc = st_wait(h->pev[4])) || (rc = alt_gemm(1, 1, kDA[3], kDW[3], false, h->D0)))) return rc;
+    if (pr && (rc = alt_asm(2, h->P, T3p, h->D0, kDW[3], 1, 4, 1, 3, kA4u, h->pev[5], h->pev[6]))) return rc;
+    const bool pfused = conv4_pool_fused(h, (long long)ns * T3p, n_ph, ph);
+    struct PQSwap {
+      expecto_beluga* h;
+      bool on;
+      ~PQSwap() {
+        if (on) std::swap(h->P, h->Q);
+      }
+    } pq{h, false};
+    if (pfused) {
+      if ((rc = run_conv4_pool_fused(h, h->P, h->Q, ns, T3p, g.T4, g.S5, pr ? h->seg_tab : nullptr, st))) return rc;
+      std::swap(h->P, h->Q);
+      pq.on = true;
+    } else if ((rc = run_conv(h, 2, h->P, h->Q, ns, T3p, g.T4, g.T4, false, st))) {
+      return rc;
+    }
+    if (pr && ((rc = st_wait(h->pev[6])) || (rc = alt_gemm(2, 1, kA4u, kW4u, false, h->D1)))) return rc;
+    if (!pfused) {
+      LayerTimer lt(h, 3, st);
+      if (act_fmt() == 2 && h->pool_one_pass) {
+        dim3 grid((g.S5 + 3) / 4, ns);
+        pool4_phases_h2m<<<grid, dim3(256), 0, st>>>(h->Q, g.T4, g.T4, 480, n_ph, ph4, g.S5, h->P);
+      } else if (act_fmt() == 2) {
+        dim3 grid((g.S5 + 3) / 4, ns * n_ph);
+        pool4_phases_h2<<<grid, dim3(256), 0, st>>>(h->Q, g.T4, g.T4, 480, n_ph, ph4, g.S5, h->P);
+      } else {
+        dim3 grid(g.S5, ns * n_ph);
+        pool4_phases<<<grid, dim3(480), 0, st>>>(h->Q, ns, g.T4, g.T4, 480, n_ph, ph4, g.S5, h->P, act_fmt());
+      }
+      if ((rc = check_launch("pool4_phases"))) return rc;
+    }
+    if (pr) {
+      if (sa != st) {
+        EXPECTO_HIP_CHECK(hipEventRecord(h->pev[7], st));
+        EXPECTO_HIP_CHECK(hipStreamWaitEvent(sa, h->pev[7], 0));
+      }
+      seg_delta_pool<<<dim3(kDW[4], (unsigned)nb), dim3(480), 0, sa>>>(pfused ? h->edge : h->Q, g.T4, h->D1, n_ph,
+                                                                       ph4, h->seg_tab, act_fmt(), h->D0,
+                                                                       pfused ? 1 : 0);
+      if ((rc = check_launch("seg_delta_pool"))) return rc;
+      if (sa != st) EXPECTO_HIP_CHECK(hipEventRecord(h->pev[8], sa));
+      if ((rc = alt_asm(3, h->P, g.S5, h->D0, kDW[4], n_ph, 9, 1, 5, kDA[5], h->pev[9], h->pev[10]))) return rc;
+      if ((rc = st_wait(h->pev[8]))) return rc;
+    }
+    if ((rc = run_conv(h, 3, h->P, h->Q, nb, g.S5, g.T5, g.T5, false, st))) return rc;
+    if (pr && ((rc = st_wait(h->pev[10])) || (rc = alt_gemm(3, n_ph, kDA[5], kDW[5], false, h->D1)))) return rc;
+    if (pr && (rc = alt_asm(4, h->Q, g.T5, h->D1, kDW[5], n_ph, 13, 1, 9, kDA[6], h->pev[11], h->pev[12])))
+      return rc;
+    if ((rc = run_conv(h, 4, h->Q, h->P, nb, g.T5, g.T6, g.T6, false, st))) return rc;
+    if (pr) {
+      if ((rc = alt_gemm(4, n_ph, kDA[6], kDW[6], false, h->D0))) return rc;
+      if (sa != st) EXPECTO_HIP_CHECK(hipEventRecord(h->pev[13], sa));
+    }
+    if (nw > 0 && fkm) {
+      const int4 phi = make_int4(ph_idx[0], ph_idx[1], ph_idx[2], ph_idx[3]);
+      const size_t ci = (size_t)(&chunk - chunks.data());
+      const long long cap = fk_cap(h);
+      const std::vector<FkWin>& ws = fk_ref[ci];
+      const int* perm = h->fc_perm_d + w0;
+      std::vector<int> gres((size_t)nb, -2);
+      for (const FkWin& w : ws) {
+        const int r = (w.off6 - 25 * fk_role_of(w.off6)) % 100;
+        int& e = gres[(size_t)w.blk];
+        e = e == -2 ? r : (e == r ? r : -1);
+      }
+      EXPECTO_REQUIRE(nb <= kGresPerBatch * (long long)h->max_batch, "conv6 blocks of a chunk exceed fk_gres");
+      if ((rc = stage_copies(h, {{h->fk_gres, gres.data(), gres.size() * sizeof(int)}}, st)) || (rc = fk_tables(h)) ||
+          (rc = fk_seg_buffers(h)) || (rc = fk_sequences(h, h->P, nb, g.T6, g.T6, nullptr, n_ph, st, h->fk_gres)))
+        return rc;
+      const bool has_alt = pr && !fk_alt[ci].empty();
+      bool alt_ready = false;
+      for (size_t i0 = 0; i0 < ws.size();) {
+        size_t i1 = i0;
+        while (i1 < ws.size()) {
+          size_t j = i1 + 1;
+          while (j < ws.size() && fk_same_group(ws[j], ws[i1])) ++j;
+          if (j - i0 > (size_t)cap && i1 > i0) break;
+          i1 = j;
         }
-        const int row16 = kConv[l].cin * eb / 16;
-        seg_delta_assemble<<<dim3(ns * nbk), dim3(256), 0, sa>>>(ref, ref_rows, dprev, wprev, h->seg_tab, nbk,
-                                                                      ib, mult, irp, arows, row16, h->DA);
-        int r = check_launch("seg_delta_assemble");
-        if (!r && sa != st) EXPECTO_HIP_CHECK(hipEventRecord(done, sa));
-        return r;
-      };
-      auto alt_gemm = [&](int l, int nbk, int arows, int w, bool pool, float* dnext) -> int {
-        DeltaScope ds(h);
-        return run_conv(h, l, h->DA, dnext, (long long)ns * nbk, arows, w, w, pool, sa);
-      };
-      auto st_wait = [&](hipEvent_t e) -> int {
-        if (sa != st) EXPECTO_HIP_CHECK(hipStreamWaitEvent(st, e, 0));
-        return EXPECTO_OK;
-      };
-      if (pr && sa != st) {
-        EXPECTO_HIP_CHECK(hipEventRecord(h->pev[0], st));
-        EXPECTO_HIP_CHECK(hipStreamWaitEvent(sa, h->pev[0], 0));
-      }
-      const bool kmer = use_kmer(h, nullptr);
-      const bool fuse = !kmer && fuse_conv1(h, nullptr);
-      const C1Src f1{codes + (long long)s0 * code_stride, code_stride, ns, is_rc ? EXPECTO_STRAND_RC : EXPECTO_STRAND_FWD,
-                     0, L};
-      if (!kmer && !fuse && (rc = run_conv1(h, nullptr, f1.codes, code_stride, ns, f1.mode, 0, ns, L, g.S1, st)))
-        return rc;
-      if (pr) {
-        seg_delta_table<<<dim3((ns + 255) / 256), dim3(256), 0, sa>>>(h->seg_var_d, s0, ns, is_rc ? 1 : 0, gd, n_ph,
-                                                                     ph4, h->seg_tab);
-        if ((rc = check_launch("seg_delta_table"))) return rc;
-        if (kmer || fuse) {
-          seg_delta_codes2<<<dim3((ns + 4) / 5), dim3(5 * kC1PatStride), 0, sa>>>(
-              codes, code_stride, pr->alt_code, s0, ns, is_rc ? 1 : 0, L, h->seg_tab, h->delta_codes);
-          if ((rc = check_launch("seg_delta_codes2"))) return rc;
-          DeltaScope ds(h);
-          if (fuse && (rc = run_conv1(h, nullptr, h->delta_codes, kC1PatStride, ns, EXPECTO_STRAND_FWD, 0, ns, kC1Pat,
-                                      kDA[2], sa, h->DA)))
+        EXPECTO_REQUIRE(i1 - i0 <= (size_t)cap, "a Karatsuba FC1 window group exceeds the FC1 slice");
+        const int fn = (int)(i1 - i0);
+        std::vector<long long> grows;
+        std::vector<int> prow, rgrp, ginfo;
+        FkProducts prd{h->fk_grows, {}, {}, {}};
+        fk_slice_tables(ws, (int)i0, (int)i1, g.T6, grows, prd, prow, &rgrp, &ginfo);
+        if ((rc = stage_copies(h, {{h->fk_grows, grows.data(), grows.size() * sizeof(long long)},
+                                   {h->fk_prow, prow.data(), prow.size() * sizeof(int)}}, st)))
+          return rc;
+        seg_a_rows<<<dim3((fn + 255) / 256), dim3(256), 0, st>>>(
+            h->win_seg_d, h->win_off_d, win_row ? h->win_row_d : nullptr, perm + i0, 0, fn, s0, ss, L, n_ph, phi,
+            g.T6, h->fk_arows, h->fk_crows);
+        if ((rc = check_launch("seg_a_rows")) ||
+            (rc = fk_fc1(h, h->P, h->fk_seq, prd, h->fk_arows, fn, h->fk_prow, h->fk_h1, st, nullptr, 0, h->fk_part,
+                         kFkParts * cap)))
+          return rc;
+        for (int r0 = 0; r0 < fn; r0 += h->max_batch)
+          if ((rc = run_fc2(h, h->fk_h1 + (long long)r0 * kHidLd, std::min(h->max_batch, fn - r0), y, st,
+                            h->fk_crows + r0)))
             return rc;
-        } else {
-          seg_delta_codes<<<dim3((ns + 15) / 16), dim3(256), 0, sa>>>(codes, code_stride, pr->alt_code, s0, ns,
-                                                                     is_rc ? 1 : 0, L, h->seg_tab, h->delta_codes);
-          if ((rc = check_launch("seg_delta_codes"))) return rc;
-          DeltaScope ds(h);
-          if ((rc = run_conv1(h, nullptr, h->delta_codes, 16, ns, EXPECTO_STRAND_FWD, 0, ns, kDA[1], kDW[1], sa,
-                              h->D0)))
-            return rc;
+        int n_ag = 0;
+        size_t nw_pre = 0;
+        for (size_t i = i0; has_alt && i < i1; ++i) {
+          bool galt = false;
+          size_t j = i;
+          for (; j < i1 && fk_same_group(ws[j], ws[i]); ++j) galt |= fk_is_alt(ws[j].w);
+          if (!galt) break;
+          ++n_ag;
+          nw_pre = j - i0;
+          i = j - 1;
         }
-      }
-      if (pr && !kmer && !fuse && (rc = alt_asm(0, h->P, g.S1, h->D0, kDW[1], 1, 2, 4, 1, kDA[2], h->pev[1], h->pev[2])))
-        return rc;
-      if (kmer)
-        rc = run_conv2_kmer(h, f1, ns, g.P1, g.P1, h->Q, st);
-      else
-        rc = run_conv(h, 0, h->P, h->Q, ns, g.S1, g.P1, g.P1, true, st, fuse ? &f1 : nullptr);
-      if (rc) return rc;
-      if (pr && kmer) {
-        DeltaScope ds(h);
-        const C1Src fa{h->delta_codes, kC1PatStride, ns, EXPECTO_STRAND_FWD, 0, kC1Pat};
-        if ((rc = run_conv2_kmer(h, fa, ns, kDW[2], kDW[2], h->D1, sa))) return rc;
-      } else if (pr && ((!fuse && (rc = st_wait(h->pev[2]))) || (rc = alt_gemm(0, 1, kDA[2], kDW[2], true, h->D1)))) {
-        return rc;
-      }
-      if (pr && (rc = alt_asm(1, h->Q, g.P1, h->D1, kDW[2], 1, 3, 1, 2, kDA[3], h->pev[3], h->pev[4]))) return rc;
-      const int T3p = (g.T3 + 3) & ~3;
-      if ((rc = run_conv(h, 1, h->Q, h->P, ns, g.P1, g.T3, T3p, false, st))) return rc;
-      if (pr && ((rc = st_wait(h->pev[4])) || (rc = alt_gemm(1, 1, kDA[3], kDW[3], false, h->D0)))) return rc;
-      if (pr && (rc = alt_asm(2, h->P, T3p, h->D0, kDW[3], 1, 4, 1, 3, kA4u, h->pev[5], h->pev[6]))) return rc;
-      const bool pfused = conv4_pool_fused(h, (long long)ns * T3p, n_ph, ph);
-      struct PQSwap {
-        expecto_beluga* h;
-        bool on;
-        ~PQSwap() {
-          if (on) std::swap(h->P, h->Q);
-        }
-      } pq{h, false};
-      if (pfused) {
-        if ((rc = run_conv4_pool_fused(h, h->P, h->Q, ns, T3p, g.T4, g.S5, pr ? h->seg_tab : nullptr, st))) return rc;
-        std::swap(h->P, h->Q);
-        pq.on = true;
-      } else if ((rc = run_conv(h, 2, h->P, h->Q, ns, T3p, g.T4, g.T4, false, st))) {
-        return rc;
-      }
-      if (pr && ((rc = st_wait(h->pev[6])) || (rc = alt_gemm(2, 1, kA4u, kW4u, false, h->D1)))) return rc;
-      if (!pfused) {
-        LayerTimer lt(h, 3, st);
-        if (act_fmt() == 2 && h->pool_one_pass) {
-          dim3 grid((g.S5 + 3) / 4, ns);
-          pool4_phases_h2m<<<grid, dim3(256), 0, st>>>(h->Q, g.T4, g.T4, 480, n_ph, ph4, g.S5, h->P);
-        } else if (act_fmt() == 2) {
-          dim3 grid((g.S5 + 3) / 4, ns * n_ph);
-          pool4_phases_h2<<<grid, dim3(256), 0, st>>>(h->Q, g.T4, g.T4, 480, n_ph, ph4, g.S5, h->P);
-        } else {
-          dim3 grid(g.S5, ns * n_ph);
-          pool4_phases<<<grid, dim3(480), 0, st>>>(h->Q, ns, g.T4, g.T4, 480, n_ph, ph4, g.S5, h->P, act_fmt());
-        }
-        if ((rc = check_launch("pool4_phases"))) return rc;
-      }
-      if (pr) {
-        if (sa != st) {
-          EXPECTO_HIP_CHECK(hipEventRecord(h->pev[7], st));
-          EXPECTO_HIP_CHECK(hipStreamWaitEvent(sa, h->pev[7], 0));
-        }
-        seg_delta_pool<<<dim3(kDW[4], (unsigned)nb), dim3(480), 0, sa>>>(pfused ? h->edge : h->Q, g.T4, h->D1, n_ph,
-                                                                         ph4, h->seg_tab, act_fmt(), h->D0,
-                                                                         pfused ? 1 : 0);
-        if ((rc = check_launch("seg_delta_pool"))) return rc;
-        if (sa != st) EXPECTO_HIP_CHECK(hipEventRecord(h->pev[8], sa));
-        if ((rc = alt_asm(3, h->P, g.S5, h->D0, kDW[4], n_ph, 9, 1, 5, kDA[5], h->pev[9], h->pev[10]))) return rc;
-        if ((rc = st_wait(h->pev[8]))) return rc;
-      }
-      if ((rc = run_conv(h, 3, h->P, h->Q, nb, g.S5, g.T5, g.T5, false, st))) return rc;
-      if (pr && ((rc = st_wait(h->pev[10])) || (rc = alt_gemm(3, n_ph, kDA[5], kDW[5], false, h->D1)))) return rc;
-      if (pr && (rc = alt_asm(4, h->Q, g.T5, h->D1, kDW[5], n_ph, 13, 1, 9, kDA[6], h->pev[11], h->pev[12])))
-        return rc;
-      if ((rc = run_conv(h, 4, h->Q, h->P, nb, g.T5, g.T6, g.T6, false, st))) return rc;
-      if (pr) {
-        if ((rc = alt_gemm(4, n_ph, kDA[6], kDW[6], false, h->D0))) return rc;
-        if (sa != st) EXPECTO_HIP_CHECK(hipEventRecord(h->pev[13], sa));
-      }
-      if (nw > 0 && fkm) {
-        const int4 phi = make_int4(ph_idx[0], ph_idx[1], ph_idx[2], ph_idx[3]);
-        const long long row_base = (long long)sd * strand_rows;
-        const size_t ci = (size_t)sd * chunks.size() + (size_t)(&chunk - chunks.data());
-        const long long cap = fk_cap(h);
-        const std::vector<FkWin>& ws = fk_ref[ci];
-        const int* perm = h->fc_perm_d + (size_t)sd * n_win + w0;
-        std::vector<int> gres((size_t)nb, -2);
-        for (const FkWin& w : ws) {
-          const int r = (w.off6 - 25 * fk_role_of(w.off6)) % 100;
-          int& e = gres[(size_t)w.blk];
-          e = e == -2 ? r : (e == r ? r : -1);
-        }
-        if (nb > h->fk_gres_cap) {
-          if (h->fk_gres) EXPECTO_HIP_CHECK(hipFree(h->fk_gres));
-          h->fk_gres = nullptr;
-          h->bytes -= (size_t)h->fk_gres_cap * sizeof(int);
-          h->fk_gres_cap = 0;
-          EXPECTO_HIP_CHECK(hipMalloc(&h->fk_gres, (size_t)nb * sizeof(int)));
-          h->fk_gres_cap = nb;
-          h->bytes += (size_t)nb * sizeof(int);
-        }
-        if ((rc = stage_copies(h, {{h->fk_gres, gres.data(), gres.size() * sizeof(int)}}, st)) || (rc = fk_tables(h)) ||
-            (rc = fk_seg_buffers(h)) || (rc = fk_sequences(h, h->P, nb, g.T6, g.T6, nullptr, n_ph, st, h->fk_gres)))
-          return rc;
-        const bool has_alt = pr && !fk_alt[ci].empty();
-        bool alt_ready = false;
-        for (size_t i0 = 0; i0 < ws.size();) {
-          size_t i1 = i0;
-          while (i1 < ws.size()) {
-            size_t j = i1 + 1;
-            while (j < ws.size() && fk_same_group(ws[j], ws[i1])) ++j;
-            if (j - i0 > (size_t)cap && i1 > i0) break;
-            i1 = j;
-          }
-          EXPECTO_REQUIRE(i1 - i0 <= (size_t)cap, "a Karatsuba FC1 window group exceeds the FC1 slice");
-          const int fn = (int)(i1 - i0);
-          std::vector<long long> grows;
-          std::vector<int> prow, rgrp, ginfo;
-          FkProducts prd{h->fk_grows, {}, {}, {}};
-          fk_slice_tables(ws, (int)i0, (int)i1, g.T6, grows, prd, prow, &rgrp, &ginfo);
-          if ((rc = stage_copies(h, {{h->fk_grows, grows.data(), grows.size() * sizeof(long long)},
-                                     {h->fk_prow, prow.data(), prow.size() * sizeof(int)}}, st)))
-            return rc;
-          seg_a_rows<<<dim3((fn + 255) / 256), dim3(256), 0, st>>>(
-              h->win_seg_d, h->win_off_d, win_row ? h->win_row_d : nullptr, perm + i0, 0, fn, s0, is_rc ? 1 : 0, L,
-              n_ph, phi, g.T6, row_base, h->fk_arows, h->fk_crows);
-          if ((rc = check_launch("seg_a_rows")) ||
-              (rc = fk_fc1(h, h->P, h->fk_seq, prd, h->fk_arows, fn, h->fk_prow, h->fk_h1, st, nullptr, 0, h->fk_part,
-                           kFkParts * cap)))
-            return rc;
-          for (int r0 = 0; r0 < fn; r0 += h->max_batch)
-            if ((rc = run_fc2(h, h->fk_h1 + (long long)r0 * kHidLd, std::min(h->max_batch, fn - r0), y, st,
-                              h->fk_crows + r0)))
-              return rc;
-          int n_ag = 0;
-          size_t nw_pre = 0;
-          for (size_t i = i0; has_alt && i < i1; ++i) {
-            bool galt = false;
-            size_t j = i;
-            for (; j < i1 && fk_same_group(ws[j], ws[i]); ++j) galt |= fk_is_alt[ws[j].w] != 0;
-            if (!galt) break;
-            ++n_ag;
-            nw_pre = j - i0;
-            i = j - 1;
-          }
-          if (n_ag > 0) {
-            FkProducts pa = prd;
-            FkMaskDesc md{};
-            for (int gq = 0; gq < 9; ++gq) {
-              int c = 0;
-              for (int i = 0; i < prd.cnt[gq]; ++i)
-                if (rgrp[prd.off[gq] + i] < n_ag) ++c;
-              pa.cnt[gq] = c;
-              pa.lay[gq] = prd.cnt[gq];
-              for (int sb = 0; prd.cnt[gq] > 0 && sb < kFkSlabs; ++sb) {
-                md.g[md.n] = gq;
-                md.s[md.n] = sb;
-                md.off[md.n] = prd.off[gq];
-                md.cnt[md.n] = c;
-                ++md.n;
-              }
-            }
-            md.nw = (int)nw_pre;
-            std::vector<int> winfo, aperm, aprow;
-            for (size_t i = 0; i < nw_pre; ++i) {
-              winfo.push_back(ws[i0 + i].blk);
-              winfo.push_back(ws[i0 + i].off6);
-              if (fk_is_alt[ws[i0 + i].w]) {
-                aperm.push_back(ws[i0 + i].w);
-                aprow.insert(aprow.end(), prow.begin() + (long long)i * kFkParts, prow.begin() + (long long)(i + 1) * kFkParts);
-              }
-            }
-            const int na = (int)aperm.size();
-            const int tiles = (int)(cap / 256 + 1);
-            if ((rc = stage_copies(h, {{h->fk_rgrp, rgrp.data(), rgrp.size() * sizeof(int)},
-                                       {h->fk_ginfo, ginfo.data(), ginfo.size() * sizeof(int)},
-                                       {h->fk_winfo, winfo.data(), winfo.size() * sizeof(int)},
-                                       {h->fk_aperm, aperm.data(), aperm.size() * sizeof(int)},
-                                       {h->fk_aprow, aprow.data(), aprow.size() * sizeof(int)}}, st)))
-              return rc;
-            if (!alt_ready) {
-              if ((rc = st_wait(h->pev[13]))) return rc;
-              seg_alt_blocks<<<dim3(kAltRows6, (unsigned)nb), dim3(64), 0, st>>>(h->P, h->D0, n_ph, g.T6, h->seg_tab,
-                                                                                640 * eb / 16, h->Q);
-              if ((rc = check_launch("seg_alt_blocks"))) return rc;
-              DeltaScope ds(h);
-              if ((rc = fk_sequences(h, h->Q, nb, g.T6, g.T6, h->seg_tab, n_ph, st, h->fk_gres, 1))) return rc;
-              alt_ready = true;
-            }
-            EXPECTO_HIP_CHECK(hipMemsetAsync(h->fk_smask, 0, (size_t)(md.n + 1) * tiles * sizeof(unsigned), st));
-            int rows_max = md.nw;
-            for (int i = 0; i < md.n; ++i) rows_max = std::max(rows_max, md.cnt[i]);
-            if (rows_max > 0) {
-              fk_seg_mask<<<dim3((rows_max + 255) / 256, md.n + 1), dim3(256), 0, st>>>(
-                  md, h->fk_rgrp, h->fk_ginfo, h->fk_winfo, h->seg_tab, n_ph, make_int4(0, 0, 0, 0), tiles, h->fk_smask);
-              if ((rc = check_launch("fk_seg_mask"))) return rc;
-            }
-            DeltaScope ds(h);
-            if ((rc = fk_fc1(h, h->Q, h->fk_aseq, pa, h->fk_arows, (int)nw_pre, nullptr, h->fk_h1, st, h->fk_smask, tiles,
-                             h->fk_part, kFkParts * cap)) ||
-                (na > 0 && (rc = fk_reduce(h, h->fk_part, h->fk_aprow, na, h->fk_h1, st))))
-              return rc;
-            if (na > 0) {
-              seg_a_rows<<<dim3((na + 255) / 256), dim3(256), 0, st>>>(
-                  h->win_seg_d, h->win_off_d, win_row ? h->win_row_d : nullptr, h->fk_aperm, 0, na, s0, is_rc ? 1 : 0,
-                  L, n_ph, phi, g.T6, row_base, h->fk_arows, h->fk_crows);
-              if ((rc = check_launch("seg_a_rows"))) return rc;
-              for (int r0 = 0; r0 < na; r0 += h->max_batch)
-                if ((rc = run_fc2(h, h->fk_h1 + (long long)r0 * kHidLd, std::min(h->max_batch, na - r0), pr->y_alt, st,
-                                  h->fk_crows + r0)))
-                  return rc;
+        if (n_ag > 0) {
+          FkProducts pa = prd;
+          FkMaskDesc md{};
+          for (int gq = 0; gq < 9; ++gq) {
+            int c = 0;
+            for (int i = 0; i < prd.cnt[gq]; ++i)
+              if (rgrp[prd.off[gq] + i] < n_ag) ++c;
+            pa.cnt[gq] = c;
+            pa.lay[gq] = prd.cnt[gq];
+            for (int sb = 0; prd.cnt[gq] > 0 && sb < kFkSlabs; ++sb) {
+              md.g[md.n] = gq;
+              md.s[md.n] = sb;
+              md.off[md.n] = prd.off[gq];
+              md.cnt[md.n] = c;
+              ++md.n;
             }
           }
-          i0 = i1;
-        }
-        if (pr) {
-          const int ic0 = (int)(std::lower_bound(copy_w.begin(), copy_w.end(), w0) - copy_w.begin());
-          const int ic1 = (int)(std::lower_bound(copy_w.begin(), copy_w.end(), w0 + nw) - copy_w.begin());
-          if (ic1 > ic0) {
-            copy_rows<<<dim3(ic1 - ic0), dim3(256), 0, st>>>(y, pr->y_alt, h->copy_w_d + ic0,
-                                                             win_row ? h->win_row_d : nullptr, row_base);
-            if ((rc = check_launch("copy_rows"))) return rc;
+          md.nw = (int)nw_pre;
+          std::vector<int> winfo, aperm, aprow;
+          for (size_t i = 0; i < nw_pre; ++i) {
+            winfo.push_back(ws[i0 + i].blk);
+            winfo.push_back(ws[i0 + i].off6);
+            if (fk_is_alt(ws[i0 + i].w)) {
+              aperm.push_back(ws[i0 + i].w);
+              aprow.insert(aprow.end(), prow.begin() + (long long)i * kFkParts, prow.begin() + (long long)(i + 1) * kFkParts);
+            }
           }
-        }
-      } else if (nw > 0) {
-        const int4 phi = make_int4(ph_idx[0], ph_idx[1], ph_idx[2], ph_idx[3]);
-        const long long row_base = (long long)sd * strand_rows;
-        const int* widx = pr ? h->fc_perm_d + (size_t)sd * n_win + w0 : nullptr;
-        int n_alt = 0, ic0 = 0, ic1 = 0;
-        if (pr) {
-          n_alt = (int)(std::lower_bound(alt_w.begin(), alt_w.end(), w0 + nw) -
-                        std::lower_bound(alt_w.begin(), alt_w.end(), w0));
-          ic0 = (int)(std::lower_bound(copy_w.begin(), copy_w.end(), w0) - copy_w.begin());
-          ic1 = (int)(std::lower_bound(copy_w.begin(), copy_w.end(), w0 + nw) - copy_w.begin());
-        }
-        const bool gather2 = h->fc2_splits == 1;
-        int pend = 0;
-        auto flush2 = [&]() -> int {
-          const int n2 = pend;
-          pend = 0;
-          return n2 ? run_fc2(h, h->h1, n2, y, st, h->c_rows) : EXPECTO_OK;
-        };
-        for (int f0 = 0; f0 < nw; f0 += h->max_batch) {
-          const int fn = std::min(h->max_batch, nw - f0);
-          if (gather2 && pend + fn > h->fc2_rows && (rc = flush2())) return rc;
-          long long* crow = h->c_rows + (gather2 ? pend : 0);
-          seg_a_rows<<<dim3((fn + 255) / 256), dim3(256), 0, st>>>(
-              h->win_seg_d, h->win_off_d, win_row ? h->win_row_d : nullptr, widx ? widx + f0 : nullptr, w0 + f0,
-              fn, s0, is_rc ? 1 : 0, L, n_ph, phi, g.T6, row_base, h->a_rows, crow);
-          if ((rc = check_launch("seg_a_rows"))) return rc;
-          if (gather2) {
-            if ((rc = run_fc1(h, h->P, h->a_rows, fn, h1_rows(h, pend), st))) return rc;
-            pend += fn;
-          } else if ((rc = run_fc(h, h->P, h->a_rows, fn, y, st, h->c_rows))) {
+          const int na = (int)aperm.size();
+          const int tiles = (int)(cap / 256 + 1);
+          if ((rc = stage_copies(h, {{h->fk_rgrp, rgrp.data(), rgrp.size() * sizeof(int)},
+                                     {h->fk_ginfo, ginfo.data(), ginfo.size() * sizeof(int)},
+                                     {h->fk_winfo, winfo.data(), winfo.size() * sizeof(int)},
+                                     {h->fk_aperm, aperm.data(), aperm.size() * sizeof(int)},
+                                     {h->fk_aprow, aprow.data(), aprow.size() * sizeof(int)}}, st)))
             return rc;
-          }
-          const int na = std::min(n_alt - f0, fn);
-          if (na <= 0) continue;
-          if (f0 == 0) {
+          if (!alt_ready) {
             if ((rc = st_wait(h->pev[13]))) return rc;
             seg_alt_blocks<<<dim3(kAltRows6, (unsigned)nb), dim3(64), 0, st>>>(h->P, h->D0, n_ph, g.T6, h->seg_tab,
                                                                               640 * eb / 16, h->Q);
             if ((rc = check_launch("seg_alt_blocks"))) return rc;
+            DeltaScope ds(h);
+            if ((rc = fk_sequences(h, h->Q, nb, g.T6, g.T6, h->seg_tab, n_ph, st, h->fk_gres, 1))) return rc;
+            alt_ready = true;
           }
-          long long* acrow = gather2 ? h->c_rows + h->fc2_rows : h->c_rows;
-          seg_a_rows<<<dim3((na + 255) / 256), dim3(256), 0, st>>>(
-              h->win_seg_d, h->win_off_d, win_row ? h->win_row_d : nullptr, widx + f0, 0, na, s0, is_rc ? 1 : 0,
-              L, n_ph, phi, g.T6, row_base, h->a_rows, acrow);
-          if ((rc = check_launch("seg_a_rows"))) return rc;
-          const unsigned* mask = nullptr;
-          double frac = 1.0;
-          if (planes_gemm()) {
-            const int tiles = (int)((na + gemm_bm() - 1) / gemm_bm());
-            unsigned* md = reinterpret_cast<unsigned*>(h->slab_mask);
-            EXPECTO_HIP_CHECK(hipMemsetAsync(md, 0, tiles * sizeof(unsigned), st));
-            fc1_slab_mask_seg<<<dim3((na + 255) / 256), dim3(256), 0, st>>>(
-                widx + f0, na, h->win_seg_d, h->win_off_d, s0, is_rc ? 1 : 0, L, phi, h->seg_tab, (int)gemm_bm(),
-                kFc1In / h->fc_splits, md);
-            if ((rc = check_launch("fc1_slab_mask_seg"))) return rc;
-            mask = md;
-            if (h->profiling) {
-              if ((rc = count_slab_macs(h, md, tiles, na, st))) return rc;
-              frac = 0.0;
-            }
+          EXPECTO_HIP_CHECK(hipMemsetAsync(h->fk_smask, 0, (size_t)(md.n + 1) * tiles * sizeof(unsigned), st));
+          int rows_max = md.nw;
+          for (int i = 0; i < md.n; ++i) rows_max = std::max(rows_max, md.cnt[i]);
+          if (rows_max > 0) {
+            fk_seg_mask<<<dim3((rows_max + 255) / 256, md.n + 1), dim3(256), 0, st>>>(
+                md, h->fk_rgrp, h->fk_ginfo, h->fk_winfo, h->seg_tab, n_ph, make_int4(0, 0, 0, 0), tiles, h->fk_smask);
+            if ((rc = check_launch("fk_seg_mask"))) return rc;
           }
           DeltaScope ds(h);
-          if (gather2) {
-            float* h1a = h1_rows(h, h->fc2_rows);
-            if ((rc = run_fc1(h, h->Q, h->a_rows, na, h1a, st, mask, frac, fn)) ||
-                (rc = run_fc2(h, h1a, na, pr->y_alt, st, acrow)))
-              return rc;
-          } else if ((rc = run_fc(h, h->Q, h->a_rows, na, pr->y_alt, st, h->c_rows, mask, frac, fn))) {
+          if ((rc = fk_fc1(h, h->Q, h->fk_aseq, pa, h->fk_arows, (int)nw_pre, nullptr, h->fk_h1, st, h->fk_smask, tiles,
+                           h->fk_part, kFkParts * cap)) ||
+              (na > 0 && (rc = fk_reduce(h, h->fk_part, h->fk_aprow, na, h->fk_h1, st))))
             return rc;
+          if (na > 0) {
+            seg_a_rows<<<dim3((na + 255) / 256), dim3(256), 0, st>>>(
+                h->win_seg_d, h->win_off_d, win_row ? h->win_row_d : nullptr, h->fk_aperm, 0, na, s0, ss, L, n_ph,
+                phi, g.T6, h->fk_arows, h->fk_crows);
+            if ((rc = check_launch("seg_a_rows"))) return rc;
+            for (int r0 = 0; r0 < na; r0 += h->max_batch)
+              if ((rc = run_fc2(h, h->fk_h1 + (long long)r0 * kHidLd, std::min(h->max_batch, na - r0), pr->y_alt, st,
+                                h->fk_crows + r0)))
+                return rc;
           }
         }
-        if ((rc = flush2())) return rc;
-        if (pr) {
-          if (ic1 > ic0) {
-            copy_rows<<<dim3(ic1 - ic0), dim3(256), 0, st>>>(y, pr->y_alt, h->copy_w_d + ic0,
-                                                             win_row ? h->win_row_d : nullptr, row_base);
-            if ((rc = check_launch("copy_rows"))) return rc;
+        i0 = i1;
+      }
+      if (pr) {
+        const int ic0 = (int)(std::lower_bound(copy_w.begin(), copy_w.end(), w0) - copy_w.begin());
+        const int ic1 = (int)(std::lower_bound(copy_w.begin(), copy_w.end(), w0 + nw) - copy_w.begin());
+        if (ic1 > ic0) {
+          copy_rows<<<dim3(ic1 - ic0), dim3(256), 0, st>>>(y, pr->y_alt, h->copy_w_d + ic0,
+                                                           win_row ? h->win_row_d : nullptr, n_win, ss.rc_rows);
+          if ((rc = check_launch("copy_rows"))) return rc;
+        }
+      }
+    } else if (nw > 0) {
+      const int4 phi = make_int4(ph_idx[0], ph_idx[1], ph_idx[2], ph_idx[3]);
+      const int* widx = pr ? h->fc_perm_d + w0 : nullptr;
+      int n_alt = 0, ic0 = 0, ic1 = 0;
+      if (pr) {
+        n_alt = (int)(std::lower_bound(alt_w.begin(), alt_w.end(), w0 + nw) -
+                      std::lower_bound(alt_w.begin(), alt_w.end(), w0));
+        ic0 = (int)(std::lower_bound(copy_w.begin(), copy_w.end(), w0) - copy_w.begin());
+        ic1 = (int)(std::lower_bound(copy_w.begin(), copy_w.end(), w0 + nw) - copy_w.begin());
+      }
+      const bool gather2 = h->fc2_splits == 1;
+      int pend = 0;
+      auto flush2 = [&]() -> int {
+        const int n2 = pend;
+        pend = 0;
+        return n2 ? run_fc2(h, h->h1, n2, y, st, h->c_rows) : EXPECTO_OK;
+      };
+      for (int f0 = 0; f0 < nw; f0 += h->max_batch) {
+        const int fn = std::min(h->max_batch, nw - f0);
+        if (gather2 && pend + fn > h->fc2_rows && (rc = flush2())) return rc;
+        long long* crow = h->c_rows + (gather2 ? pend : 0);
+        seg_a_rows<<<dim3((fn + 255) / 256), dim3(256), 0, st>>>(
+            h->win_seg_d, h->win_off_d, win_row ? h->win_row_d : nullptr, widx ? widx + f0 : nullptr, w0 + f0,
+            fn, s0, ss, L, n_ph, phi, g.T6, h->a_rows, crow);
+        if ((rc = check_launch("seg_a_rows"))) return rc;
+        if (gather2) {
+          if ((rc = run_fc1(h, h->P, h->a_rows, fn, h1_rows(h, pend), st))) return rc;
+          pend += fn;
+        } else if ((rc = run_fc(h, h->P, h->a_rows, fn, y, st, h->c_rows))) {
+          return rc;
+        }
+        const int na = std::min(n_alt - f0, fn);
+        if (na <= 0) continue;
+        if (f0 == 0) {
+          if ((rc = st_wait(h->pev[13]))) return rc;
+          seg_alt_blocks<<<dim3(kAltRows6, (unsigned)nb), dim3(64), 0, st>>>(h->P, h->D0, n_ph, g.T6, h->seg_tab,
+                                                                            640 * eb / 16, h->Q);
+          if ((rc = check_launch("seg_alt_blocks"))) return rc;
+        }
+        long long* acrow = gather2 ? h->c_rows + h->fc2_rows : h->c_rows;
+        seg_a_rows<<<dim3((na + 255) / 256), dim3(256), 0, st>>>(
+            h->win_seg_d, h->win_off_d, win_row ? h->win_row_d : nullptr, widx + f0, 0, na, s0, ss, L, n_ph, phi,
+            g.T6, h->a_rows, acrow);
+        if ((rc = check_launch("seg_a_rows"))) return rc;
+        const unsigned* mask = nullptr;
+        double frac = 1.0;
+        if (planes_gemm()) {
+          const int tiles = (int)((na + gemm_bm() - 1) / gemm_bm());
+          unsigned* md = reinterpret_cast<unsigned*>(h->slab_mask);
+          EXPECTO_HIP_CHECK(hipMemsetAsync(md, 0, tiles * sizeof(unsigned), st));
+          fc1_slab_mask_seg<<<dim3((na + 255) / 256), dim3(256), 0, st>>>(
+              widx + f0, na, h->win_seg_d, h->win_off_d, s0, ss, L, phi, h->seg_tab, (int)gemm_bm(),
+              kFc1In / h->fc_splits, md);
+          if ((rc = check_launch("fc1_slab_mask_seg"))) return rc;
+          mask = md;
+          if (h->profiling) {
+            if ((rc = count_slab_macs(h, md, tiles, na, st))) return rc;
+            frac = 0.0;
           }
         }
+        DeltaScope ds(h);
+        if (gather2) {
+          float* h1a = h1_rows(h, h->fc2_rows);
+          if ((rc = run_fc1(h, h->Q, h->a_rows, na, h1a, st, mask, frac, fn)) ||
+              (rc = run_fc2(h, h1a, na, pr->y_alt, st, acrow)))
+            return rc;
+        } else if ((rc = run_fc(h, h->Q, h->a_rows, na, pr->y_alt, st, h->c_rows, mask, frac, fn))) {
+          return rc;
+        }
       }
-      if (pr && (rc = st_wait(h->pev[13]))) return rc;
-    }
+      if ((rc = flush2())) return rc;
+      if (pr) {
+        if (ic1 > ic0) {
+          copy_rows<<<dim3(ic1 - ic0), dim3(256), 0, st>>>(y, pr->y_alt, h->copy_w_d + ic0,
+                                                           win_row ? h->win_row_d : nullptr, n_win, ss.rc_rows);
+          if ((rc = check_launch("copy_rows"))) return rc;
+        }
+      }
+    }
+    if (pr && (rc = st_wait(h->pev[13]))) return rc;
   }
   return EXPECTO_OK;
 }
@@ -3334,6 +3339,7 @@
     h->fk_role = v;
   }
   if (const char* e = getenv("EXPECTO_SEG_CHUNK_WINDOWS")) h->seg_chunk_windows = atoi(e);
+  if (const char* e = getenv("EXPECTO_SEG_MERGE_STRANDS")) h->seg_merge_strands = atoi(e) != 0;
   if (const char* e = getenv("EXPECTO_CONV_NARROW")) {
     const int v = atoi(e);
     EXPECTO_REQUIRE(v >= -1 && v <= 1, "EXPECTO_CONV_NARROW must be -1 (auto), 0 or 1");
@@ -3365,6 +3371,9 @@
     if ((rc = dalloc(h, &rows, (size_t)(max_batch + h1_rows) * 2))) return fail(rc);
     h->a_rows = reinterpret_cast<long long*>(rows);
     h->c_rows = h->a_rows + max_batch;
+    float* gr = nullptr;
+    if ((rc = dalloc(h, &gr, (size_t)kGresPerBatch * max_batch))) return fail(rc);
+    h->fk_gres = reinterpret_cast<int*>(gr);
   }
   EXPECTO_HIP_CHECK(hipMemsetAsync(h->P, 0, act_alloc(pf) * sizeof(float), st));
   EXPECTO_HIP_CHECK(hipMemsetAsync(h->Q, 0, act_alloc(qf) * sizeof(float), st));
@@ -3390,7 +3399,6 @@
     if (p) (void)hipFree(p);
   for (float* p : h->fk_aseq)
     if (p) (void)hipFree(p);
-  if (h->fk_gres) (void)hipFree(h->fk_gres);
   if (h->seam) (void)hipFree(h->seam);
   if (h->edge) (void)hipFree(h->edge);
   for (void* p : h->allocs) (void)hipFree(p);
```
